# actionml/universal-recommender

Measured on AMD Instinct MI355X. Metric: cooccurrence pairs/sec (A'A+A'B) + LLR top-k items/sec, higher is better.
Workload: dtype int32 counts / f64 LLR; 1 GPU; config4: synthetic 10M users x 2M items, Zipf-1.0, 5 event types (purchase/view/add-to-cart/search/category-pref); generator=torch Philox on the GPU (universal_recommender_amd.synth.generate_device), maxEventsPerEventType=500, maxCorrelatorsPerEventType=50, seed=20260925, entry_point=urcco_context_build_device (C ABI, include/urcco.h), launch=one process per GPU, parallelism=items range-partitioned over 1 GPU(s), one HIP stream per event type

## Files before the change

universal-recommender_amd/csrc/cco_common.h:

```cpp
#pragma once
#include "cco_kernels.h"

namespace urcco {


constexpr int WAVE = 64;

__device__ __forceinline__ unsigned long long shfl_xor_u64(unsigned long long v, int m) {
  unsigned lo = (unsigned)v, hi = (unsigned)(v >> 32);
  lo = __shfl_xor(lo, m);
  hi = __shfl_xor(hi, m);
  return ((unsigned long long)hi << 32) | lo;
}
__device__ __forceinline__ long long shfl_i64(long long v, int src) {
  unsigned lo = (unsigned)v, hi = (unsigned)((unsigned long long)v >> 32);
  lo = __shfl(lo, src);
  hi = __shfl(hi, src);
  return (long long)(((unsigned long long)hi << 32) | lo);
}
__device__ __forceinline__ long long shfl_up_i64(long long v, unsigned d) {
  unsigned lo = (unsigned)v, hi = (unsigned)((unsigned long long)v >> 32);
  lo = __shfl_up(lo, d);
  hi = __shfl_up(hi, d);
  return (long long)(((unsigned long long)hi << 32) | lo);
}

__device__ __forceinline__ int64_t upper_bound_i64(const int64_t* __restrict__ rp, int64_t lo, int64_t hi, int64_t e) {
  while (lo < hi) {
    const int64_t mid = lo + ((hi - lo) >> 1);
    if (rp[mid] > e) hi = mid; else lo = mid + 1;
  }
  return lo;
}

constexpr int SCAN_THREADS = 256;
constexpr int SCAN_ITEMS = SCAN_TILE / SCAN_THREADS;

struct LoadI32 {
  const int32_t* p;
  __device__ __forceinline__ long long operator()(int64_t i) const { return p[i]; }
  __device__ __forceinline__ void load8(int64_t i, long long* x) const {
    if ((reinterpret_cast<uintptr_t>(p) & 15) == 0) {
      const int4 a = *reinterpret_cast<const int4*>(p + i), b = *reinterpret_cast<const int4*>(p + i + 4);
      x[0] = a.x; x[1] = a.y; x[2] = a.z; x[3] = a.w; x[4] = b.x; x[5] = b.y; x[6] = b.z; x[7] = b.w;
    } else {
#pragma unroll
      for (int q = 0; q < 8; ++q) x[q] = p[i + q];
    }
  }
};
struct LoadI64 {
  const int64_t* p;
  __device__ __forceinline__ long long operator()(int64_t i) const { return p[i]; }
  __device__ __forceinline__ void load8(int64_t i, long long* x) const {
    if ((reinterpret_cast<uintptr_t>(p) & 15) == 0) {
#pragma unroll
      for (int q = 0; q < 4; ++q) {
        const int4 a = *reinterpret_cast<const int4*>(p + i + 2 * q);
        x[2 * q] = (long long)(((unsigned long long)(unsigned)a.y << 32) | (unsigned)a.x);
        x[2 * q + 1] = (long long)(((unsigned long long)(unsigned)a.w << 32) | (unsigned)a.z);
      }
    } else {
#pragma unroll
      for (int q = 0; q < 8; ++q) x[q] = p[i + q];
    }
  }
};
template <int NT = SCAN_THREADS>
__device__ __forceinline__ long long block_exclusive_scan(long long v, long long* s_wave , long long* total) {
  const int lane = threadIdx.x & (WAVE - 1), wave = threadIdx.x / WAVE;
  long long inc = v;
#pragma unroll
  for (int d = 1; d < WAVE; d <<= 1) {
    const long long o = shfl_up_i64(inc, d);
    if (lane >= d) inc += o;
  }
  if (lane == WAVE - 1) s_wave[wave] = inc;
// ... 203 lines not shown
```

universal-recommender_amd/csrc/cco_expand.hip:

```cpp
#include "cco_kernels.h"

#include <atomic>
#include <cstdio>
#include <cstdlib>

#include "cco_common.h"
#include "cco_device.h"


namespace urcco {

__global__ __launch_bounds__(256) void item_entropy_kernel(const int32_t* __restrict__ counts, int32_t n, long long n_users,
                                                           double* __restrict__ ent, double* __restrict__ xlx_n) {
  const int64_t i = (int64_t)blockIdx.x * 256 + threadIdx.x;
  if (i < n) {
    const long long c = counts[i];
    ent[i] = entropy2(c, n_users - c);
  }
  if (i == 0 && xlx_n) *xlx_n = x_log_x(n_users);
}

hipError_t launch_item_entropy(hipStream_t st, const int32_t* counts, int32_t n, long long n_users, double* ent, double* xlx_n) {
  const int blocks = n > 0 ? (n + 255) / 256 : 1;
  hipLaunchKernelGGL(item_entropy_kernel, dim3(blocks), dim3(256), 0, st, counts, n, n_users, ent, xlx_n);
// ... 58 lines not shown
    const unsigned d0 = two ? (unsigned)cnt[z.x] : 0u, d1 = two ? (unsigned)cnt[z.y] : 0u, d2 = two ? (unsigned)cnt[z.z] : 0u, d3 = two ? (unsigned)cnt[z.w] : 0u;
    n_bad += (c0 >= limit) + (c1 >= limit) + (c2 >= limit) + (c3 >= limit) + (d0 >= limit) + (d1 >= limit) + (d2 >= limit) + (d3 >= limit);
    int4 y;
    y.x = (int)((unsigned)x.x | (c0 << shift)); y.y = (int)((unsigned)x.y | (c1 << shift));
    y.z = (int)((unsigned)x.z | (c2 << shift)); y.w = (int)((unsigned)x.w | (c3 << shift));
    nt_store4(out + 4 * v, y);
    if (two) {
      y.x = (int)((unsigned)z.x | (d0 << shift)); y.y = (int)((unsigned)z.y | (d1 << shift));
      y.z = (int)((unsigned)z.z | (d2 << shift)); y.w = (int)((unsigned)z.w | (d3 << shift));
      nt_store4(out + 4 * (v + stride), y);
    }
  }
  for (int64_t e = (nvec << 2) + (int64_t)blockIdx.x * 256 + threadIdx.x; e < nnz; e += stride) {
    const unsigned j = (unsigned)ci[e], c = (unsigned)cnt[j];
    n_bad += c >= limit;
    out[e] = (int)(j | (c << shift));
  }
  if (n_bad) atomicAdd(bad, n_bad);
}
hipError_t launch_pack_counts(hipStream_t st, int n_cu, const int32_t* col_idx, const int64_t* nnz_dev, int64_t nnz_bound, const unsigned short* counts16,
                              const int32_t* bad16, int32_t count_bits, int32_t* out, int32_t* bad) {
  hipError_t e = hipMemsetAsync(bad, 0, sizeof(int32_t), st);
  if (e != hipSuccess || nnz_bound <= 0) return e;
  const int shift = 32 - count_bits;
  int64_t blocks = (nnz_bound / 4 + 255) / 256;
  const int64_t cap = (int64_t)n_cu * 16;
  if (blocks > cap) blocks = cap;
  if (blocks < 1) blocks = 1;
  const int vec_ok = ((reinterpret_cast<uintptr_t>(col_idx) | reinterpret_cast<uintptr_t>(out)) & 15) == 0;
  hipLaunchKernelGGL(pack_counts_kernel, dim3((unsigned)blocks), dim3(256), 0, st, col_idx, nnz_dev, nnz_bound, counts16, bad16, shift, out, bad, vec_ok);
  return hipGetLastError();
}

__global__ __launch_bounds__(256) void xlx_table_kernel(double* __restrict__ tab) {
  const int x = blockIdx.x * 256 + threadIdx.x;
  if (x < XLX_TABLE) tab[x] = x_log_x((long long)x);
}
hipError_t launch_xlx_table(hipStream_t st, double* tab) {
  hipLaunchKernelGGL(xlx_table_kernel, dim3(XLX_TABLE / 256), dim3(256), 0, st, tab);
  return hipGetLastError();
}
__global__ __launch_bounds__(256) void xlx_hi_table_kernel(double* __restrict__ tab, const double* __restrict__ xlx_tab, long long n_users) {
  const int d = blockIdx.x * 256 + threadIdx.x;
  if (d >= XLX_TABLE) return;
  tab[d] = n_users - d >= 0 ? x_log_x(n_users - (long long)d) : 0.0;
  const double hi = n_users - d >= 0 ? x_log_x(n_users - (long long)d) : 0.0;
  tab[XLX_TABLE + d] = d <= n_users ? (x_log_x(n_users) - x_log_x_tab((long long)d, xlx_tab)) - hi : 0.0;
}
hipError_t launch_xlx_hi_table(hipStream_t st, double* tab, const double* xlx_tab, long long n_users) {
  hipLaunchKernelGGL(xlx_hi_table_kernel, dim3(XLX_TABLE / 256), dim3(256), 0, st, tab, xlx_tab, n_users);
  return hipGetLastError();
}

__global__ __launch_bounds__(SCAN_THREADS) void expand_downsweep_kernel(const int32_t* __restrict__ plen, int64_t n, const int64_t* __restrict__ tile_sums,
                                                                        int64_t n_tiles, int64_t* __restrict__ out, const int64_t* __restrict__ n_live,
                                                                        const int32_t* __restrict__ form, const unsigned* __restrict__ pstart32,
                                                                        int64_t* __restrict__ pstart64) {
  __shared__ long long s_wave[SCAN_THREADS / WAVE];
  if ((int64_t)blockIdx.x * SCAN_TILE > *n_live) return;
  const int f = *form;
  const LoadI32 ld{plen};
  const int64_t first = (int64_t)blockIdx.x * SCAN_TILE + (int64_t)threadIdx.x * SCAN_ITEMS;
  static_assert(SCAN_ITEMS == 8, "load8");
  long long x[SCAN_ITEMS];
  long long v = 0;
  const bool interior = first + SCAN_ITEMS <= n;
  if (interior) {
    ld.load8(first, x);
  } else {
#pragma unroll
    for (int q = 0; q < SCAN_ITEMS; ++q) x[q] = first + q < n ? ld(first + q) : 0;
  }
#pragma unroll
  for (int q = 0; q < SCAN_ITEMS; ++q) v += x[q];
  long long tot;
  long long run = block_exclusive_scan(v, s_wave, &tot) + tile_sums[blockIdx.x];
  if (f == 0) {
    unsigned* out32 = reinterpret_cast<unsigned*>(out);
    unsigned r = (unsigned)run;
    if (interior && (reinterpret_cast<uintptr_t>(out) & 15) == 0) {
      unsigned e[SCAN_ITEMS];
#pragma unroll
      for (int q = 0; q < SCAN_ITEMS; ++q) {
        e[q] = r;
        r += (unsigned)x[q];
      }
      *reinterpret_cast<uint4*>(out32 + first) = make_uint4(e[0], e[1], e[2], e[3]);
      *reinterpret_cast<uint4*>(out32 + first + 4) = make_uint4(e[4], e[5], e[6], e[7]);
    } else {
#pragma unroll
      for (int q = 0; q < SCAN_ITEMS; ++q) {
        if (first + q < n) out32[first + q] = r;
        r += (unsigned)x[q];
      }
    }
    if (blockIdx.x == 0 && threadIdx.x == 0) out32[n] = (unsigned)tile_sums[n_tiles];
    return;
  }
  if (interior && (reinterpret_cast<uintptr_t>(out) & 15) == 0) {
#pragma unroll
    for (int q = 0; q < SCAN_ITEMS; q += 2) {
      const long long e0 = run, e1 = run + x[q];
      run = e1 + x[q + 1];
      int4 w;
      w.x = (int)(unsigned)e0; w.y = (int)(unsigned)((unsigned long long)e0 >> 32);
      w.z = (int)(unsigned)e1; w.w = (int)(unsigned)((unsigned long long)e1 >> 32);
      *reinterpret_cast<int4*>(out + first + q) = w;
    }
  } else {
#pragma unroll
    for (int q = 0; q < SCAN_ITEMS; ++q) {
      const int64_t i = first + q;
      if (i < n) out[i] = run;
      run += x[q];
    }
  }
  if (!(f & FORM_PS64) && pstart32 && pstart64) {
#pragma unroll
    for (int q = 0; q < SCAN_ITEMS; ++q)
      if (first + q < n) pstart64[first + q] = (int64_t)pstart32[first + q];
  }
  if (blockIdx.x == 0 && threadIdx.x == 0) out[n] = tile_sums[n_tiles];
}
static hipError_t expand_scan(hipStream_t st, const int32_t* plen, int64_t cap, int64_t* wp, int64_t* tile_sums, const int64_t* n_live, bool tile_sums_ready,
                              const unsigned* pstart32, int64_t* pstart64, ExpandForm form) {
  const int64_t n_tiles = cap > 0 ? (cap + SCAN_TILE - 1) / SCAN_TILE : 1;
  if (!tile_sums_ready || cap <= 0)
    hipLaunchKernelGGL((scan_reduce_kernel<LoadI32>), dim3((unsigned)n_tiles), dim3(SCAN_THREADS), 0, st, LoadI32{plen}, cap, tile_sums, n_live);
  hipLaunchKernelGGL(scan_tiles_kernel, dim3(1), dim3(ST_THREADS), 0, st, tile_sums, n_tiles, n_live, form);
  hipLaunchKernelGGL(expand_downsweep_kernel, dim3((unsigned)n_tiles), dim3(SCAN_THREADS), 0, st, plen, cap, (const int64_t*)tile_sums, n_tiles, wp, n_live,
                     (const int32_t*)form.word, pstart32, pstart64);
  return hipGetLastError();
}

__global__ __launch_bounds__(256) void narrow_row_ptr_kernel(const int64_t* __restrict__ rp, int64_t n, unsigned* __restrict__ out) {
  for (int64_t i = (int64_t)blockIdx.x * 256 + threadIdx.x; i < n; i += (int64_t)gridDim.x * 256) out[i] = (unsigned)rp[i];
}

__global__ __launch_bounds__(256) void expand_prepare_kernel(const int64_t* __restrict__ a_cp, int32_t n_items_a, const int32_t* __restrict__ a_ri,
                                                             const int64_t* __restrict__ b_rp, const unsigned* __restrict__ b_rp32, int64_t n_rows_b,
                                                             int64_t cap, unsigned* __restrict__ pstart32, int64_t* __restrict__ pstart64,
                                                             int32_t* __restrict__ plen, int32_t* __restrict__ form) {
  const int64_t nnz = a_cp[n_items_a];
  int64_t lim = (nnz / SCAN_TILE + 1) * SCAN_TILE;
  if (lim > cap) lim = cap;
  const bool narrow = b_rp32 != nullptr && b_rp[n_rows_b] < ((int64_t)1 << 32);
  if (!narrow && pstart64 && blockIdx.x == 0 && threadIdx.x == 0) *form = FORM_PS64;
  const int64_t stride = (int64_t)gridDim.x * 256;
  for (int64_t p0 = (int64_t)blockIdx.x * 256 + threadIdx.x; p0 < lim; p0 += stride * 4) {
    int u[4];
#pragma unroll
    for (int q = 0; q < 4; ++q) {
      const int64_t p = p0 + q * stride;
      u[q] = p < nnz ? a_ri[p] : -1;
    }
    int64_t s[4], e[4];
    if (narrow) {
#pragma unroll
      for (int q = 0; q < 4; ++q) {
        s[q] = u[q] >= 0 ? (int64_t)b_rp32[u[q]] : 0;
        e[q] = u[q] >= 0 ? (int64_t)b_rp32[u[q] + 1] : 0;
      }
    } else {
#pragma unroll
      for (int q = 0; q < 4; ++q) {
        s[q] = u[q] >= 0 ? b_rp[u[q]] : 0;
        e[q] = u[q] >= 0 ? b_rp[u[q] + 1] : 0;
      }
    }
#pragma unroll
    for (int q = 0; q < 4; ++q) {
      const int64_t p = p0 + q * stride;
      if (p < lim) {
        if (narrow) {
          if (pstart32) pstart32[p] = (unsigned)s[q];
        } else if (pstart64) {
          pstart64[p] = s[q];
        }
        plen[p] = (int32_t)(e[q] - s[q]);
      }
    }
  }
}

hipError_t launch_expand_prepare(hipStream_t st, int n_cu, const int64_t* a_col_ptr, int32_t n_items_a, const int32_t* a_row_idx,
                                 const int64_t* b_row_ptr, unsigned* b_rp32_scratch, int64_t n_rows_b, int64_t cap, unsigned* pstart32, int64_t* pstart64,
                                 int32_t* plen, int64_t* wp, int64_t* tile_sums, ExpandForm form) {
  hipError_t e = hipMemsetAsync(form.word, 0, sizeof(int32_t), st);
  if (e != hipSuccess) return e;
  if (cap > 0) {
    if (b_rp32_scratch) {
      int64_t nb = (n_rows_b + 1 + 255) / 256;
      if (nb > (int64_t)n_cu * 8) nb = (int64_t)n_cu * 8;
      hipLaunchKernelGGL(narrow_row_ptr_kernel, dim3((unsigned)nb), dim3(256), 0, st, b_row_ptr, n_rows_b + 1, b_rp32_scratch);
    }
    int64_t blocks = (cap + 1023) / 1024;
    const int64_t lim = (int64_t)n_cu * 16;
    if (blocks > lim) blocks = lim;
    hipLaunchKernelGGL(expand_prepare_kernel, dim3((unsigned)blocks), dim3(256), 0, st, a_col_ptr, n_items_a, a_row_idx, b_row_ptr,
                       (const unsigned*)b_rp32_scratch, n_rows_b, cap, pstart32, pstart64, plen, form.word);
  }
  return expand_scan(st, plen, cap, wp, tile_sums, a_col_ptr + n_items_a, false, pstart32, pstart64, form);
}

struct __attribute__((packed, aligned(4))) Words4 { unsigned a, b, c, d; };
struct __attribute__((packed, aligned(4))) Words2 { unsigned a, b; };
struct ExpandMultiArgs {
  const int64_t* b_rp[EXPAND_MULTI_MAX];
  unsigned* pstart[EXPAND_MULTI_MAX];
  int32_t* plen[EXPAND_MULTI_MAX];
  int64_t* tsum[EXPAND_MULTI_MAX];
  int n;
};
__global__ __launch_bounds__(256) void expand_pack_kernel(ExpandMultiArgs a, int64_t n_rows_b, unsigned* __restrict__ T) {
  for (int64_t u = (int64_t)blockIdx.x * 256 + threadIdx.x; u <= n_rows_b; u += (int64_t)gridDim.x * 256)
    for (int d = 0; d < a.n; ++d) T[u * a.n + d] = (unsigned)a.b_rp[d][u];
}
template <int N>
__global__ __launch_bounds__(256) void expand_prepare_multi_kernel(const int64_t* __restrict__ a_cp, int32_t n_items_a, const int32_t* __restrict__ a_ri,
                                                                   const unsigned* __restrict__ T, int64_t cap, ExpandMultiArgs a) {
  __shared__ long long s_part[256 / WAVE][N];
  const int64_t nnz = a_cp[n_items_a];
  int64_t lim = (nnz / SCAN_TILE + 1) * SCAN_TILE;
  if (lim > cap) lim = cap;
  const int64_t n_tiles = (lim + SCAN_TILE - 1) / SCAN_TILE;
  for (int64_t tile = blockIdx.x; tile < n_tiles; tile += gridDim.x) {
    const int64_t base = tile * SCAN_TILE;
    long long sum[N];
#pragma unroll
    for (int d = 0; d < N; ++d) sum[d] = 0;
    for (int r = 0; r < SCAN_ITEMS; r += 2) {
      int u[2];
      unsigned v[2][2 * N];
#pragma unroll
      for (int q = 0; q < 2; ++q) {
        const int64_t p = base + (int64_t)(r + q) * 256 + threadIdx.x;
        u[q] = p < nnz ? a_ri[p] : -1;
      }
#pragma unroll
      for (int q = 0; q < 2; ++q) {
        if (u[q] >= 0) {
          const unsigned* t = T + (int64_t)u[q] * N;
          if (N == 4) {
            const uint4 x = *reinterpret_cast<const uint4*>(t), y = *reinterpret_cast<const uint4*>(t + 4);
            v[q][0] = x.x; v[q][1] = x.y; v[q][2] = x.z; v[q][3] = x.w;
            v[q][4 % (2 * N)] = y.x; v[q][5 % (2 * N)] = y.y; v[q][6 % (2 * N)] = y.z; v[q][7 % (2 * N)] = y.w;
          } else {
            constexpr int W = 2 * N;
#pragma unroll
            for (int d = 0; d + 4 <= W; d += 4) {
              const Words4 x = *reinterpret_cast<const Words4*>(t + d);
              v[q][d] = x.a; v[q][(d + 1) % W] = x.b; v[q][(d + 2) % W] = x.c; v[q][(d + 3) % W] = x.d;
            }
            if (W % 4 >= 2) {
              const Words2 x = *reinterpret_cast<const Words2*>(t + (W / 4) * 4);
              v[q][(W / 4) * 4 % W] = x.a; v[q][((W / 4) * 4 + 1) % W] = x.b;
            }
            if (W % 2 == 1) v[q][W - 1] = t[W - 1];
          }
        } else {
#pragma unroll
          for (int d = 0; d < 2 * N; ++d) v[q][d] = 0u;
        }
      }
#pragma unroll
      for (int q = 0; q < 2; ++q) {
        const int64_t p = base + (int64_t)(r + q) * 256 + threadIdx.x;
        if (p < lim) {
#pragma unroll
          for (int d = 0; d < N; ++d) {
            const int32_t len = (int32_t)(v[q][N + d] - v[q][d]);
            a.pstart[d][p] = v[q][d];
            a.plen[d][p] = len;
            sum[d] += (long long)len;
          }
        }
      }
    }
#pragma unroll
    for (int d = 0; d < N; ++d) {
      unsigned long long x = (unsigned long long)sum[d];
#pragma unroll
      for (int m = 1; m < WAVE; m <<= 1) x += shfl_xor_u64(x, m);
      if ((threadIdx.x & (WAVE - 1)) == 0) s_part[threadIdx.x / WAVE][d] = (long long)x;
    }
    __syncthreads();
    if (threadIdx.x < N && a.tsum[threadIdx.x]) {
      long long tot = 0;
#pragma unroll
      for (int w = 0; w < 256 / WAVE; ++w) tot += s_part[w][threadIdx.x];
      a.tsum[threadIdx.x][tile] = tot;
    }
    __syncthreads();
  }
}
hipError_t launch_expand_prepare_multi(hipStream_t st, int n_cu, const int64_t* a_col_ptr, int32_t n_items_a, const int32_t* a_row_idx, int n,
                                       const int64_t* const* b_row_ptr, int64_t n_rows_b, int64_t cap, unsigned* const* pstart, int32_t* const* plen, void* T,
                                       int64_t* const* tsum) {
  if (n < 1 || n > EXPAND_MULTI_MAX) return hipErrorInvalidValue;
  if (cap <= 0) return hipSuccess;
  ExpandMultiArgs a;
  a.n = n;
  for (int d = 0; d < EXPAND_MULTI_MAX; ++d) {
    a.b_rp[d] = d < n ? b_row_ptr[d] : nullptr;
    a.pstart[d] = d < n ? pstart[d] : nullptr;
    a.plen[d] = d < n ? plen[d] : nullptr;
    a.tsum[d] = (d < n && tsum) ? tsum[d] : nullptr;
  }
  int64_t nb = (n_rows_b + 255) / 256;
  if (nb > (int64_t)n_cu * 8) nb = (int64_t)n_cu * 8;
  if (nb < 1) nb = 1;
  hipLaunchKernelGGL(expand_pack_kernel, dim3((unsigned)nb), dim3(256), 0, st, a, n_rows_b, static_cast<unsigned*>(T));
  int64_t blocks = (cap + SCAN_TILE - 1) / SCAN_TILE;
  const int64_t lim = (int64_t)n_cu * 16;
  if (blocks > lim) blocks = lim;
  const unsigned* Tc = static_cast<const unsigned*>(T);
  switch (n) {
    case 1: hipLaunchKernelGGL(expand_prepare_multi_kernel<1>, dim3((unsigned)blocks), dim3(256), 0, st, a_col_ptr, n_items_a, a_row_idx, Tc, cap, a); break;
    case 2: hipLaunchKernelGGL(expand_prepare_multi_kernel<2>, dim3((unsigned)blocks), dim3(256), 0, st, a_col_ptr, n_items_a, a_row_idx, Tc, cap, a); break;
    case 3: hipLaunchKernelGGL(expand_prepare_multi_kernel<3>, dim3((unsigned)blocks), dim3(256), 0, st, a_col_ptr, n_items_a, a_row_idx, Tc, cap, a); break;
    case 4: hipLaunchKernelGGL(expand_prepare_multi_kernel<4>, dim3((unsigned)blocks), dim3(256), 0, st, a_col_ptr, n_items_a, a_row_idx, Tc, cap, a); break;
    case 5: hipLaunchKernelGGL(expand_prepare_multi_kernel<5>, dim3((unsigned)blocks), dim3(256), 0, st, a_col_ptr, n_items_a, a_row_idx, Tc, cap, a); break;
    case 6: hipLaunchKernelGGL(expand_prepare_multi_kernel<6>, dim3((unsigned)blocks), dim3(256), 0, st, a_col_ptr, n_items_a, a_row_idx, Tc, cap, a); break;
    case 7: hipLaunchKernelGGL(expand_prepare_multi_kernel<7>, dim3((unsigned)blocks), dim3(256), 0, st, a_col_ptr, n_items_a, a_row_idx, Tc, cap, a); break;
    default: hipLaunchKernelGGL(expand_prepare_multi_kernel<8>, dim3((unsigned)blocks), dim3(256), 0, st, a_col_ptr, n_items_a, a_row_idx, Tc, cap, a); break;
  }
  return hipGetLastError();
}
hipError_t launch_expand_scan(hipStream_t st, const int64_t* a_col_ptr, int32_t n_items_a, const int32_t* plen, int64_t cap, int64_t* wp, int64_t* tile_sums,
                              bool tile_sums_ready, const unsigned* pstart32, int64_t* pstart64, ExpandForm form) {
  hipError_t e = hipMemsetAsync(form.word, 0, sizeof(int32_t), st);
  if (e != hipSuccess) return e;
  return expand_scan(st, plen, cap, wp, tile_sums, a_col_ptr + n_items_a, tile_sums_ready, pstart32, pstart64, form);
}

__device__ __forceinline__ int64_t work_prefix_at(const int64_t* __restrict__ wp, const int64_t* __restrict__ tile_sums, bool narrow, int64_t p) {
  if (!narrow) return wp[p];
  const int64_t base = tile_sums[p / SCAN_TILE];
  return base + (int64_t)(unsigned)(reinterpret_cast<const unsigned*>(wp)[p] - (unsigned)base);
}
__global__ __launch_bounds__(256) void row_work_kernel(int32_t item_lo, int32_t item_hi, const int64_t* __restrict__ a_cp,
                                                       const int64_t* __restrict__ wp, const int64_t* __restrict__ tile_sums, const int32_t* __restrict__ form,
                                                       int64_t* __restrict__ work) {
  const int64_t n = (int64_t)item_hi - item_lo;
  const bool narrow = *form == 0;
  for (int64_t t = (int64_t)blockIdx.x * 256 + threadIdx.x; t < n; t += (int64_t)gridDim.x * 256) {
    const int64_t i = item_lo + t;
    work[t] = work_prefix_at(wp, tile_sums, narrow, a_cp[i + 1]) - work_prefix_at(wp, tile_sums, narrow, a_cp[i]);
  }
}

hipError_t launch_row_work(hipStream_t st, int n_cu, int32_t item_lo, int32_t item_hi, const int64_t* a_col_ptr, const int64_t* wp, const int64_t* tile_sums,
                           const int32_t* form, int64_t* work) {
  const int64_t n = (int64_t)item_hi - item_lo;
  if (n <= 0) return hipSuccess;
  int64_t blocks = (n + 255) / 256;
  const int64_t cap = (int64_t)n_cu * 8;
  if (blocks > cap) blocks = cap;
  hipLaunchKernelGGL(row_work_kernel, dim3((unsigned)blocks), dim3(256), 0, st, item_lo, item_hi, a_col_ptr, wp, tile_sums, form, work);
  return hipGetLastError();
}


}
```

universal-recommender_amd/csrc/cco_kernels.h:

```cpp
#pragma once
#include <hip/hip_runtime.h>
#include <stdint.h>

namespace urcco {

constexpr int NBINS = 7;
constexpr int MP_KMAX_HOST = 256;

constexpr int SCAN_TILE = 2048;
constexpr int DS_TILE = 4096;
constexpr int GLOBAL_BIN_BLOCKS = 128;
constexpr int BIN_TILE = 1024;
constexpr int XLX_TABLE_HOST = 4096;
constexpr int BIN_COLS_HOST = 3 * NBINS + 3;
constexpr int BIN_OFF_LEN = NBINS + 3;
constexpr int CAND_SLOTS = 64;
constexpr int STATS_LEN = 32;

constexpr int32_t DBG_GATHER_ONLY = 1;
constexpr int32_t DBG_NO_LLR = 2;
constexpr int32_t DBG_NO_TOPK = 4;
constexpr int32_t DBG_NO_SELECT = 8;
constexpr int32_t DBG_NO_RANK = 16;
constexpr int32_t DBG_NO_COUNT_GATHER = 512;
constexpr int32_t DBG_UNFUSED_EXPAND = 4096;
constexpr int32_t DBG_GATHERED_PRIMARY = 8192;
constexpr int32_t DBG_UNFILTERED_EXCHANGE = 16384;
constexpr int32_t DBG_SELECT_DELAY = 131072;
constexpr int32_t DBG_UNPACKED_COUNTS = 1048576;
constexpr int32_t DBG_ROW_KERNELS = DBG_GATHER_ONLY | DBG_NO_LLR | DBG_NO_TOPK | DBG_NO_SELECT | DBG_NO_RANK | DBG_NO_COUNT_GATHER | DBG_SELECT_DELAY;

constexpr int32_t FORM_WIDE = 1;
constexpr int32_t FORM_PS64 = 2;
constexpr int32_t FORM_TILE = 4;
constexpr int32_t FORM_PACK = 8;
constexpr int32_t FORM_HOST = 16;
constexpr unsigned long long NARROW_LIMIT = 1ull << 32;
struct ExpandForm {
  int32_t* word;
  const int32_t* pack_bad;
  int32_t host_wide;
  int32_t host_narrow;
  unsigned long long limit;
  long long seed;
};

struct CcoArgs {
  const int32_t* bin_rows;
  const int32_t* bin_off;
  const int64_t* a_col_ptr;
  const unsigned* pstart32;
  const int64_t* wp;
  const int32_t* b_col_idx;
  const int32_t* b_packed;
  const int32_t* form;
  int32_t pk_known;
  uint32_t b_col_mask;
  const int32_t* cnt_a;
  const int32_t* cnt_b;
  const double* ent_a;
  const unsigned short* cnt_b16;
  const int32_t* cnt16_bad;
  const double* xlx_n;
  const double* xlx_tab;
  const double* xlx_hi;
  const double* col_ent;
  int32_t debug;
  long long n_users;
  int32_t n_cols_b;
  int32_t item_lo;
  int32_t exclude_self;
  int32_t k;
  int32_t has_min_llr;
  double min_llr;
  int32_t count_bits;
  int32_t col_bytes;
  int32_t g_log2;
  int32_t unordered;
  int32_t* out_count;
  int32_t* out_idx;
  double* out_llr;
  unsigned long long* err;
  unsigned long long* cand;
  int32_t* g_counts;
  unsigned long long* g_cand_key;
  int32_t* g_cand_col;
  int32_t g_blocks;
  const int64_t* pstart64;
  const int64_t* work;
};

hipError_t launch_column_counts(hipStream_t st, int n_cu, const int32_t* col_idx, int64_t nnz, int32_t n_cols, int32_t* counts);
constexpr int64_t PH_MIN_NNZ = 1 << 20;
int64_t column_counts_scratch_bytes(int64_t nnz, int32_t n_cols);
hipError_t launch_column_counts_partitioned(hipStream_t st, const int32_t* col_idx, int64_t nnz, const int64_t* nnz_dev, int32_t n_cols,
                                            int32_t* counts, char* scratch);

hipError_t launch_scan_i32(hipStream_t st, const int32_t* in, int64_t n, int64_t* out, int64_t* tile_sums);
hipError_t launch_slice_weights(hipStream_t st, const unsigned short* loc_t, int n_buckets, int64_t n_parts, long long* weight);

hipError_t launch_downsample_flags(hipStream_t st, int n_cu, int64_t n_rows, const int64_t* row_ptr, const int32_t* col_idx, int64_t nnz,
                                   int32_t n_cols, const int32_t* raw_counts, unsigned long long* thresholds, uint32_t seed, int32_t max_n,
                                   int row_rate_mode, int64_t row_base, int64_t* tile_rows, unsigned long long* flags, int64_t* tile_count,
                                   int32_t* post_counts);
hipError_t launch_downsample_scan(hipStream_t st, int64_t nnz, int64_t* tile_count);
hipError_t launch_downsample_compact(hipStream_t st, int64_t n_rows, const int64_t* row_ptr, const int32_t* col_idx, int64_t nnz,
                                     const int64_t* tile_rows, const unsigned long long* flags, const int64_t* tile_off, int64_t* out_row_ptr,
                                     int32_t* out_col_idx);

hipError_t launch_scan_i32_range(hipStream_t st, const int32_t* in, int64_t n, int32_t lo, int32_t hi, int64_t* out, int64_t* tile_sums);
hipError_t launch_transpose(hipStream_t st, int n_cu, int64_t n_rows, const int64_t* row_ptr, const int32_t* col_idx, int g_log2,
                            const int64_t* col_ptr, int32_t* cursor, int32_t* out_row_idx, int32_t col_lo, int32_t col_hi);
int64_t transpose_scratch_bytes(int64_t n_rows, int64_t nnz, int32_t n_cols);
hipError_t launch_transpose_partitioned(hipStream_t st, int64_t n_rows, const int64_t* row_ptr, const int32_t* col_idx, int64_t nnz, int32_t n_cols,
                                        const int64_t* col_ptr, int32_t* cursor , int32_t* out_row_idx, int32_t col_lo, int32_t col_hi, char* scratch);
hipError_t launch_row_work_csr(hipStream_t st, int n_cu, int64_t n_rows, const int64_t* a_row_ptr, const int32_t* a_col_idx,
                               const int64_t* b_row_ptr, int g_log2, int32_t n_items_a, int64_t* work);

struct KeyTable {
  unsigned long long* keys;
  unsigned* minpos;
  unsigned* count;
  int32_t* id;
  unsigned long long mask;
};
hipError_t launch_dictionary_build(hipStream_t st, int n_cu, KeyTable t, int64_t n, const unsigned long long* keys, const int32_t* select,
                                   int32_t min_count, int32_t* flag, int64_t* prefix, int64_t* tile_sums, int64_t* first_pos);
hipError_t launch_dictionary_lookup(hipStream_t st, int n_cu, KeyTable t, int64_t n, const unsigned long long* keys, const int32_t* select,
                                    int32_t* ids);
hipError_t launch_dictionary_verify(hipStream_t st, int n_cu, KeyTable t, int64_t n, const unsigned long long* keys, const int32_t* select,
                                    const unsigned long long* check, const unsigned long long* ref_check, const int64_t* first_pos, unsigned long long* err);
hipError_t launch_csr_from_pairs(hipStream_t st, int n_cu, int64_t n, const int32_t* rows, const int32_t* cols, int64_t n_rows, int32_t* cnt,
                                 int64_t* raw_ptr, int32_t* tmp, int64_t* tile_sums, int64_t* out_row_ptr, int32_t* out_col_idx);

constexpr int EXCH_SIZES = 4;
hipError_t launch_row_lengths(hipStream_t st, int n_cu, int64_t n_rows, const int64_t* row_ptr, int32_t* len, unsigned short* len16, int64_t* sizes);
hipError_t launch_counts_over_limit(hipStream_t st, int n_cu, const int32_t* counts, int64_t n, int32_t count_bits, int64_t* out);
hipError_t launch_need_mask(hipStream_t st, int n_cu, int64_t n_rows, const int64_t* a_row_ptr, const int32_t* a_col_idx, const int32_t* bounds, int world,
                            unsigned long long* mask);
hipError_t launch_masked_lengths(hipStream_t st, int n_cu, int64_t n_rows, const int64_t* row_ptr, const unsigned long long* mask, int world, int32_t* mlen, int64_t* off,
                                 int64_t* tile_sums, int64_t* to_nnz);
hipError_t launch_pack_rows(hipStream_t st, int n_cu, int64_t n_rows, const int64_t* row_ptr, const int32_t* col_idx, const unsigned long long* mask, int world,
                            const int64_t* off, int32_t* pack);
hipError_t launch_scan_u16(hipStream_t st, const unsigned short* in, int64_t n, int64_t* out, int64_t* tile_sums);
hipError_t launch_frag_record(hipStream_t st, int32_t world, const int32_t* bounds, const int64_t* l_cp, const int32_t* bad, int64_t* rec);
hipError_t launch_frag_place(hipStream_t st, int n_cu, int32_t world, int32_t lo, int32_t n_range, const void* lens, int wire16, const int64_t* src_off,
                             const int32_t* ents, const int64_t* a_cp, const int64_t* sizes, int32_t* a_ri);

hipError_t launch_validate_csr(hipStream_t st, int n_cu, int64_t n_rows, const int64_t* row_ptr, const int32_t* col_idx, int64_t nnz, int32_t n_cols,
                               int g_log2, int64_t rp0, unsigned long long* err);
hipError_t launch_rebase_i64(hipStream_t st, int n_cu, int64_t* p, int64_t n, int64_t delta);
hipError_t launch_publish_word(hipStream_t st, const unsigned long long* src, unsigned long long* dst_mapped);

hipError_t launch_pop_counts(hipStream_t st, int n_cu, int64_t n, const int32_t* item, const int64_t* t_ms, int32_t n_items, int n_buckets,
                             const int64_t* bounds, int32_t* counts);

hipError_t launch_pack_counts(hipStream_t st, int n_cu, const int32_t* col_idx, const int64_t* nnz_dev, int64_t nnz_bound, const unsigned short* counts16,
                              const int32_t* bad16, int32_t count_bits, int32_t* out, int32_t* bad);
hipError_t launch_xlx_table(hipStream_t st, double* tab);
hipError_t launch_xlx_hi_table(hipStream_t st, double* tab , const double* xlx_tab, long long n_users);
hipError_t launch_item_entropy(hipStream_t st, const int32_t* counts, int32_t n, long long n_users, double* ent, double* xlx_n);
hipError_t launch_narrow_counts(hipStream_t st, int n_cu, const int32_t* counts, int64_t n, unsigned short* out16, int32_t* bad);

hipError_t launch_expand_prepare(hipStream_t st, int n_cu, const int64_t* a_col_ptr, int32_t n_items_a, const int32_t* a_row_idx,
                                 const int64_t* b_row_ptr, unsigned* b_rp32_scratch , int64_t n_rows_b, int64_t cap,
                                 unsigned* pstart32, int64_t* pstart64, int32_t* plen, int64_t* wp, int64_t* tile_sums, ExpandForm form);
constexpr int EXPAND_MULTI_MAX = 8;
hipError_t launch_expand_prepare_multi(hipStream_t st, int n_cu, const int64_t* a_col_ptr, int32_t n_items_a, const int32_t* a_row_idx, int n,
                                       const int64_t* const* b_row_ptr, int64_t n_rows_b, int64_t cap, unsigned* const* pstart, int32_t* const* plen, void* T,
                                       int64_t* const* tsum );
hipError_t launch_expand_scan(hipStream_t st, const int64_t* a_col_ptr, int32_t n_items_a, const int32_t* plen, int64_t cap, int64_t* wp, int64_t* tile_sums,
                              bool tile_sums_ready, const unsigned* pstart32, int64_t* pstart64, ExpandForm form);
hipError_t launch_row_work(hipStream_t st, int n_cu, int32_t item_lo, int32_t item_hi, const int64_t* a_col_ptr, const int64_t* wp, const int64_t* tile_sums,
                           const int32_t* form, int64_t* work);

hipError_t launch_binning(hipStream_t st, int32_t item_lo, int32_t n, const int64_t* work, const int32_t* cnt_a, int32_t n_cols_b,
                          int32_t count_bits, int32_t k, int64_t* tile_counts, int32_t* bin_off, int32_t* bin_rows, int64_t* stats);

hipError_t launch_cco_rows_bin(hipStream_t st, int n_cu, const CcoArgs& args, int bin, int32_t n_rows );
hipError_t launch_bin_out_stats(hipStream_t st, const int32_t* bin_rows, const int32_t* bin_off, int32_t item_lo, const int32_t* out_count,
                                const unsigned long long* cand, int64_t* stats);

hipError_t launch_compact_indicators(hipStream_t st, int32_t n_rows, int32_t k, const int32_t* count, const int32_t* idx,
                                     const double* llr, const int64_t* row_ptr, int32_t* out_idx, double* out_llr);

hipError_t launch_partition(hipStream_t st, int32_t n_items, const int64_t* work_prefix, int32_t n_parts, int32_t* bounds);
hipError_t launch_scan_i64(hipStream_t st, const int64_t* in, int64_t n, int64_t* out, int64_t* tile_sums);

constexpr int REC_MAX_CLAUSES = 16;
constexpr int REC_MAX_NUM = 256;
constexpr int REC_NO_BACKFILL = 1;
constexpr int REC_STATS_LEN = 8;
constexpr int REC_LDS_LIMIT = 3072;
struct RecClause {
  const int64_t* ind_col_ptr;
  const int32_t* ind_row_idx;
  const int64_t* q_row_ptr;
  const int32_t* q_col_idx;
  double boost;
  int32_t n_cols;
  int32_t reserved;
};
constexpr int REC_MAX_RULES = 16;
constexpr int REC_RULE_ANY = 0;
constexpr int REC_RULE_NONE = 1;
constexpr int REC_RULE_RANGE = 2;
struct RecRule {
  const int64_t* m_row_ptr;
  const int32_t* m_col_idx;
  const int64_t* q_row_ptr;
  const int32_t* q_col_idx;
  const int64_t* item_value;
  const int64_t* q_lo;
  const int64_t* q_hi;
  int32_t kind, n_cols;
};
struct RecArgs;
int32_t recommend_global_blocks(int64_t n_queries, int32_t n_items, int n_cu);
hipError_t launch_recommend(hipStream_t st, int n_cu, int64_t n_queries, int32_t n_items, const RecClause* clauses, int32_t n_clauses, const int64_t* excl_row_ptr,
                            const int32_t* excl_col_idx, const uint8_t* item_mask, const int32_t* fill_order, int32_t num, int32_t flags, int32_t* out_count,
                            int32_t* out_idx, double* out_score, int64_t* stats_dev, unsigned long long* ctr, int32_t* list, int32_t* pos, int32_t g_blocks,
                            unsigned* g_state, unsigned* g_m, int32_t* g_list, double* g_score, int32_t lds_limit = REC_LDS_LIMIT, const RecRule* rules = nullptr,
                            int32_t n_rules = 0);

hipError_t launch_llr_test(hipStream_t st, int64_t n, const int64_t* a, const int64_t* b, const int64_t* ab, const int64_t* nu, double* out);
hipError_t launch_u01_test(hipStream_t st, int64_t n, uint32_t seed, const int32_t* row, const int32_t* col, double* out, int rng32 = 0);

// ... 2 lines not shown
```

universal-recommender_amd/csrc/cco_rows.hip:

```cpp
#include "cco_kernels.h"

#include <atomic>
#include <cstdlib>

#include "cco_common.h"
#include "cco_device.h"


namespace urcco {

constexpr int E0 = 1024, E1S = 4096, E1 = 8192, E2S = 16384, E2 = 32768;
constexpr int MP_KMAX = 256;

__host__ __device__ constexpr int table_slots(int E, int T) { return (2 * E / 3) / (2 * T) * (2 * T); }
constexpr int URCCO_WB1 = 512;
constexpr int URCCO_WB2 = 8192;
__device__ __forceinline__ int choose_bin(long long w, long long ca, int32_t n_cols_b, int32_t count_bits, int32_t k) {
  if (ca <= 0 || w <= 0) return -1;
  if (count_bits < 31 && ca > ((1ll << count_bits) - 1)) return NBINS - 1;
  if (w <= 64 && ca <= 64) return 0;
  int cap_bin = NBINS - 1;
  const long long dmax = (w < (long long)n_cols_b ? w : (long long)n_cols_b) * 3 + (long long)k * 3 + 2;
  if (dmax <= E0) cap_bin = 1;
  else if (dmax <= E1S) cap_bin = 2;
// ... 390 lines not shown

template <int T>
__device__ __forceinline__ unsigned claim_positions(bool want, unsigned* counter, unsigned& wave_count) {
  const unsigned long long m = __ballot(want);
  const unsigned c = (unsigned)__popcll(m);
  unsigned base;
  if (T == WAVE) {
    base = wave_count;
    wave_count += c;
  } else {
    unsigned b = 0u;
    if ((threadIdx.x & (WAVE - 1)) == 0 && c != 0u) b = atomicAdd(counter, c);
    base = wave_read_lane(b, 0);
  }
  return base + lanes_below(m);
}
template <int T>
__device__ __forceinline__ unsigned team_exclusive_scan(unsigned v, unsigned* s_wsum , unsigned* total) {
  const int lane = threadIdx.x & (WAVE - 1);
  const unsigned inc = wave_inclusive_sum(v);
  if (T == WAVE) {
    *total = wave_read_lane(inc, WAVE - 1);
    return inc - v;
  }
  const int wave = (threadIdx.x % T) / WAVE;
  if (lane == WAVE - 1) s_wsum[wave] = inc;
  __syncthreads();
  unsigned base = 0, tot = 0;
#pragma unroll
  for (int w = 0; w < T / WAVE; ++w) {
    const unsigned sw = s_wsum[w];
    if (w < wave) base += sw;
    tot += sw;
  }
  __syncthreads();
  *total = tot;
  return base + inc - v;
}

constexpr int URCCO_U_WAVE = 2;
constexpr int URCCO_U_BS = 2;
constexpr int URCCO_U_B = 2;
constexpr int URCCO_U_H = 1;
constexpr int URCCO_U_C = 1;
constexpr int URCCO_OCC_WAVE = 8;
constexpr int URCCO_OCC_BS = 7;
constexpr int URCCO_G_WAVE = 2;
constexpr int URCCO_SEL_AMB_WAVE = 64;
constexpr int URCCO_SEL_AMB_BLOCK = 128;
constexpr int URCCO_G_BLOCK = 2;
constexpr int URCCO_SEL_M_BLOCK = 128;
constexpr int URCCO_G_CU = 2;
template <bool NARROW> struct PStart { typedef int64_t type; };
template <> struct PStart<true> { typedef unsigned type; };
template <int T, int E, int U, bool MP = false, bool DBG = false, bool PK = false>
__global__ __launch_bounds__((T < 256 ? 256 : T), (T == 64 ? URCCO_OCC_WAVE : (T == 256 && E == 4096 ? URCCO_OCC_BS : (T == 512 ? 4 : 1)))) void cco_rows_kernel(CcoArgs a, int bin) {
  if ((a.b_packed != nullptr && (a.pk_known != 0 || *a.form == 0)) != PK) return;
  using PS = typename PStart<PK>::type;
  constexpr int WS = PK ? 1 : 2;
  const int dbg = DBG ? a.debug : 0;
  constexpr bool packed = PK;
  URCCO_OWN_GLOBAL_PTR(const int32_t, b_col_idx, PK ? a.b_packed : a.b_col_idx);
  const int cshift = 32 - a.count_bits;
  const unsigned colmask = PK ? (1u << cshift) - 1u : a.b_col_mask;
  URCCO_OWN_GLOBAL_PTR(const unsigned short, cnt_b16, a.cnt_b16);
  URCCO_OWN_GLOBAL_PTR(const int32_t, cnt_b, a.cnt_b);
  URCCO_OWN_GLOBAL_PTR(const double, xlx_tab, a.xlx_tab);
  URCCO_OWN_GLOBAL_PTR(const double, xlx_hi, a.xlx_hi);
  URCCO_OWN_GLOBAL_PTR(const double, col_ent, a.col_ent);
  URCCO_OWN_GLOBAL_PTR(int32_t, out_idx, a.out_idx);
  URCCO_OWN_GLOBAL_PTR(double, out_llr, a.out_llr);
  long long n_users = a.n_users;
  URCCO_OWN_SGPRS(n_users);
  constexpr int BLOCK = T < 256 ? 256 : T;
  constexpr int TEAMS = BLOCK / T;
  constexpr int SH = table_slots(E, T);
  constexpr int SPT = SH / T;
  static_assert(SH % (2 * T) == 0 && SH + SH / 2 <= E && SH <= 65536, "slots and the candidate list share the table; a slot index takes 16 bits of a list word");
  constexpr unsigned CAND_CAP = (unsigned)(E - SH);
  constexpr int CPT = ((E - 5) / 3 + T - 1) / T;
  constexpr int NW = T / WAVE;
  constexpr int G = T == WAVE ? URCCO_G_WAVE : (T == 256 ? URCCO_G_BLOCK : URCCO_G_CU);
  constexpr int LOG2E = E == 1024 ? 10 : (E == 4096 ? 12 : (E == 8192 ? 13 : (E == 16384 ? 14 : 15)));
  static_assert((1 << LOG2E) == E, "table size");
  constexpr int LOG2T = T == 64 ? 6 : (T == 256 ? 8 : (T == 512 ? 9 : 10));
  static_assert((1 << LOG2T) == T, "team size");
  __shared__ __attribute__((aligned(16))) unsigned s_tab[TEAMS * E];
  constexpr int NH = T == WAVE ? 1 : 3;
  constexpr int SEL_CAP = T == WAVE ? 0 : (T == 256 ? 512 : 2048);
  constexpr int SEL_M = T == WAVE ? 64 : URCCO_SEL_M_BLOCK;
  constexpr int SEL_AMB = T == WAVE ? URCCO_SEL_AMB_WAVE : URCCO_SEL_AMB_BLOCK;
  static_assert(SEL_AMB <= SEL_M, "ambiguous set capacity");
  constexpr bool SHARE = T == WAVE || (T == 256 && E == 4096);
  constexpr int SH_INS = T * 8 + (T + 1) * 4;
  constexpr int SH_LST = ((NH * 128 * 4 > SEL_M * 12 ? NH * 128 * 4 : SEL_M * 12) + 7) / 8 * 8;
  constexpr int SH_SEL = SH_LST + SEL_CAP * 2;
  constexpr int SHARE_WORDS = ((SH_INS > SH_SEL ? SH_INS : SH_SEL) + 7) / 8;
  __shared__ unsigned long long s_share[SHARE ? TEAMS * SHARE_WORDS : 1];
  __shared__ long long s_ustart[SHARE ? 1 : TEAMS * T];
  __shared__ unsigned s_uoff[SHARE ? 1 : TEAMS * (T + 1)];
  __shared__ unsigned s_wsum[NW];
  __shared__ unsigned s_hist[SHARE ? 1 : TEAMS * NH * 128];
  __shared__ unsigned s_selres[TEAMS * 4];
  __shared__ unsigned short s_lst[SHARE ? 1 : TEAMS * (SEL_CAP > 0 ? SEL_CAP : 1)];
  __shared__ unsigned long long s_ambkey[SHARE ? 1 : TEAMS * SEL_M];
  __shared__ unsigned s_ambcol[SHARE ? 1 : TEAMS * SEL_M];
  __shared__ unsigned long long s_selthr[TEAMS * 2];
  constexpr bool SKIP_SHARED = T >= 256;
  __shared__ unsigned long long s_kbits[2 * NW];
  __shared__ unsigned s_mpflag;
  __shared__ unsigned s_ncand;
  __shared__ unsigned long long s_runk[MP ? 2 * MP_KMAX : 1];
  __shared__ unsigned s_runc[MP ? 2 * MP_KMAX : 1];

  const int team = TEAMS == 1 ? 0 : uni((int)threadIdx.x / T);
  const int tl = threadIdx.x % T;
  const int lane = threadIdx.x & (WAVE - 1);
  unsigned* tab = s_tab + team * E;
  unsigned* cand = tab + SH;
  unsigned long long* share = s_share + (SHARE ? team * SHARE_WORDS : 0);
  PS* ustart = reinterpret_cast<PS*>(SHARE ? reinterpret_cast<long long*>(share) : s_ustart + team * T);
  unsigned* uoff = SHARE ? reinterpret_cast<unsigned*>(share + T) : s_uoff + team * (T + 1);
  unsigned* hist = SHARE ? reinterpret_cast<unsigned*>(share) : s_hist + team * NH * 128;
  unsigned* sel_res = s_selres + team * 4;
  unsigned* nsel = sel_res + 3;
  unsigned short* lst = SHARE ? reinterpret_cast<unsigned short*>(share) + SH_LST / 2 : s_lst + team * (SEL_CAP > 0 ? SEL_CAP : 1);
  unsigned long long* amb_key = SHARE ? share : s_ambkey + team * SEL_M;
  unsigned* amb_col = SHARE ? reinterpret_cast<unsigned*>(share + SEL_M) : s_ambcol + team * SEL_M;
  unsigned long long* sel_thr = s_selthr + team * 2;
  const int list_start = a.bin_off[bin];
  const int list_n = a.bin_off[bin + 1] - list_start;
  const int total_teams = gridDim.x * TEAMS;
  bool ident = (long long)a.n_cols_b * 3 + (long long)a.k * 3 + 2 <= E && a.n_cols_b <= SH;
  int cb = a.count_bits;
  unsigned cmask = (1u << cb) - 1u;
  unsigned long long cand_acc = 0ull;
  const double xlx_n = *a.xlx_n;
  const bool use16 = *a.cnt16_bad == 0;

  int li = blockIdx.x * TEAMS + team;
  if (li >= list_n) return;
  const int S = total_teams;
  auto pos_of = [&](int l) { return list_start + (l < list_n ? l : list_n - 1); };
  const unsigned* wp32 = reinterpret_cast<const unsigned*>(a.wp);
  const PS* pstart;
  if constexpr (PK) pstart = a.pstart32;
  else pstart = a.pstart64;
  const int lane3 = lane < 3 ? lane : 2;
  int idv = a.bin_rows[pos_of(li + lane3 * S)];
  int64_t cs_c, ce_c;
  int64_t bnd_b;
  {
    const int id0 = (int)wave_read_lane((unsigned)idv, 0);
    const int id1 = (int)wave_read_lane((unsigned)idv, 1);
    cs_c = uni(a.a_col_ptr[id0]);
    ce_c = uni(a.a_col_ptr[id0 + 1]);
    bnd_b = a.a_col_ptr[id1 + (lane & 1)];
  }
  unsigned pf_w0, pf_w1, pf_wp;
  PS pf_start;
  {
    const int64_t c1 = cs_c + T < ce_c ? cs_c + T : ce_c;
    const int64_t pl = cs_c + tl < c1 ? cs_c + tl : c1 - 1;
    pf_w0 = wp32[WS * cs_c];
    pf_w1 = wp32[WS * c1];
    pf_wp = wp32[WS * pl];
    pf_start = pstart[pl];
  }
  URCCO_SETTLE(idv); URCCO_SETTLE(bnd_b); URCCO_SETTLE(pf_w0); URCCO_SETTLE(pf_w1); URCCO_SETTLE(pf_wp); URCCO_SETTLE(pf_start);
  int64_t cs_n = 0, ce_n = 0, bnd_c = 0;
  for (; li < list_n; li += S, cs_c = cs_n, ce_c = ce_n, bnd_b = bnd_c) {
    const int i = (int)wave_read_lane((unsigned)idv, 0);
    const int id2 = (int)wave_read_lane((unsigned)idv, 2);
    const int64_t cs = cs_c, ce = ce_c;
    cs_n = wave_read_lane64(bnd_b, 0);
    ce_n = wave_read_lane64(bnd_b, 1);
    const unsigned row_w0 = uni(pf_w0), row_w1 = uni(pf_w1);
    const unsigned my_wp = pf_wp;
    const PS my_start = pf_start;
    int lz = lane;
    URCCO_OPAQUE(lz);
    idv = a.bin_rows[pos_of(li + (1 + (lz < 3 ? lz : 2)) * S)];
    bnd_c = a.a_col_ptr[id2 + (lz & 1)];
    if (!MP) {
      const int64_t c1 = cs_n + T < ce_n ? cs_n + T : ce_n;
      const int64_t pl = cs_n + tl < c1 ? cs_n + tl : c1 - 1;
      pf_w0 = wp32[WS * cs_n];
      pf_w1 = wp32[WS * c1];
      pf_wp = wp32[WS * pl];
      pf_start = pstart[pl];
    }
    int mp_s = 0;
    unsigned mp_q = 0u, n_run = 0u, run_cur = 0u;
    if (MP) {
      const long long w_row = (long long)uni(a.work[i - a.item_lo]);
      const long long ca_row = a.cnt_a[i];
      const long long dd = w_row < (long long)a.n_cols_b ? w_row : (long long)a.n_cols_b;
      const long long cap = ((long long)E - 3ll * a.k - 2ll) / 3ll;
      for (;; ++mp_s) {
        const long long cols_pp = ((long long)a.n_cols_b + (1ll << mp_s) - 1) >> mp_s;
        int kb = 1;
        while ((1ll << kb) <= cols_pp) ++kb;
        const bool count_ok = kb <= 1 || ca_row <= (1ll << (32 - kb)) - 1;
        const long long exp_d = ((dd >> mp_s) + (dd >> (mp_s + 2)) + 1) < cols_pp ? ((dd >> mp_s) + (dd >> (mp_s + 2)) + 1) : cols_pp;
        if (count_ok && exp_d <= cap) break;
      }
    }
  mp_again:
    if (MP) {
      const long long cols_pp = ((long long)a.n_cols_b + (1ll << mp_s) - 1) >> mp_s;
      int kb = 1;
      while ((1ll << kb) <= cols_pp) ++kb;
      cb = 32 - kb;
      cmask = cb >= 32 ? 0xffffffffu : (1u << cb) - 1u;
      ident = cols_pp * 3 + 3ll * a.k + 2ll <= (long long)E && cols_pp <= (long long)SH;
      if (tl == 0) s_mpflag = 0u;
    }
    const unsigned mp_mask = MP ? (1u << mp_s) - 1u : 0u;
#pragma unroll
    for (int q = 0; q < SPT / 2; ++q) *reinterpret_cast<uint2*>(&tab[2 * (tl + q * T)]) = make_uint2(0u, 0u);
    unsigned n_cand = 0u;
    if (T != WAVE && tl == 0) s_ncand = 0u;
    team_sync<T>();
    for (int64_t c0 = cs; c0 < ce; c0 += T) {
      const int64_t c1 = c0 + T < ce ? c0 + T : ce;
      const bool pre = !MP && c0 == cs;
      const unsigned w0 = pre ? row_w0 : uni(wp32[WS * c0]);
      const unsigned total = (pre ? row_w1 : uni(wp32[WS * c1])) - w0;
      const int64_t p = c0 + tl;
      if (p < c1) {
        ustart[tl] = pre ? my_start : pstart[p];
        uoff[tl] = (pre ? my_wp : wp32[WS * p]) - w0;
      } else {
        uoff[tl] = total;
      }
      if (tl == 0) uoff[T] = total;
      team_sync<T>();
      if (total > 0u) {
        const unsigned per = (total + T - 1) / T;
        const unsigned first = (unsigned)tl * per;
        const bool act = first < total;
        const unsigned last = act ? (first + per < total ? first + per : total) : first;
        int o = 0;
        int64_t pos = 0;
        unsigned uend = 0u;
        if (act) {
          int lo = 1, hi = T;
#pragma unroll
          for (int step = 0; step < LOG2T; ++step) {
            const int mid = (lo + hi) >> 1;
            const bool gt = uoff[mid] > first;
            hi = gt ? mid : hi;
            lo = gt ? lo : mid + 1;
          }
          o = lo - 1;
          pos = (int64_t)ustart[o] + (first - uoff[o]);
          uend = uoff[o + 1];
        }
        for (unsigned x = 0; x < per; x += G) {
          unsigned jj[G];
          bool on[G];
#pragma unroll
          for (int q = 0; q < G; ++q) {
            const unsigned t = first + x + (unsigned)q;
            on[q] = t < last;
            jj[q] = 0u;
            if (on[q]) {
              if (t >= uend) {
                do { ++o; } while (uoff[o + 1] <= t);
                pos = (int64_t)ustart[o];
                uend = uoff[o + 1];
              }
              jj[q] = (unsigned)b_col_idx[pos++];
            }
          }
          unsigned at[G];
#pragma unroll
          for (int q = 0; q < G; ++q) {
            at[q] = ~0u;
            if (on[q]) {
              const unsigned col = jj[q] & colmask;
              if (dbg & DBG_GATHER_ONLY) {
                if (jj[q] == 0xffffffffu) tab[0] = 1u;
              } else if (MP) {
                if ((col & mp_mask) == mp_q && !tab_insert<SH>(tab, (col >> mp_s) + 1u, cb, ident, at[q])) s_mpflag = 1u;
// ... 72 lines not shown
    }
    cand_acc += D;
    unsigned long long* kk = reinterpret_cast<unsigned long long*>(tab + ((D + 1u) & ~1u));
    unsigned n_valid = 0;
    unsigned long long kand = ~0ull, kor = 0ull;
    {
      const long long ca = a.cnt_a[i];
      const double row_entropy = a.ent_a[i];
      for (unsigned base = 0; base < D; base += U * T) {
        const unsigned t0 = base + (unsigned)tl;
        unsigned vv[U];
        int cbj[U];
#pragma unroll
        for (int x = 0; x < U; ++x) {
          const unsigned t = t0 + (unsigned)x * T;
          vv[x] = t < D ? tab[t] : 0u;
          cbj[x] = 0;
          if (vv[x] != 0u) {
            const int j = MP ? (int)((((vv[x] >> cb) - 1u) << mp_s) | mp_q) : (int)(vv[x] >> cb) - 1;
            cbj[x] = packed ? (int)(unsigned)kk[t] : ((dbg & DBG_NO_COUNT_GATHER) ? (int)(vv[x] & cmask) + 100 : (use16 ? (int)cnt_b16[j] : cnt_b[j]));
          }
        }
        bool in_tables = true;
#pragma unroll
        for (int x = 0; x < U; ++x)
          if (vv[x] != 0u) in_tables = in_tables && llr_operands_in_tables(vv[x] & cmask, ca, (unsigned)cbj[x], n_users, col_ent);
        const bool all_in_tables = !(dbg & DBG_NO_LLR) && __ballot(!in_tables) == 0ull;
#pragma unroll
        for (int x = 0; x < U; ++x) {
          const unsigned t = t0 + (unsigned)x * T;
          if (t < D) {
            const int j = MP ? (int)((((vv[x] >> cb) - 1u) << mp_s) | mp_q) : (int)(vv[x] >> cb) - 1;
            const long long k11 = (long long)(vv[x] & cmask);
            unsigned long long key = 0ull;
            if (!(a.exclude_self && j == i)) {
              const double llr = all_in_tables ? llr_from_tables(row_entropy, xlx_n, (unsigned)k11, (unsigned)ca, (unsigned)cbj[x], xlx_tab, xlx_hi, col_ent)
                                               : ((dbg & DBG_NO_LLR) ? (double)k11
                                                            : llr_of(row_entropy, xlx_n, k11, ca, (long long)cbj[x], n_users, xlx_tab, xlx_hi, col_ent));
              if (llr > 0.0 && (!a.has_min_llr || llr >= a.min_llr)) key = (unsigned long long)__double_as_longlong(llr);
            }
            kk[t] = key;
            if (key != 0ull) {
              ++n_valid;
              if (SKIP_SHARED) {
                kand &= key;
                kor |= key;
              }
            }
          }
        }
      }
    }
    URCCO_SETTLE(idv); URCCO_SETTLE(bnd_c);
    if (!MP) { URCCO_SETTLE(pf_w0); URCCO_SETTLE(pf_w1); URCCO_SETTLE(pf_wp); URCCO_SETTLE(pf_start); }
    if (SKIP_SHARED) {
      wave_and_or_u64(kand, kor);
      if (lane == 0) {
        s_kbits[2 * (tl / WAVE)] = kand;
        s_kbits[2 * (tl / WAVE) + 1] = kor;
      }
    }
    unsigned C;
    team_exclusive_scan<T>(n_valid, s_wsum, &C);
    C = uni(C);
    team_sync<T>();
    const int64_t obase = ((int64_t)(i - a.item_lo)) * a.k;
    unsigned long long thr_key = 0ull;
    unsigned thr_ncol = 0u;
    bool row_done = false;
    if (!(dbg & DBG_NO_TOPK)) {
      if (dbg & DBG_NO_SELECT) {
        if (C > (unsigned)a.k) thr_key = ~0ull;
      } else if (C > (unsigned)a.k) {
        unsigned need = (unsigned)a.k;
        if (a.col_bytes < 4) thr_ncol = 0xffffffffu << (8 * a.col_bytes);
        int p0 = 0;
        if (!SKIP_SHARED) {
          kand = ~0ull;
          kor = 0ull;
          for (unsigned base = 0; base < D; base += T) {
            const unsigned t = base + (unsigned)tl;
            const unsigned long long key = t < D ? kk[t] : 0ull;
            if (key != 0ull) {
              kand &= key;
              kor |= key;
            }
          }
          wave_and_or_u64(kand, kor);
          if (T != WAVE) {
            if (lane == 0) {
              s_kbits[2 * (tl / WAVE)] = kand;
              s_kbits[2 * (tl / WAVE) + 1] = kor;
            }
            team_sync<T>();
          }
        }
        {
          if (T != WAVE) {
#pragma unroll
            for (int w = 0; w < NW; ++w) {
              kand &= s_kbits[2 * w];
              kor |= s_kbits[2 * w + 1];
            }
          }
          const unsigned long long kdiff = kand ^ kor;
          p0 = kdiff == 0ull ? 8 : (__clzll((long long)kdiff) >> 3);
          thr_key = p0 == 0 ? 0ull : (kor & ~(p0 >= 8 ? 0ull : (~0ull >> (8 * p0))));
// ... 267 lines not shown
    }
    team_sync<T>();
  }
  if (a.cand && tl == 0 && cand_acc != 0ull) atomicAdd(&a.cand[(blockIdx.x * TEAMS + team) & (CAND_SLOTS - 1)], cand_acc);
}

constexpr int URCCO_OCC_MICRO = 8;
template <int L> struct MicroGeom {
  static constexpr int S = WAVE / L;
  static constexpr int TW = 256 / S;
  static constexpr int LOG2TW = S == 1 ? 8 : (S == 2 ? 7 : 6);
  static constexpr int LIST = L + 4;
  static constexpr int MARKS = L + 2;
  static constexpr int ROW_WORDS = LIST + 2 * LIST + MARKS;
  static constexpr int WORDS = (256 + S * ROW_WORDS + 3) / 4 * 4;
};
template <int L>
__device__ __forceinline__ unsigned seg_inclusive_max(unsigned v) {
  if (L == WAVE) return wave_inclusive_max(v);
  int x = (int)v;
  int y;
  y = __builtin_amdgcn_update_dpp(0, x, 0x111, 0xf, 0xf, true);
  x = (unsigned)y > (unsigned)x ? y : x;
  y = __builtin_amdgcn_update_dpp(0, x, 0x112, 0xf, 0xf, true);
  x = (unsigned)y > (unsigned)x ? y : x;
  y = __builtin_amdgcn_update_dpp(0, x, 0x114, 0xf, 0xf, true);
  x = (unsigned)y > (unsigned)x ? y : x;
  y = __builtin_amdgcn_update_dpp(0, x, 0x118, 0xf, 0xf, true);
  x = (unsigned)y > (unsigned)x ? y : x;
  if (L == 32) {
    y = __builtin_amdgcn_update_dpp(0, x, 0x142, 0xa, 0xf, false);
    x = (unsigned)y > (unsigned)x ? y : x;
  }
  return (unsigned)x;
}
template <int L>
__device__ __forceinline__ unsigned seg_max_popc(unsigned long long m) {
  if (L == WAVE) return (unsigned)__popcll(m);
  unsigned best = 0;
#pragma unroll
  for (int q = 0; q < WAVE / L; ++q) {
    const unsigned c = (unsigned)__popcll((m >> (q * L)) & ((1ull << L) - 1ull));
    best = c > best ? c : best;
  }
  return best;
}

__device__ __forceinline__ unsigned gather_start(unsigned v, unsigned src) { return wave_gather(v, src); }
__device__ __forceinline__ int64_t gather_start(int64_t v, unsigned src) { return wave_gather64(v, src); }
template <int L, bool DBG, bool PK = false>
__global__ __launch_bounds__(256, (L == WAVE ? URCCO_OCC_MICRO : URCCO_OCC_MICRO - 2)) void cco_rows_micro_kernel(CcoArgs a) {
  if ((a.b_packed != nullptr && (a.pk_known != 0 || *a.form == 0)) != PK) return;
  using PS = typename PStart<PK>::type;
  constexpr int WS = PK ? 1 : 2;
  using G = MicroGeom<L>;
  constexpr int S = G::S;
  const int dbg = DBG ? a.debug : 0;
  const int32_t* bin_rows = a.bin_rows;
  const int64_t* a_col_ptr = a.a_col_ptr;
  const PS* pstart;
  if constexpr (PK) pstart = a.pstart32;
  else pstart = a.pstart64;
  constexpr bool packed = PK;
  const int32_t* b_col_idx = PK ? a.b_packed : a.b_col_idx;
  const int cshift = 32 - a.count_bits;
  const unsigned colmask = PK ? (1u << cshift) - 1u : a.b_col_mask;
  const int32_t* cnt_a = a.cnt_a;
  const double* ent_a = a.ent_a;
  const double* xlx_tab = a.xlx_tab;
  const double* xlx_hi = a.xlx_hi;
  const double* col_ent = a.col_ent;
  int32_t* out_idx = a.out_idx;
  double* out_llr = a.out_llr;
  int32_t* out_count = a.out_count;
  long long n_users = a.n_users;
  constexpr int TEAMS = 256 / WAVE;
  __shared__ __attribute__((aligned(16))) unsigned s_tab[TEAMS * G::WORDS];
  const int team = threadIdx.x / WAVE;
  const int lane = threadIdx.x & (WAVE - 1);
  const int seg = lane / L, sl = lane % L;
  const unsigned long long seg_mask = L == WAVE ? ~0ull : (((1ull << (L % WAVE)) - 1ull) << (seg * L));
  unsigned* tab_w = s_tab + team * G::WORDS;
  unsigned* tab = tab_w + seg * G::TW;
  unsigned* cand = tab_w + 256 + seg * G::ROW_WORDS;
  unsigned long long* kkm = reinterpret_cast<unsigned long long*>(cand + G::LIST);
  unsigned* marks = cand + 3 * G::LIST;
  const int list_start = L == 16 ? a.bin_off[0] : a.bin_off[NBINS + (L == 32 ? 1 : 2)];
  const int list_n = (L == 16 ? a.bin_off[NBINS + 1] : (L == 32 ? a.bin_off[NBINS + 2] : a.bin_off[1])) - list_start;
  const int n_groups = (list_n + S - 1) / S;
  const int total_teams = gridDim.x * TEAMS;
  const bool ident = a.n_cols_b <= G::TW;
  const int cb = a.count_bits;
  const unsigned cmask = (1u << cb) - 1u;
  const double xlx_n = *a.xlx_n;
  const bool use16 = *a.cnt16_bad == 0;
  unsigned long long cand_acc = 0ull;

  int li = blockIdx.x * TEAMS + team;
  if (li >= n_groups) return;
  const int stride = total_teams;
  auto row_at = [&](int g) { const int l = g * S + seg; return bin_rows[list_start + (l < list_n ? l : list_n - 1)]; };
  const unsigned* wp32 = reinterpret_cast<const unsigned*>(a.wp);
  const unsigned* cnt_words = use16 ? reinterpret_cast<const unsigned*>(a.cnt_b16) : reinterpret_cast<const unsigned*>(a.cnt_b);
  int i_cur = row_at(li);
  int i_n1 = row_at(li + stride);
  int i_n2 = row_at(li + 2 * stride);
  int64_t cs1 = a_col_ptr[i_n1], ce1 = a_col_ptr[i_n1 + 1];
  unsigned pf_w1, pf_wp;
  PS pf_start;
  int pf_ca;
  double pf_ent;
  int n_cur;
  {
    const int64_t cs0 = a_col_ptr[i_cur], ce0 = a_col_ptr[i_cur + 1];
    n_cur = (int)(ce0 - cs0);
    const int64_t pl = sl < n_cur ? cs0 + sl : ce0 - 1;
    pf_w1 = wp32[WS * ce0];
    pf_wp = wp32[WS * pl];
    pf_start = pstart[pl];
    pf_ca = cnt_a[i_cur];
    pf_ent = ent_a[i_cur];
  }
  URCCO_SETTLE(pf_w1); URCCO_SETTLE(pf_wp); URCCO_SETTLE(pf_start); URCCO_SETTLE(pf_ca); URCCO_SETTLE(pf_ent);
  URCCO_SETTLE(cs1); URCCO_SETTLE(ce1); URCCO_SETTLE(i_n2);
#pragma unroll
  for (int q = 0; q < 4; ++q) tab_w[lane + q * WAVE] = 0u;
  for (; li < n_groups; li += stride) {
    const int i = i_cur;
    const bool live = S == 1 || li * S + seg < list_n;
    const unsigned w0 = S == 1 ? wave_read_lane(pf_wp, 0) : wave_gather(pf_wp, (unsigned)(lane & ~(L - 1)));
    const unsigned total = live ? pf_w1 - w0 : 0u;
    const bool owns_user = live && sl < n_cur;
    const long long ca = (long long)pf_ca;
    const double row_entropy = pf_ent;
    const PS my_start = owns_user ? pf_start : (PS)0;
    const unsigned my_off = owns_user ? pf_wp - w0 : total;
    int i_n3 = row_at(li + 3 * stride);
    int64_t cs2 = a_col_ptr[i_n2], ce2 = a_col_ptr[i_n2 + 1];
    n_cur = (int)(ce1 - cs1);
    {
      const int64_t pl = sl < n_cur ? cs1 + sl : ce1 - 1;
      pf_w1 = wp32[WS * ce1];
      pf_wp = wp32[WS * pl];
      pf_start = pstart[pl];
      pf_ca = cnt_a[i_n1];
      pf_ent = ent_a[i_n1];
    }
    marks[sl] = 0u;
    wave_sync();
    if (owns_user) atomicMax(&marks[my_off], (unsigned)sl);
    wave_sync();
    const unsigned o = seg_inclusive_max<L>(marks[sl]);
    const PS base_o = gather_start(my_start - (PS)my_off, (unsigned)(seg * L) + o);
    unsigned slot = 0xffffffffu;
    unsigned jj = 0u;
    if ((unsigned)sl < total) {
      jj = (unsigned)b_col_idx[base_o + (PS)sl];
      if (!(dbg & DBG_GATHER_ONLY)) {
        bool ok;
        slot = tab_insert_claim(tab, (jj & colmask) + 1u, cb, (unsigned)(G::TW - 1), 32 - G::LOG2TW, ident, &ok);
        if (!ok) atomicAdd(a.err, 1ull);
      }
    }
    wave_sync();
    const bool is_cand = slot != 0xffffffffu;
    const unsigned long long cand_mask = __ballot(is_cand);
    const unsigned D = (unsigned)__popcll(cand_mask & seg_mask);
    const unsigned D_max = seg_max_popc<L>(cand_mask);
    cand_acc += (unsigned)__popcll(cand_mask);
    unsigned long long mk = 0ull;
    unsigned vv = 0u, cb_raw = 0u;
    if (is_cand) {
      vv = tab[slot];
      tab[slot] = 0u;
      const int j = (int)(vv >> cb) - 1;
      if (!packed) cb_raw = cnt_words[use16 ? j >> 1 : j];
    }
    if (D + (unsigned)sl < (unsigned)G::LIST) {
      kkm[D + (unsigned)sl] = 0ull;
      cand[D + (unsigned)sl] = 0xffffffffu;
    }
    bool in_tables = true;
    if (is_cand) {
      const int j = (int)(vv >> cb) - 1;
      const long long k11 = (long long)(vv & cmask);
      const unsigned cbj = packed ? jj >> cshift : ((dbg & DBG_NO_COUNT_GATHER) ? (unsigned)k11 + 100u : (use16 ? ((j & 1) ? cb_raw >> 16 : cb_raw & 0xffffu) : cb_raw));
      in_tables = llr_operands_in_tables((unsigned)k11, ca, cbj, n_users, col_ent);
    }
    const bool all_in_tables = !(dbg & DBG_NO_LLR) && __ballot(is_cand && !in_tables) == 0ull;
    if (is_cand) {
      const int j = (int)(vv >> cb) - 1;
      const long long k11 = (long long)(vv & cmask);
      if (!(a.exclude_self && j == i)) {
        const unsigned cbj = packed ? jj >> cshift : ((dbg & DBG_NO_COUNT_GATHER) ? (unsigned)k11 + 100u : (use16 ? ((j & 1) ? cb_raw >> 16 : cb_raw & 0xffffu) : cb_raw));
        const double llr = all_in_tables ? llr_from_tables(row_entropy, xlx_n, (unsigned)k11, (unsigned)ca, cbj, xlx_tab, xlx_hi, col_ent)
                                         : ((dbg & DBG_NO_LLR) ? (double)k11
                                                      : llr_of(row_entropy, xlx_n, k11, ca, (long long)cbj, n_users, xlx_tab, xlx_hi, col_ent));
        if (llr > 0.0 && (!a.has_min_llr || llr >= a.min_llr)) mk = (unsigned long long)__double_as_longlong(llr);
      }
      const unsigned pos = lanes_below(cand_mask & seg_mask);
      kkm[pos] = mk;
      cand[pos] = (unsigned)j;
    }
    wave_sync();
    const unsigned long long valid_mask = __ballot(mk != 0ull);
    const int n_valid = __popcll(valid_mask & seg_mask);
    const bool all_fit_k = (int)seg_max_popc<L>(valid_mask) <= a.k;
    auto settle_prefetch = [&]() {
      URCCO_SETTLE(pf_w1); URCCO_SETTLE(pf_wp); URCCO_SETTLE(pf_start); URCCO_SETTLE(pf_ca); URCCO_SETTLE(pf_ent);
      URCCO_SETTLE(cs2); URCCO_SETTLE(ce2); URCCO_SETTLE(i_n3);
    };
    if (a.unordered && all_fit_k && !(dbg & DBG_NO_TOPK)) {
      const int64_t obase = ((int64_t)(i - a.item_lo)) * a.k;
      settle_prefetch();
      if (mk != 0ull) {
        const unsigned opos = lanes_below(valid_mask & seg_mask);
        out_idx[obase + opos] = (int)(vv >> cb) - 1;
        out_llr[obase + opos] = __longlong_as_double((long long)mk);
      }
      if (sl == 0 && live) out_count[i - a.item_lo] = n_valid;
    } else if (!(dbg & DBG_NO_TOPK)) {
      const int64_t obase = ((int64_t)(i - a.item_lo)) * a.k;
      unsigned rank;
      unsigned long long rk;
      unsigned rc;
      unsigned ln = (unsigned)sl;
      URCCO_OPAQUE(ln);
      if (D_max <= (unsigned)(L / 4)) {
        const unsigned c = ln & (unsigned)(L / 4 - 1);
        rk = kkm[c];
        rc = cand[c];
        rank = rank_by_counting_strided<4>(kkm, cand, ln / (unsigned)(L / 4), (D_max + 3u) & ~3u, rk, rc);
        rank += (unsigned)__shfl_xor((int)rank, L / 4);
        rank += (unsigned)__shfl_xor((int)rank, L / 2);
      } else if (D_max <= (unsigned)(L / 2)) {
        const unsigned c = ln & (unsigned)(L / 2 - 1);
        rk = kkm[c];
        rc = cand[c];
        rank = rank_by_counting_strided<2>(kkm, cand, ln / (unsigned)(L / 2), (D_max + 1u) & ~1u, rk, rc);
        rank += (unsigned)__shfl_xor((int)rank, L / 2);
      } else {
        rk = kkm[ln];
        rc = cand[ln];
        rank = rank_by_counting_strided<1>(kkm, cand, 0u, D_max, rk, rc);
      }
      wave_sync();
      const unsigned n_out = (unsigned)(n_valid < a.k ? n_valid : a.k);
      if ((unsigned)sl < D && rk != 0ull && rank < n_out) {
        cand[rank] = rc;
        kkm[rank] = rk;
      }
      wave_sync();
      settle_prefetch();
      if ((unsigned)sl < n_out) {
        out_idx[obase + sl] = (int)cand[sl];
        out_llr[obase + sl] = __longlong_as_double((long long)kkm[sl]);
      }
      if (sl == 0 && live) out_count[i - a.item_lo] = (int)n_out;
    } else {
      settle_prefetch();
    }
    i_cur = i_n1;
    i_n1 = i_n2;
    i_n2 = i_n3;
    cs1 = cs2;
    ce1 = ce2;
    wave_sync();
  }
  if (a.cand && lane == 0 && cand_acc != 0ull) atomicAdd(&a.cand[(blockIdx.x * TEAMS + team) & (CAND_SLOTS - 1)], cand_acc);
}

constexpr int GB_THREADS = 1024;
constexpr int GSEL_K = 1024;

__device__ __forceinline__ int64_t g_start(const unsigned* ps32, const int64_t* ps64, bool nar, int64_t p) { return nar ? (int64_t)ps32[p] : ps64[p]; }
__device__ __forceinline__ int64_t g_len(const int64_t* wp, bool nar, int64_t p) {
  const unsigned* w = reinterpret_cast<const unsigned*>(wp);
  return nar ? (int64_t)(unsigned)(w[p + 1] - w[p]) : wp[p + 1] - wp[p];
}
__global__ __launch_bounds__(GB_THREADS) void cco_rows_global_kernel(CcoArgs a) {
  constexpr int NW = GB_THREADS / WAVE;
  __shared__ unsigned long long s_pkey[2][NW];
  __shared__ int s_pcol[2][NW];
  __shared__ int s_ncand;
  __shared__ unsigned s_hist[256];
  __shared__ unsigned s_sel[4];
  __shared__ int s_nsel;
  __shared__ unsigned long long s_selk[GSEL_K];
  __shared__ unsigned s_selc[GSEL_K];
  const int bin = NBINS - 1;
  const int list_start = a.bin_off[bin];
  const int list_n = a.bin_off[bin + 1] - list_start;
  int32_t* cnt = a.g_counts + (int64_t)blockIdx.x * a.n_cols_b;
  unsigned long long* ckey = a.g_cand_key + (int64_t)blockIdx.x * a.n_cols_b;
  int32_t* ccol = a.g_cand_col + (int64_t)blockIdx.x * a.n_cols_b;
  const int lane = threadIdx.x & (WAVE - 1), wv = threadIdx.x / WAVE;
  const int G = 1 << a.g_log2;
  const int grp = threadIdx.x >> a.g_log2, gl = threadIdx.x & (G - 1), ngrp = GB_THREADS >> a.g_log2;
  const double xlx_n = *a.xlx_n;
  const bool nar = *a.form == 0;
  for (int li = blockIdx.x; li < list_n; li += gridDim.x) {
    const int i = a.bin_rows[list_start + li];
    const int64_t cs = a.a_col_ptr[i], ce = a.a_col_ptr[i + 1];
    if (threadIdx.x == 0) s_ncand = 0;
    for (int64_t p = cs + grp; p < ce; p += ngrp) {
      const int64_t s = g_start(a.pstart32, a.pstart64, nar, p), e = s + g_len(a.wp, nar, p);
      for (int64_t q = s + gl; q < e; q += G) atomicAdd(&cnt[(unsigned)a.b_col_idx[q] & a.b_col_mask], 1);
    }
    __syncthreads();
    const long long ca = a.cnt_a[i];
    const double row_entropy = a.ent_a[i];
    for (int64_t p = cs + grp; p < ce; p += ngrp) {
      const int64_t s = g_start(a.pstart32, a.pstart64, nar, p), e = s + g_len(a.wp, nar, p);
      for (int64_t q = s + gl; q < e; q += G) {
        const int j = (int)((unsigned)a.b_col_idx[q] & a.b_col_mask);
        const long long k11 = atomicExch(&cnt[j], 0);
        if (k11 > 0 && !(a.exclude_self && j == i)) {
          const long long cbj = a.cnt_b[j];
          const double llr = llr_from_entropies_tab(row_entropy, column_entropy_of(cbj, xlx_n, a.n_users, a.xlx_tab, a.xlx_hi, a.col_ent), xlx_n, k11, ca - k11, cbj - k11,
                                                    a.n_users - ca - cbj + k11, a.xlx_tab, a.n_users, a.xlx_hi);
          if (llr > 0.0 && (!a.has_min_llr || llr >= a.min_llr)) {
            const int pos = atomicAdd(&s_ncand, 1);
            ckey[pos] = (unsigned long long)__double_as_longlong(llr);
            ccol[pos] = j;
          }
        }
      }
    }
    __syncthreads();
    const int ncand = s_ncand;
    const int64_t obase = ((int64_t)(i - a.item_lo)) * a.k;
    if (a.k <= GSEL_K) {
      unsigned long long thr_key = 0ull;
      unsigned thr_ncol = 0u;
      if (ncand > a.k) {
        unsigned need = (unsigned)a.k;
        if (a.col_bytes < 4) thr_ncol = 0xffffffffu << (8 * a.col_bytes);
        const int first_col_pass = 8 + (3 - (a.col_bytes - 1));
        for (int p = 0; p < 12; ++p) {
          if (p >= 8 && p < first_col_pass) continue;
          if (threadIdx.x < 256) s_hist[threadIdx.x] = 0u;
          __syncthreads();
          const int shk = p < 8 ? 56 - 8 * p : 0, shc = p < 8 ? 0 : 24 - 8 * (p - 8);
          for (int t = threadIdx.x; t < ncand; t += GB_THREADS) {
            const unsigned long long key = ckey[t];
            bool match;
            unsigned dig;
            if (p < 8) {
              match = p == 0 || (key >> (shk + 8)) == (thr_key >> (shk + 8));
              dig = (unsigned)(key >> shk) & 255u;
            } else {
              const unsigned ncol = ~(unsigned)ccol[t];
              match = key == thr_key && (p == first_col_pass || (ncol >> (shc + 8)) == (thr_ncol >> (shc + 8)));
              dig = (ncol >> shc) & 255u;
            }
            if (match) atomicAdd(&s_hist[dig], 1u);
          }
          __syncthreads();
          if (threadIdx.x == 0) {
            unsigned above = 0u, d = 255u;
            for (;; --d) {
              if (above + s_hist[d] >= need || d == 0u) break;
              above += s_hist[d];
            }
            s_sel[0] = d;
            s_sel[1] = s_hist[d];
// ... 188 lines not shown
```

universal-recommender_amd/csrc/urcco_api.hip:

```cpp
#include <memory>

#include "urcco_internal.h"

using namespace urcco_detail;

#include <signal.h>
#include <unistd.h>

#include <mutex>

namespace urcco_detail {
char* err_buf() {
  static thread_local char buf[512] = "";
  return buf;
}

const DebugCfg& debug_cfg() {
  static const DebugCfg cfg = [] {
    DebugCfg c;
    const char* m = getenv("URCCO_DEBUG_MARKS");
    const char* p = getenv("URCCO_DEBUG_POISON");
    c.marks = m && *m && *m != '0';
    c.poison = p && *p && *p != '0';
    return c;
// ... 258 lines not shown
    HIPC(urcco::launch_column_counts_partitioned(s->stream, out_col_idx, nnz, out_row_ptr + n_rows, n_cols, post_counts, s->take<char>((size_t)ph_bytes)));
    s->end();
  }
  return URCCO_OK;
}

int urcco_dev_transpose(urcco_session* s, int64_t n_rows, const int64_t* row_ptr, const int32_t* col_idx, int64_t nnz, int32_t n_cols,
                        const int32_t* counts, int32_t col_lo, int32_t col_hi, int64_t* out_col_ptr, int32_t* out_row_idx) {
  if (!s || n_rows < 0 || nnz < 0 || n_cols < 0 || !row_ptr || !out_col_ptr || (n_cols > 0 && !counts) || (nnz > 0 && (!col_idx || !out_row_idx)) ||
      col_lo < 0 || col_hi < col_lo || col_hi > n_cols)
    return fail(URCCO_BAD_ARG, "urcco_dev_transpose: bad argument");
  const int64_t n_tiles = ((int64_t)n_cols + urcco::SCAN_TILE - 1) / urcco::SCAN_TILE;
  const int64_t tr_bytes = urcco::transpose_scratch_bytes(n_rows, nnz, n_cols);
  URC(s->reserve(urcco_session::need((size_t)n_cols, 4) + urcco_session::need((size_t)n_tiles + 2, 8) + (size_t)tr_bytes + 256));
  int32_t* cursor = s->take<int32_t>((size_t)n_cols);
  int64_t* tile_sums = s->take<int64_t>((size_t)n_tiles + 2);
  s->begin(URCCO_STAGE_TRANSPOSE);
  HIPC(urcco::launch_scan_i32_range(s->stream, counts, n_cols, col_lo, col_hi, out_col_ptr, tile_sums));
  if (nnz > 0 && n_rows > 0) {
    int g = ceil_log2_i64((nnz + n_rows - 1) / n_rows);
    if (g < 1) g = 1;
    if (g > 6) g = 6;
    HIPC(hipMemsetAsync(cursor, 0, sizeof(int32_t) * (size_t)n_cols, s->stream));
    if (tr_bytes > 0) {
      HIPC(urcco::launch_transpose_partitioned(s->stream, n_rows, row_ptr, col_idx, nnz, n_cols, out_col_ptr, cursor, out_row_idx, col_lo, col_hi,
                                               s->take<char>((size_t)tr_bytes)));
    } else {
      HIPC(urcco::launch_transpose(s->stream, s->n_cu, n_rows, row_ptr, col_idx, g, out_col_ptr, cursor, out_row_idx, col_lo, col_hi));
    }
  }
  s->end();
  return URCCO_OK;
}

int urcco_dev_row_work_csr(urcco_session* s, int64_t n_rows, const int64_t* a_row_ptr, const int32_t* a_col_idx, int64_t nnz_a, const int64_t* b_row_ptr,
                           int32_t n_items_a, int64_t* work) {
  if (!s || n_rows < 0 || nnz_a < 0 || n_items_a < 0 || !a_row_ptr || !b_row_ptr || (nnz_a > 0 && !a_col_idx) || (n_items_a > 0 && !work))
    return fail(URCCO_BAD_ARG, "urcco_dev_row_work_csr: bad argument");
  int g = n_rows > 0 ? ceil_log2_i64((nnz_a + n_rows - 1) / n_rows) : 1;
  if (g < 1) g = 1;
  if (g > 6) g = 6;
  s->begin(URCCO_STAGE_ROW_WORK);
  HIPC(urcco::launch_row_work_csr(s->stream, s->n_cu, n_rows, a_row_ptr, a_col_idx, b_row_ptr, g, n_items_a, work));
  s->end();
  return URCCO_OK;
}

int urcco_dev_row_work(urcco_session* s, int32_t item_lo, int32_t item_hi, int32_t n_items_a, const int64_t* a_col_ptr, const int32_t* a_row_idx,
                       int64_t nnz_a_bound, const int64_t* b_row_ptr, int64_t* work) {
  if (!s || item_lo < 0 || item_hi < item_lo || item_hi > n_items_a || nnz_a_bound < 0 || !a_col_ptr || !b_row_ptr || (item_hi > item_lo && !work))
    return fail(URCCO_BAD_ARG, "urcco_dev_row_work: bad argument");
  const int64_t cap = nnz_a_bound;
  const int64_t n_tiles = (cap + urcco::SCAN_TILE - 1) / urcco::SCAN_TILE;
  URC(s->reserve(urcco_session::need((size_t)cap, 4) + urcco_session::need((size_t)cap + 1, 8) + urcco_session::need((size_t)n_tiles + 2, 8)));
  if (!s->form_word) HIPC(hipMalloc((void**)&s->form_word, sizeof(int32_t)));
  s->form_valid = false;
  int32_t* plen = s->take<int32_t>((size_t)cap);
  int64_t* wp = s->take<int64_t>((size_t)cap + 1);
  int64_t* tile_sums = s->take<int64_t>((size_t)n_tiles + 2);
  int32_t* form = s->form_word;
  s->begin(URCCO_STAGE_ROW_WORK);
  HIPC(urcco::launch_expand_prepare(s->stream, s->n_cu, a_col_ptr, n_items_a, a_row_idx, b_row_ptr, nullptr, 0, cap, nullptr, nullptr, plen, wp, tile_sums,
                                    urcco::ExpandForm{form, nullptr, 0, 0, s->narrow_limit, s->prefix_seed}));
  HIPC(urcco::launch_row_work(s->stream, s->n_cu, item_lo, item_hi, a_col_ptr, wp, tile_sums, form, work));
  s->form_valid = true;
  s->end();
  return URCCO_OK;
}

int urcco_dev_partition(urcco_session* s, int32_t n_items, const int64_t* work, int32_t n_parts, int32_t* bounds_host) {
  if (!s || n_items < 0 || n_parts <= 0 || n_parts > 4096 || !bounds_host || (n_items > 0 && !work)) return fail(URCCO_BAD_ARG, "urcco_dev_partition: bad argument");
  int32_t* bounds = nullptr;
  URC(urcco_detail::partition_dev(s, n_items, work, n_parts, nullptr, &bounds));
  HIPC(hipMemcpyAsync(bounds_host, bounds, sizeof(int32_t) * (size_t)(n_parts + 1), hipMemcpyDeviceToHost, s->stream));
  HIPC(hipStreamSynchronize(s->stream));
  return URCCO_OK;
}

int urcco_dev_merge_fragments(urcco_session* s, int32_t world, int32_t item_lo, int32_t item_hi, int32_t n_items, const void* lens, int32_t wire16,
                              const int32_t* entries, int64_t n_entries, const int64_t* sizes, const int32_t* counts, int64_t* out_col_ptr,
                              int32_t* out_row_idx) {
  if (!s || world <= 0 || item_lo < 0 || item_hi < item_lo || item_hi > n_items || n_entries < 0 || !sizes || !out_col_ptr || (n_items > 0 && !counts) ||
      (item_hi > item_lo && !lens) || (n_entries > 0 && (!entries || !out_row_idx)))
    return fail(URCCO_BAD_ARG, "urcco_dev_merge_fragments: bad argument");
  const int32_t n_range = item_hi - item_lo;
  const int64_t n_runs = (int64_t)world * n_range;
  const int64_t t_items = ((int64_t)n_items + urcco::SCAN_TILE - 1) / urcco::SCAN_TILE, t_runs = (n_runs + urcco::SCAN_TILE - 1) / urcco::SCAN_TILE;
  URC(s->reserve(urcco_session::need((size_t)n_runs + 1, 8) + urcco_session::need((size_t)(t_items > t_runs ? t_items : t_runs) + 2, 8)));
  int64_t* src_off = s->take<int64_t>((size_t)n_runs + 1);
  int64_t* tile_sums = s->take<int64_t>((size_t)(t_items > t_runs ? t_items : t_runs) + 2);
  s->begin(URCCO_STAGE_TRANSPOSE);
  HIPC(urcco::launch_scan_i32_range(s->stream, counts, n_items, item_lo, item_hi, out_col_ptr, tile_sums));
  if (wire16) {
    HIPC(urcco::launch_scan_u16(s->stream, static_cast<const unsigned short*>(lens), n_runs, src_off, tile_sums));
  } else {
    HIPC(urcco::launch_scan_i32(s->stream, static_cast<const int32_t*>(lens), n_runs, src_off, tile_sums));
  }
  HIPC(urcco::launch_frag_place(s->stream, s->n_cu, world, item_lo, n_range, lens, wire16, src_off, entries, out_col_ptr, sizes, out_row_idx));
  s->end();
  return URCCO_OK;
}

int urcco_dev_cco_rows(urcco_session* s, int32_t item_lo, int32_t item_hi, int32_t n_items_a, const int64_t* a_col_ptr,
                       const int32_t* a_row_idx, int64_t nnz_a_bound, const int64_t* b_row_ptr, const int32_t* b_col_idx, int32_t n_cols_b,
                       const int32_t* counts_a, const int32_t* counts_b, int64_t n_users, int32_t exclude_self, int32_t k,
                       int32_t has_min_llr, double min_llr, int32_t* out_count, int32_t* out_idx, double* out_llr, int64_t* stats_dev) {
  return urcco_detail::cco_rows_impl(s, item_lo, item_hi, n_items_a, a_col_ptr, a_row_idx, nnz_a_bound, b_row_ptr, b_col_idx, n_cols_b, counts_a, counts_b, n_users,
                                     exclude_self, k, has_min_llr, min_llr, out_count, out_idx, out_llr, stats_dev, nullptr, nullptr);
}

int urcco_dev_pack_counts(urcco_session* s, int64_t n_rows_b, const int64_t* b_row_ptr, const int32_t* b_col_idx, int64_t nnz_b_bound, const int32_t* counts_b,
                          int32_t n_cols_b, int32_t* out_packed, int32_t* out_bad) {
  return urcco_detail::pack_counts(s, b_row_ptr, n_rows_b, b_col_idx, nnz_b_bound, counts_b, n_cols_b, out_packed, out_bad);
}

int urcco_dev_cco_rows_packed(urcco_session* s, int32_t item_lo, int32_t item_hi, int32_t n_items_a, const int64_t* a_col_ptr,
                              const int32_t* a_row_idx, int64_t nnz_a_bound, const int64_t* b_row_ptr, const int32_t* b_col_idx, int32_t n_cols_b,
                              const int32_t* counts_a, const int32_t* counts_b, int64_t n_users, int32_t exclude_self, int32_t k,
                              int32_t has_min_llr, double min_llr, int32_t* out_count, int32_t* out_idx, double* out_llr, int64_t* stats_dev,
                              const int32_t* b_packed, const int32_t* pack_bad) {
  if ((b_packed == nullptr) != (pack_bad == nullptr)) return fail(URCCO_BAD_ARG, "urcco_dev_cco_rows_packed: b_packed and pack_bad come together");
  return urcco_detail::cco_rows_impl(s, item_lo, item_hi, n_items_a, a_col_ptr, a_row_idx, nnz_a_bound, b_row_ptr, b_col_idx, n_cols_b, counts_a, counts_b, n_users,
                                     exclude_self, k, has_min_llr, min_llr, out_count, out_idx, out_llr, stats_dev, nullptr, nullptr, nullptr, b_packed, pack_bad);
}

}

namespace urcco_detail {

int partition_dev(urcco_session* s, int32_t n_items, const int64_t* work, int32_t n_parts, int32_t* bounds_dev, int32_t** bounds_out) {
  const int64_t n_tiles = ((int64_t)n_items + urcco::SCAN_TILE - 1) / urcco::SCAN_TILE;
  URC(s->reserve(urcco_session::need((size_t)n_items + 1, 8) + urcco_session::need((size_t)n_tiles + 2, 8) + urcco_session::need((size_t)n_parts + 1, 4)));
  int64_t* prefix = s->take<int64_t>((size_t)n_items + 1);
  int64_t* tile_sums = s->take<int64_t>((size_t)n_tiles + 2);
  int32_t* bounds = bounds_dev ? bounds_dev : s->take<int32_t>((size_t)n_parts + 1);
  HIPC(urcco::launch_scan_i64(s->stream, work, n_items, prefix, tile_sums));
  HIPC(urcco::launch_partition(s->stream, n_items, prefix, n_parts, bounds));
  if (bounds_out) *bounds_out = bounds;
  return URCCO_OK;
}

int cco_rows_impl(urcco_session* s, int32_t item_lo, int32_t item_hi, int32_t n_items_a, const int64_t* a_col_ptr, const int32_t* a_row_idx, int64_t nnz_a_bound,
                  const int64_t* b_row_ptr, const int32_t* b_col_idx, int32_t n_cols_b, const int32_t* counts_a, const int32_t* counts_b, int64_t n_users,
                  int32_t exclude_self, int32_t k, int32_t has_min_llr, double min_llr, int32_t* out_count, int32_t* out_idx, double* out_llr, int64_t* stats_dev,
                  const unsigned* pre_pstart, const int32_t* pre_plen, int64_t* pre_tile_sums, const int32_t* b_packed, const int32_t* pack_bad, bool pk_known, int64_t b_nnz_bound) {
  if (!s || item_lo < 0 || item_hi < item_lo || item_hi > n_items_a || n_cols_b < 0 || n_users < 0 || nnz_a_bound < 0 || !a_col_ptr || !b_row_ptr)
    return fail(URCCO_BAD_ARG, "urcco_dev_cco_rows: bad argument");
  if (k <= 0) return fail(URCCO_BAD_ARG, "maxInterestingElements must be positive, got %d", k);
  const int32_t n = item_hi - item_lo;
  if (n == 0) {
    if (stats_dev) HIPC(hipMemsetAsync(stats_dev, 0, sizeof(int64_t) * URCCO_STATS_LEN, s->stream));
    return URCCO_OK;
  }
  if (!out_count || !out_idx || !out_llr || !counts_a || (n_cols_b > 0 && !counts_b)) return fail(URCCO_BAD_ARG, "urcco_dev_cco_rows: NULL buffer");
  HIPC(hipMemsetAsync(out_count, 0, sizeof(int32_t) * (size_t)n, s->stream));
  if (n_cols_b == 0 || n_users == 0) {
    if (stats_dev) HIPC(hipMemsetAsync(stats_dev, 0, sizeof(int64_t) * URCCO_STATS_LEN, s->stream));
    return URCCO_OK;
  }
  int key_bits = 1;
  while (((int64_t)1 << key_bits) <= (int64_t)n_cols_b) ++key_bits;
  const int count_bits = 32 - key_bits;
  if (count_bits < 1) return fail(URCCO_BAD_ARG, "n_cols_b %d too large for the packed accumulator", n_cols_b);
  const bool dense_bin6 = k > urcco::MP_KMAX_HOST || 3ll * k + 5 > 32768ll;
  if (dense_bin6) URC(s->ensure_global_bin(n_cols_b));
  if (!s->xlx_tab) {
    HIPC(hipMalloc((void**)&s->xlx_tab, sizeof(double) * urcco::XLX_TABLE_HOST));
    HIPC(urcco::launch_xlx_table(s->stream, s->xlx_tab));
  }
  if (!s->xlx_hi) HIPC(hipMalloc((void**)&s->xlx_hi, sizeof(double) * 2 * urcco::XLX_TABLE_HOST));
  if (s->xlx_hi_n != n_users) {
    HIPC(urcco::launch_xlx_hi_table(s->stream, s->xlx_hi, s->xlx_tab, n_users));
    s->xlx_hi_n = n_users;
  }
  const int64_t n_tiles = ((int64_t)n + urcco::BIN_TILE - 1) / urcco::BIN_TILE;
  const int64_t cap = nnz_a_bound;
  const int64_t p_tiles = (cap + urcco::SCAN_TILE - 1) / urcco::SCAN_TILE;
  if (!s->form_word) HIPC(hipMalloc((void**)&s->form_word, sizeof(int32_t)));
  s->form_valid = false;
  URC(s->reserve(urcco_session::need((size_t)cap, 8) + urcco_session::need((size_t)cap, 4) + (pre_pstart ? 0 : urcco_session::need((size_t)cap, 4)) + urcco_session::need((size_t)cap + 1, 8) +
                 urcco_session::need((size_t)p_tiles + 2, 8) +
                 urcco_session::need((size_t)n, 8) + urcco_session::need((size_t)(n_tiles + 1) * urcco::BIN_COLS_HOST, 8) +
                 urcco_session::need(urcco::BIN_OFF_LEN, 4) + urcco_session::need((size_t)n, 4) + urcco_session::need((size_t)n_items_a, 8) +
                 urcco_session::need((size_t)n_cols_b, 2) + urcco_session::need(1, 4) + urcco_session::need(urcco::CAND_SLOTS, 8) + urcco_session::need(1, 8) + urcco_session::need(URCCO_STATS_LEN, 8) +
                 urcco_session::need((size_t)n_users + 1, 4)));
  int64_t* pstart64 = s->take<int64_t>((size_t)cap);
  unsigned* own_pstart = pre_pstart ? nullptr : s->take<unsigned>((size_t)cap);
  int32_t* own_plen = s->take<int32_t>((size_t)cap);
  const unsigned* pstart32 = pre_pstart ? pre_pstart : own_pstart;
  int64_t* wp = s->take<int64_t>((size_t)cap + 1);
  int32_t* form = s->form_word;
  int64_t* p_tile_sums = s->take<int64_t>((size_t)p_tiles + 2);
  int64_t* work = s->take<int64_t>((size_t)n);
  int64_t* tile_counts = s->take<int64_t>((size_t)(n_tiles + 1) * urcco::BIN_COLS_HOST);
  int32_t* bin_off = s->take<int32_t>(urcco::BIN_OFF_LEN);
  int32_t* bin_rows = s->take<int32_t>((size_t)n);
  double* ent_a = s->take<double>((size_t)n_items_a);
  unsigned short* cnt_b16 = s->take<unsigned short>((size_t)n_cols_b);
  int32_t* cnt16_bad = s->take<int32_t>(1);
  unsigned long long* cand = s->take<unsigned long long>(urcco::CAND_SLOTS);
  double* xlx_n = s->take<double>(1);
  int64_t* stats = stats_dev ? stats_dev : s->take<int64_t>(URCCO_STATS_LEN);
  unsigned* b_rp32 = s->take<unsigned>((size_t)n_users + 1);

  const int32_t* packed = pk_known ? b_col_idx : ((b_packed && pack_bad && !(s->debug & urcco::DBG_UNPACKED_COUNTS)) ? b_packed : nullptr);
  const bool host_wide = packed == nullptr || (s->debug & urcco::DBG_ROW_KERNELS) != 0;
  const bool narrow_known = pk_known && !host_wide && b_nnz_bound >= 0 && b_nnz_bound < ((int64_t)1 << 32) &&
                            (unsigned long long)n_cols_b * (unsigned long long)urcco::SCAN_TILE < s->narrow_limit;
  const urcco::ExpandForm ef{form, pk_known ? nullptr : pack_bad, host_wide ? 1 : 0, narrow_known ? 1 : 0, s->narrow_limit, s->prefix_seed};
  int64_t* tile_sums = (pre_pstart && pre_plen && pre_tile_sums) ? pre_tile_sums : p_tile_sums;
  s->begin(URCCO_STAGE_ROW_WORK);
  if (pre_pstart && pre_plen)
    HIPC(urcco::launch_expand_scan(s->stream, a_col_ptr, n_items_a, pre_plen, cap, wp, tile_sums, pre_tile_sums != nullptr, pre_pstart, pstart64, ef));
  else
    HIPC(urcco::launch_expand_prepare(s->stream, s->n_cu, a_col_ptr, n_items_a, a_row_idx, b_row_ptr, b_rp32, n_users, cap, own_pstart, pstart64, own_plen, wp, tile_sums, ef));
  HIPC(urcco::launch_row_work(s->stream, s->n_cu, item_lo, item_hi, a_col_ptr, wp, tile_sums, form, work));
  s->form_valid = true;
  s->end();
  s->begin(URCCO_STAGE_BINNING);
  HIPC(hipMemsetAsync(stats, 0, sizeof(int64_t) * URCCO_STATS_LEN, s->stream));
  HIPC(urcco::launch_binning(s->stream, item_lo, n, work, counts_a, n_cols_b, count_bits, k, tile_counts, bin_off, bin_rows, stats));
  s->end();
  s->begin(URCCO_STAGE_ENTROPY);
  HIPC(urcco::launch_item_entropy(s->stream, counts_a, n_items_a, n_users, ent_a, xlx_n));
  HIPC(urcco::launch_narrow_counts(s->stream, s->n_cu, counts_b, n_cols_b, cnt_b16, cnt16_bad));
  s->end();

  urcco::CcoArgs a;
  a.bin_rows = bin_rows; a.bin_off = bin_off;
  a.a_col_ptr = a_col_ptr; a.pstart32 = pstart32; a.pstart64 = pstart64; a.wp = wp; a.form = form; a.work = work; a.b_col_idx = b_col_idx;
  a.b_packed = packed; a.pk_known = narrow_known ? 1 : 0;
  a.b_col_mask = pk_known ? (key_bits >= 32 ? 0xffffffffu : (1u << key_bits) - 1u) : 0xffffffffu;
  a.cnt_a = counts_a; a.cnt_b = counts_b; a.ent_a = ent_a; a.cnt_b16 = cnt_b16; a.cnt16_bad = cnt16_bad; a.xlx_n = xlx_n; a.xlx_tab = s->xlx_tab; a.xlx_hi = s->xlx_hi; a.col_ent = s->xlx_hi + urcco::XLX_TABLE_HOST; a.debug = s->debug;
  a.n_users = n_users; a.n_cols_b = n_cols_b; a.item_lo = item_lo; a.exclude_self = exclude_self ? 1 : 0; a.k = k;
  a.has_min_llr = has_min_llr ? 1 : 0; a.min_llr = min_llr; a.count_bits = count_bits;
  a.col_bytes = n_cols_b <= (1 << 8) ? 1 : (n_cols_b <= (1 << 16) ? 2 : (n_cols_b <= (1 << 24) ? 3 : 4));
  a.unordered = s->unordered_rows ? 1 : 0;
  a.g_log2 = 4;
  a.out_count = out_count; a.out_idx = out_idx; a.out_llr = out_llr;
  a.err = reinterpret_cast<unsigned long long*>(stats + 1 + 4 * urcco::NBINS);
  a.cand = s->timing ? cand : nullptr;
  if (s->timing) HIPC(hipMemsetAsync(cand, 0, sizeof(unsigned long long) * urcco::CAND_SLOTS, s->stream));
  a.g_counts = s->g_counts; a.g_cand_key = s->g_cand_key; a.g_cand_col = s->g_cand_col; a.g_blocks = dense_bin6 ? s->g_blocks : 0;
  for (int step = 0; step < urcco::NBINS; ++step) {
    const int bin = urcco::NBINS - 1 - step;
    s->begin(URCCO_STAGE_CCO_BIN0 + bin);
    HIPC(urcco::launch_cco_rows_bin(s->stream, s->n_cu, a, bin, n));
    s->end();
  }
  if (s->timing) HIPC(urcco::launch_bin_out_stats(s->stream, bin_rows, bin_off, item_lo, out_count, cand, stats));
  return URCCO_OK;
}

int pack_counts(urcco_session* s, const int64_t* b_row_ptr, int64_t n_rows_b, const int32_t* b_col_idx, int64_t nnz_bound, const int32_t* counts_b, int32_t n_cols_b,
                int32_t* out, int32_t* bad) {
  if (!s || !b_row_ptr || n_rows_b < 0 || nnz_bound < 0 || !out || !bad || (nnz_bound > 0 && (!b_col_idx || !counts_b))) return fail(URCCO_BAD_ARG, "pack_counts: bad argument");
  int key_bits = 1;
  while (((int64_t)1 << key_bits) <= (int64_t)n_cols_b) ++key_bits;
  const int count_bits = 32 - key_bits;
  if (count_bits < 1) return fail(URCCO_BAD_ARG, "n_cols_b %d too large for the packed accumulator", n_cols_b);
  URC(s->reserve(urcco_session::need((size_t)n_cols_b + 8, 2) + urcco_session::need(1, 4) + 256));
  unsigned short* c16 = s->take<unsigned short>((size_t)n_cols_b + 8);
  int32_t* bad16 = s->take<int32_t>(1);
  s->begin(URCCO_STAGE_ENTROPY);
  HIPC(urcco::launch_narrow_counts(s->stream, s->n_cu, counts_b, n_cols_b, c16, bad16));
  HIPC(urcco::launch_pack_counts(s->stream, s->n_cu, b_col_idx, b_row_ptr + n_rows_b, nnz_bound, c16, bad16, count_bits, out, bad));
  s->end();
  return URCCO_OK;
}

int expand_multi(urcco_session* s, int n, const int64_t* a_col_ptr, int32_t n_items_a, const int32_t* a_row_idx, int64_t cap, const int64_t* const* b_row_ptr,
                 int64_t n_users, unsigned* const* pstart, int32_t* const* plen, int64_t* const* tile_sums) {
  if (!s || n < 1 || n > urcco::EXPAND_MULTI_MAX || !a_col_ptr || cap < 0) return fail(URCCO_BAD_ARG, "expand_multi: bad argument");
  URC(s->reserve(urcco_session::need(((size_t)n_users + 2) * (size_t)n, 4) + 256));
  void* T = s->take<unsigned>(((size_t)n_users + 2) * (size_t)n);
  s->begin(URCCO_STAGE_ROW_WORK);
  HIPC(urcco::launch_expand_prepare_multi(s->stream, s->n_cu, a_col_ptr, n_items_a, a_row_idx, n, b_row_ptr, n_users, cap, pstart, plen, T, tile_sums));
  s->end();
  return URCCO_OK;
}

}

extern "C" {

int urcco_dev_compact_indicators(urcco_session* s, int32_t n_rows, int32_t k, const int32_t* count, const int32_t* idx, const double* llr,
                                 int64_t* out_row_ptr, int32_t* out_col_idx, double* out_llr) {
  if (!s || n_rows < 0 || k <= 0 || !out_row_ptr || (n_rows > 0 && (!count || !idx || !llr || !out_col_idx || !out_llr)))
    return fail(URCCO_BAD_ARG, "urcco_dev_compact_indicators: bad argument");
  const int64_t n_tiles = ((int64_t)n_rows + urcco::SCAN_TILE - 1) / urcco::SCAN_TILE;
  URC(s->reserve(urcco_session::need((size_t)n_tiles + 2, 8)));
  int64_t* tile_sums = s->take<int64_t>((size_t)n_tiles + 2);
  s->begin(URCCO_STAGE_COMPACT_INDICATORS);
  HIPC(urcco::launch_scan_i32(s->stream, count, n_rows, out_row_ptr, tile_sums));
  HIPC(urcco::launch_compact_indicators(s->stream, n_rows, k, count, idx, llr, out_row_ptr, out_col_idx, out_llr));
  s->end();
  return URCCO_OK;
}

struct urcco_key_table {
  urcco::KeyTable t{};
  int64_t capacity = 0;
  int device = 0;
};

void urcco_key_table_destroy(urcco_key_table* table) {
  if (!table) return;
  (void)hipSetDevice(table->device);
  if (table->t.keys) (void)hipFree(table->t.keys);
  if (table->t.minpos) (void)hipFree(table->t.minpos);
  if (table->t.count) (void)hipFree(table->t.count);
  if (table->t.id) (void)hipFree(table->t.id);
  delete table;
}

int urcco_dev_dictionary_build(urcco_session* s, int64_t n, const uint64_t* keys, const int32_t* select, int32_t min_count,
                               int64_t* first_pos, urcco_key_table** table, int64_t* n_ids) {
  if (!s || n < 0 || (n > 0 && (!keys || !first_pos)) || !table || !n_ids) return fail(URCCO_BAD_ARG, "urcco_dev_dictionary_build: bad argument");
  if (n >= ((int64_t)1 << 32) - 1) return fail(URCCO_BAD_ARG, "urcco_dev_dictionary_build: at most 2^32 - 2 events per stream, got %lld", (long long)n);
  *table = nullptr;
  std::unique_ptr<urcco_key_table, void (*)(urcco_key_table*)> tab(new (std::nothrow) urcco_key_table(), urcco_key_table_destroy);
  if (!tab) return fail(URCCO_OOM_HOST, "key table alloc");
  tab->device = s->device;
  int64_t cap = 1024;
  while (cap < 2 * n) cap <<= 1;
  tab->capacity = cap;
  tab->t.mask = (unsigned long long)cap - 1ull;
  HIPC(hipMalloc((void**)&tab->t.keys, sizeof(unsigned long long) * (size_t)cap));
  HIPC(hipMalloc((void**)&tab->t.minpos, sizeof(unsigned) * (size_t)cap));
  HIPC(hipMalloc((void**)&tab->t.count, sizeof(unsigned) * (size_t)cap));
// ... 173 lines not shown
```

universal-recommender_amd/csrc/urcco_context.hip:

```cpp
#include <dlfcn.h>

#include <algorithm>
#include <atomic>
#include <chrono>
#include <condition_variable>
#include <functional>
#include <memory>
#include <future>
#include <mutex>
#include <string>
#include <thread>
#include <unordered_map>

#include "urcco_internal.h"

using namespace urcco_detail;

namespace {

struct Rccl {
  typedef struct { char internal[URCCO_UNIQUE_ID_BYTES]; } UniqueId;
  typedef void* Comm;
  void* handle = nullptr;
  int (*GetUniqueId)(UniqueId*) = nullptr;
// ... 99 lines not shown
    return false;
  }
  void trim() {
    std::lock_guard<std::mutex> g(mu);
    std::vector<Block> keep;
    for (Block& b : blocks) {
      if (b.used) keep.push_back(b);
      else (void)hipHostFree(b.p);
    }
    blocks.swap(keep);
  }
};
PinnedPool& pinned_pool() {
  static PinnedPool* pool = new PinnedPool();
  return *pool;
}

constexpr int A_SETS = 2;

struct EvState {
  urcco_session* s = nullptr;
  DBuf<int64_t> in_rp;
  DBuf<int32_t> in_ci;
  DBuf<int32_t> raw, post;
  DBuf<int64_t> s_rp;
  DBuf<int32_t> s_ci;
  DBuf<int32_t> deg, f_deg;
  DBuf<unsigned short> deg16, f_deg16;
  DBuf<int64_t> f_rp;
  DBuf<int32_t> f_ci;
  DBuf<int64_t> sizes;
  DBuf<int64_t> scan_tmp;
  DBuf<int32_t> o_count, o_idx;
  DBuf<double> o_llr;
  DBuf<int64_t> c_rp;
  DBuf<int32_t> c_idx;
  DBuf<double> c_llr;
  DBuf<int64_t> stats;
  DBuf<unsigned long long> verr;
  DBuf<int32_t> b_pk;
  DBuf<int32_t> pk_bad;
  DBuf<int32_t> s_pk;
  bool b_pk_known = false;
  uint32_t b_col_mask = 0xffffffffu;
  unsigned long long* h_verr = nullptr;
  unsigned long long* h_verr_dev = nullptr;
  int ensure_h_verr() {
    if (h_verr) return URCCO_OK;
    HIPC(hipHostMalloc((void**)&h_verr, sizeof(unsigned long long), hipHostMallocMapped | hipHostMallocCoherent));
    HIPC(hipHostGetDevicePointer((void**)&h_verr_dev, h_verr, 0));
    return URCCO_OK;
  }
  DBuf<unsigned> pre_pstart;
  DBuf<int32_t> pre_plen;
  DBuf<int64_t> pre_tsum;
  DBuf<int32_t> mlen, pack;
  DBuf<unsigned short> mlen16;
  DBuf<int32_t> mlen_bad;
  DBuf<int64_t> moff, mtmp, to_nnz;
  hipEvent_t ev_sampled = nullptr, ev_done = nullptr, ev_rp = nullptr;
  hipEvent_t ev_cons[A_SETS] = {};
  bool cons_valid[A_SETS] = {};
  const int64_t* b_rp = nullptr;
  const int32_t* b_ci = nullptr;
  int64_t b_rows = 0, b_nnz_bound = 0;
  void release() {
    in_rp.release(); in_ci.release(); raw.release(); post.release(); s_rp.release(); s_ci.release(); deg.release(); f_deg.release();
    deg16.release(); f_deg16.release();
    f_rp.release(); f_ci.release(); sizes.release(); scan_tmp.release(); o_count.release(); o_idx.release(); o_llr.release(); c_rp.release();
    c_idx.release(); c_llr.release(); stats.release(); verr.release(); b_pk.release(); pk_bad.release(); s_pk.release(); pre_pstart.release(); pre_plen.release(); pre_tsum.release();
    mlen.release(); pack.release(); mlen16.release(); mlen_bad.release(); moff.release(); mtmp.release(); to_nnz.release();
    if (h_verr) (void)hipHostFree(h_verr);
    h_verr = nullptr;
    h_verr_dev = nullptr;
    if (ev_sampled) (void)hipEventDestroy(ev_sampled);
    if (ev_done) (void)hipEventDestroy(ev_done);
    if (ev_rp) (void)hipEventDestroy(ev_rp);
    for (int q = 0; q < A_SETS; ++q) {
      if (ev_cons[q]) (void)hipEventDestroy(ev_cons[q]);
      ev_cons[q] = nullptr;
      cons_valid[q] = false;
    }
    ev_sampled = ev_done = ev_rp = nullptr;
  }
};

struct DevState {
  int device = 0;
  int rank = 0;
  int n_cu = 256;
  std::vector<urcco_session*> sessions;
  std::vector<EvState> ev;
  DBuf<int64_t> a_cp[A_SETS];
  DBuf<int32_t> a_ri[A_SETS];
  DBuf<int32_t> a_post[A_SETS];
  int par = 0;
  DBuf<int64_t> work;
  DBuf<int32_t> bounds;
  DBuf<int32_t> l_cnt, l_ri, len_bad, f_ent;
  DBuf<int64_t> l_cp, rec;
  DBuf<unsigned short> len16;
  DBuf<char> f_len;
  DBuf<unsigned long long> need;
  hipEvent_t need_ready = nullptr;
  hipEvent_t a_ready = nullptr, in_ready = nullptr, b_expanded = nullptr;
  Rccl::Comm comm = nullptr;
  int32_t item_lo = 0, item_hi = 0;
  int64_t a_ents = 0;
};

struct Shard {
  int64_t n_rows = 0, row_base = 0, nnz = 0;
  const int64_t* rp = nullptr;
  const int32_t* ci = nullptr;
};
struct DsParams {
  int64_t n_cols = 0;
  int32_t max_rows = 500, k = 50, has_min_llr = 0;
  double min_llr = 0.0;
};

struct DevWorkers {
  std::vector<std::thread> threads;
// ... 214 lines not shown
    s->unordered_rows = (c->flags & URCCO_FLAG_UNORDERED_ROWS) ? 1 : 0;
    D.sessions.push_back(s);
  }
  if ((int)D.ev.size() < n_ds) D.ev.resize((size_t)n_ds);
  for (int d = 0; d < n_ds; ++d) {
    EvState& E = D.ev[(size_t)d];
    E.s = sess_of(c, D, d);
    E.s->unordered_rows = (c->flags & URCCO_FLAG_UNORDERED_ROWS) ? 1 : 0;
    if (!E.ev_sampled) HIPC(hipEventCreateWithFlags(&E.ev_sampled, hipEventDisableTiming));
    if (!E.ev_done) HIPC(hipEventCreateWithFlags(&E.ev_done, hipEventDisableTiming));
    for (int q = 0; q < A_SETS; ++q)
      if (!E.ev_cons[q]) HIPC(hipEventCreateWithFlags(&E.ev_cons[q], hipEventDisableTiming));
    if (!E.ev_rp) HIPC(hipEventCreateWithFlags(&E.ev_rp, hipEventDisableTiming));
  }
  if (!D.a_ready) HIPC(hipEventCreateWithFlags(&D.a_ready, hipEventDisableTiming));
  if (!D.in_ready) HIPC(hipEventCreateWithFlags(&D.in_ready, hipEventDisableTiming));
  if (!D.b_expanded) HIPC(hipEventCreateWithFlags(&D.b_expanded, hipEventDisableTiming));
  if (!D.need_ready) HIPC(hipEventCreateWithFlags(&D.need_ready, hipEventDisableTiming));
  return URCCO_OK;
}

int stage_raw_counts(DevState& D, EvState& E, const Shard& sh, const DsParams& p) {
  URC(E.raw.ensure((size_t)p.n_cols + 1));
  return urcco_dev_column_counts(E.s, sh.nnz, sh.ci, (int32_t)p.n_cols, E.raw.p);
}
DBuf<int32_t>& post_of(DevState& D, int d) { return d == 0 ? D.a_post[D.par] : D.ev[(size_t)d].post; }

int stage_downsample(urcco_context* c, DevState& D, int d, const Shard& sh, const DsParams& p, int32_t seed) {
  EvState& E = D.ev[(size_t)d];
  URC(E.s_rp.ensure((size_t)sh.n_rows + 1));
  URC(E.s_ci.ensure((size_t)sh.nnz + 4));
  URC(post_of(D, d).ensure((size_t)p.n_cols + 1));
  return urcco_dev_downsample(E.s, sh.n_rows, sh.rp, sh.ci, sh.nnz, (int32_t)p.n_cols, E.raw.p, seed, p.max_rows, c->row_rate_mode, sh.row_base, E.s_rp.p,
                              E.s_ci.p, post_of(D, d).p);
}

int stage_rows(DevState& D, EvState& E, EvState& A, int d, const DsParams& pa, const DsParams& p, int64_t n_users, int64_t a_nnz_bound, bool pre_expanded = false) {
  const int32_t n = D.item_hi - D.item_lo;
  const size_t strided = (size_t)(n > 0 ? n : 1) * (size_t)p.k;
  URC(E.o_count.ensure((size_t)n + 1));
  URC(E.o_idx.ensure(strided));
  URC(E.o_llr.ensure(strided));
  URC(E.c_rp.ensure((size_t)n + 2));
  URC(E.c_idx.ensure(strided));
  URC(E.c_llr.ensure(strided));
  URC(E.stats.ensure(URCCO_STATS_LEN));
  if (!E.b_pk_known) {
    URC(E.b_pk.ensure((size_t)E.b_nnz_bound + 4));
    URC(E.pk_bad.ensure(1));
    URC(pack_counts(E.s, E.b_rp, E.b_rows, E.b_ci, E.b_nnz_bound, post_of(D, d).p, (int32_t)p.n_cols, E.b_pk.p, E.pk_bad.p));
  }
  URC(cco_rows_impl(E.s, D.item_lo, D.item_hi, (int32_t)pa.n_cols, D.a_cp[D.par].p, D.a_ri[D.par].p, a_nnz_bound, E.b_rp, E.b_ci, (int32_t)p.n_cols,
                    post_of(D, 0).p, post_of(D, d).p, n_users, d == 0 ? 1 : 0, p.k, p.has_min_llr, p.min_llr, E.o_count.p, E.o_idx.p, E.o_llr.p, E.stats.p,
                    pre_expanded ? E.pre_pstart.p : nullptr, pre_expanded ? E.pre_plen.p : nullptr, pre_expanded ? E.pre_tsum.p : nullptr,
                    E.b_pk_known ? nullptr : E.b_pk.p, E.b_pk_known ? nullptr : E.pk_bad.p, E.b_pk_known, E.b_nnz_bound));
  URC(urcco_dev_compact_indicators(E.s, n, p.k, E.o_count.p, E.o_idx.p, E.o_llr.p, E.c_rp.p, E.c_idx.p, E.c_llr.p));
  HIPC(hipEventRecord(E.ev_done, E.s->stream));
  HIPC(hipEventRecord(E.ev_cons[D.par], E.s->stream));
  E.cons_valid[D.par] = true;
  return URCCO_OK;
}

struct InputGate {
  const HostTrace* trace = nullptr;
  std::function<int(int)> after_chain;
  std::vector<int> order;
  std::vector<std::promise<int>> staged;
  std::vector<std::shared_future<int>> fut;
  std::vector<char> released;
  explicit InputGate(int n) : staged((size_t)n), fut((size_t)n), released((size_t)n, 0) {
    for (int d = 0; d < n; ++d) fut[(size_t)d] = staged[(size_t)d].get_future().share();
  }
  void release(int d, int status) {
    released[(size_t)d] = 1;
    staged[(size_t)d].set_value(status);
  }
  int wait(DevState& D, int d) {
    const int st = fut[(size_t)d].get();
    if (st != URCCO_OK) return fail(st, "dataset %d: staging failed", d);
    EvState& E = D.ev[(size_t)d];
    HIPC(hipStreamSynchronize(E.s->stream));
    const unsigned long long bad = E.h_verr ? *(volatile unsigned long long*)E.h_verr : 0ull;
    if (bad)
      return fail(URCCO_BAD_ARG, "dataset %d: %llu invalid entries (row_ptr not monotone, or col_idx out of [0, n_cols) / not strictly increasing inside a row)", d, bad);
    if (trace) trace->mark("matrices landed and checked", d);
    return URCCO_OK;
  }
};

int build_single(urcco_context* c, DevState& D, const std::vector<Shard>& sh, const std::vector<DsParams>& ps_, int64_t n_users, int32_t seed,
                 InputGate* gate) {
  const int n_ds = (int)sh.size();
  URC(set_dev(D));
  EvState& A = D.ev[0];
  D.item_lo = 0;
  D.item_hi = (int32_t)ps_[0].n_cols;
  URC(D.a_cp[D.par].ensure((size_t)ps_[0].n_cols + 2));
  URC(D.a_ri[D.par].ensure((size_t)sh[0].nnz + 4));
  std::atomic<bool> a_ok{false};
  const bool threaded = n_ds > 1 && !c->single_stream();
  std::promise<void> a_recorded;
  std::shared_future<void> a_recorded_f = a_recorded.get_future().share();
  bool fuse = n_ds >= 3 && n_ds - 1 <= urcco::EXPAND_MULTI_MAX && !(c->debug & urcco::DBG_UNFUSED_EXPAND) && gate == nullptr;
  for (int d = 1; d < n_ds; ++d) fuse = fuse && sh[(size_t)d].nnz < ((int64_t)1 << 32);
  const bool fold = fuse && n_ds <= urcco::EXPAND_MULTI_MAX && sh[0].nnz < ((int64_t)1 << 32);
  const int f0 = fold ? 0 : 1;
  std::vector<std::promise<int>> sampled((size_t)n_ds);
  std::vector<std::shared_future<int>> sampled_f((size_t)n_ds);
  for (int d = 0; d < n_ds; ++d) sampled_f[(size_t)d] = sampled[(size_t)d].get_future().share();
  std::promise<int> expanded;
  std::shared_future<int> expanded_f = expanded.get_future().share();
  const int64_t a_cap = sh[0].nnz;
  auto fused_expand = [&]() -> int {
    EvState& L = D.ev[1];
    if (L.s != A.s) HIPC(hipStreamWaitEvent(L.s->stream, D.a_ready, 0));
    std::vector<const int64_t*> rp((size_t)(n_ds - f0));
    std::vector<unsigned*> ps((size_t)(n_ds - f0));
    std::vector<int32_t*> pl((size_t)(n_ds - f0));
    std::vector<int64_t*> ts((size_t)(n_ds - f0));
    for (int d = f0; d < n_ds; ++d) {
      EvState& E = D.ev[(size_t)d];
      if (d > 0 && E.s != L.s) HIPC(hipStreamWaitEvent(L.s->stream, E.ev_sampled, 0));
      URC(E.pre_pstart.ensure((size_t)a_cap + 1));
      URC(E.pre_plen.ensure((size_t)a_cap + 1));
      URC(E.pre_tsum.ensure(expand_tile_words(a_cap)));
      ts[(size_t)(d - f0)] = E.pre_tsum.p;
      rp[(size_t)(d - f0)] = E.s_rp.p;
      ps[(size_t)(d - f0)] = E.pre_pstart.p;
      pl[(size_t)(d - f0)] = E.pre_plen.p;
    }
    URC(expand_multi(L.s, n_ds - f0, D.a_cp[D.par].p, (int32_t)ps_[0].n_cols, D.a_ri[D.par].p, a_cap, rp.data(), n_users, ps.data(), pl.data(), ts.data()));
    HIPC(hipEventRecord(D.b_expanded, L.s->stream));
    return URCCO_OK;
  };
  auto sample_secondary = [&](int d) -> int {
    URC(set_dev(D));
    EvState& E = D.ev[(size_t)d];
    if (gate) URC(gate->wait(D, d));
    URC(stage_raw_counts(D, E, sh[(size_t)d], ps_[(size_t)d]));
    URC(stage_downsample(c, D, d, sh[(size_t)d], ps_[(size_t)d], seed));
    HIPC(hipEventRecord(E.ev_sampled, E.s->stream));
    return URCCO_OK;
  };
  auto rows_secondary = [&](int d) -> int {
    EvState& E = D.ev[(size_t)d];
    if (E.s != A.s) HIPC(hipStreamWaitEvent(E.s->stream, D.a_ready, 0));
    if (fuse && E.s != D.ev[1].s) HIPC(hipStreamWaitEvent(E.s->stream, D.b_expanded, 0));
    E.b_rp = E.s_rp.p;
    E.b_ci = E.s_ci.p;
    E.b_pk_known = false;
    E.b_col_mask = 0xffffffffu;
    E.b_rows = sh[(size_t)d].n_rows;
    E.b_nnz_bound = sh[(size_t)d].nnz;
    URC(stage_rows(D, E, A, d, ps_[0], ps_[(size_t)d], n_users, sh[0].nnz, fuse));
    if (gate && gate->trace) gate->trace->mark("chain enqueued", d);
    if (threaded && gate && gate->after_chain) URC(gate->after_chain(d));
    return URCCO_OK;
  };
  struct Fulfil {
    std::promise<int>* p;
    bool done = false;
    void set(int v) { if (p && !done) { done = true; p->set_value(v); } }
    ~Fulfil() { set(URCCO_INTERNAL); }
  };
  auto secondary_thread = [&](int d) -> int {
    Fulfil my_sample{fuse ? &sampled[(size_t)d] : nullptr};
    Fulfil my_expand{fuse && d == 1 ? &expanded : nullptr};
    int st = sample_secondary(d);
    my_sample.set(st);
    if (st == URCCO_OK) a_recorded_f.wait();
    if (fuse && d == 1) {
      for (int d2 = 2; d2 < n_ds && st == URCCO_OK; ++d2) st = sampled_f[(size_t)d2].get();
      if (st == URCCO_OK) st = a_ok ? fused_expand() : URCCO_INTERNAL;
      my_expand.set(st);
    } else if (fuse && st == URCCO_OK) {
      st = expanded_f.get();
    }
    if (st != URCCO_OK) return st;
    if (!a_ok) return URCCO_INTERNAL;
    return rows_secondary(d);
  };
  std::vector<std::thread> workers;
// ... 428 lines not shown
  } else {
    c->h_bounds.assign((size_t)W + 1, 0);
    for (DevState& D : c->devs) {
      URC(set_dev(D));
      std::vector<int32_t> b((size_t)W + 1);
      URC(urcco_dev_partition(D.ev[0].s, n_items_a, D.work.p, W, b.data()));
      c->h_bounds = b;
      D.item_lo = b[(size_t)D.rank];
      D.item_hi = b[(size_t)D.rank + 1];
    }
    URC(exchange_phase(c, 0, sh, ps, n_users, sizes));
  }
  c->h_sizes.assign((size_t)n_ds, 0);
  int64_t a_nnz = 0;
  for (int r = 0; r < W; ++r) a_nnz += sizes[(size_t)XS * r + 1];
  c->h_sizes[0] = a_nnz;
  URC(c->workers->run([&](size_t g) -> int {
    DevState& D = c->devs[g];
    URC(set_dev(D));
    EvState& A = D.ev[0];
    URC(D.a_cp[D.par].ensure((size_t)n_items_a + 2));
    if (fp.on) {
      int64_t ents = 0;
      for (int p = 0; p < W; ++p) ents += fp.cpb[(size_t)p * (size_t)(W + 1) + (size_t)D.rank + 1] - fp.cpb[(size_t)p * (size_t)(W + 1) + (size_t)D.rank];
      D.a_ents = ents;
      URC(D.a_ri[D.par].ensure((size_t)ents + 4));
      URC(urcco_dev_merge_fragments(A.s, W, D.item_lo, D.item_hi, n_items_a, D.f_len.p, fp.wire16 ? 1 : 0, D.f_ent.p, ents, A.sizes.p, post_of(D, 0).p,
                                    D.a_cp[D.par].p, D.a_ri[D.par].p));
    } else {
      D.a_ents = a_nnz;
      URC(D.a_ri[D.par].ensure((size_t)a_nnz + 4));
      URC(urcco_dev_transpose(A.s, n_users, A.f_rp.p, A.f_ci.p, a_nnz, n_items_a, post_of(D, 0).p, D.item_lo, D.item_hi, D.a_cp[D.par].p, D.a_ri[D.par].p));
    }
    HIPC(hipEventRecord(D.a_ready, A.s->stream));
    return stage_rows(D, A, A, 0, ps[0], ps[0], n_users, D.a_ents);
  }));
  for (int d = 1; d < n_ds; ++d) URC(input_phase(c, d, sh, ps, seed));
  std::vector<int64_t> b_nnz((size_t)n_ds, 0);
  for (int d = 1; d < n_ds; ++d) {
    URC(exchange_phase(c, d, sh, ps, n_users, sizes));
    for (int r = 0; r < W; ++r) b_nnz[(size_t)d] += sizes[(size_t)XS * r + 1];
    c->h_sizes[(size_t)d] = b_nnz[(size_t)d];
  }
  bool fuse = n_ds >= 3 && n_ds - 1 <= urcco::EXPAND_MULTI_MAX && !(c->debug & urcco::DBG_UNFUSED_EXPAND);
  for (int d = 1; d < n_ds; ++d) fuse = fuse && b_nnz[(size_t)d] < ((int64_t)1 << 32);
  URC(c->workers->run([&](size_t g) -> int {
    DevState& D = c->devs[g];
    URC(set_dev(D));
    if (fuse && D.a_ents > 0) {
      EvState& L = D.ev[1];
      if (L.s != D.ev[0].s) HIPC(hipStreamWaitEvent(L.s->stream, D.a_ready, 0));
      std::vector<const int64_t*> rp((size_t)n_ds - 1);
      std::vector<unsigned*> pst((size_t)n_ds - 1);
      std::vector<int32_t*> pl((size_t)n_ds - 1);
      std::vector<int64_t*> ts((size_t)n_ds - 1);
      for (int d = 1; d < n_ds; ++d) {
        EvState& E = D.ev[(size_t)d];
        HIPC(hipEventRecord(E.ev_sampled, E.s->stream));
        if (E.s != L.s) HIPC(hipStreamWaitEvent(L.s->stream, E.ev_sampled, 0));
        URC(E.pre_pstart.ensure((size_t)D.a_ents + 1));
        URC(E.pre_plen.ensure((size_t)D.a_ents + 1));
        URC(E.pre_tsum.ensure(expand_tile_words(D.a_ents)));
        ts[(size_t)d - 1] = E.pre_tsum.p;
        rp[(size_t)d - 1] = E.b_rp;
        pst[(size_t)d - 1] = E.pre_pstart.p;
        pl[(size_t)d - 1] = E.pre_plen.p;
      }
      URC(expand_multi(L.s, n_ds - 1, D.a_cp[D.par].p, n_items_a, D.a_ri[D.par].p, D.a_ents, rp.data(), n_users, pst.data(), pl.data(), ts.data()));
      HIPC(hipEventRecord(D.b_expanded, L.s->stream));
    }
    for (int d = 1; d < n_ds; ++d) {
      EvState& E = D.ev[(size_t)d];
      if (E.s != D.ev[0].s) HIPC(hipStreamWaitEvent(E.s->stream, D.a_ready, 0));
      if (fuse && D.a_ents > 0 && E.s != D.ev[1].s) HIPC(hipStreamWaitEvent(E.s->stream, D.b_expanded, 0));
      URC(stage_rows(D, E, D.ev[0], d, ps[0], ps[(size_t)d], n_users, D.a_ents, fuse && D.a_ents > 0));
    }
    return URCCO_OK;
  }));
  return URCCO_OK;
}

int check_params(const DsParams& p, int d) {
  if (p.n_cols < 0 || p.n_cols > 0x7ffffff0ll) return fail(URCCO_BAD_ARG, "dataset %d: bad column count", d);
  if (p.max_rows <= 0 || p.k <= 0) return fail(URCCO_BAD_ARG, "dataset %d: maxElementsPerRow / maxInterestingElements must be positive", d);
  return URCCO_OK;
}

int run_build(urcco_context* c, const std::vector<std::vector<Shard>>& sh, const std::vector<DsParams>& ps, int64_t n_users, int32_t seed,
              hipStream_t input_stream, InputGate* gate = nullptr) {
  const int n_ds = (int)ps.size();
  for (DevState& D : c->devs) {
    if (!gate) URC(ensure_events(c, D, n_ds));
    D.par = (D.par + 1) % A_SETS;
    for (size_t d = 1; d < D.ev.size(); ++d)
      if (D.ev[d].cons_valid[D.par] && D.ev[d].s != D.ev[0].s) HIPC(hipStreamWaitEvent(D.ev[0].s->stream, D.ev[d].ev_cons[D.par], 0));
    if (input_stream && c->devs.size() == 1) {
      HIPC(hipEventRecord(D.in_ready, input_stream));
      for (int d = 0; d < n_ds; ++d) HIPC(hipStreamWaitEvent(D.ev[(size_t)d].s->stream, D.in_ready, 0));
    }
  }
  if (!c->exchange()) return build_single(c, c->devs[0], [&] {
    std::vector<Shard> one((size_t)n_ds);
    for (int d = 0; d < n_ds; ++d) one[(size_t)d] = sh[(size_t)d][0];
    return one;
  }(), ps, n_users, seed, gate);
  return build_sharded(c, sh, ps, n_users, seed);
}

PendingBuild::~PendingBuild() {
  if (gate)
    for (size_t d = 0; d < gate->staged.size(); ++d)
      if (!gate->released[d]) gate->release((int)d, URCCO_INTERNAL);
  if (builder.joinable()) builder.join();
  for (urcco_indicators& o : res)
    for (void* p : {(void*)o.row_ptr, (void*)o.col_idx, (void*)o.llr})
      if (p) (void)pinned_pool().put(p);
  if (stats_block) (void)pinned_pool().put(stats_block);
}

// ... 735 lines not shown
```

universal-recommender_amd/csrc/urcco_internal.h:

```cpp
#pragma once
#include <hip/hip_runtime.h>

#include <cstdarg>
#include <cstdio>
#include <cstdlib>
#include <cstring>
#include <new>
#include <vector>

#include "../../include/urcco.h"
#include "cco_kernels.h"
static_assert(urcco::EXCH_SIZES == URCCO_EXCH_SIZES && urcco::STATS_LEN == URCCO_STATS_LEN, "include/urcco.h and cco_kernels.h agree");
static_assert(urcco::REC_MAX_CLAUSES == URCCO_REC_MAX_CLAUSES && urcco::REC_MAX_NUM == URCCO_REC_MAX_NUM && urcco::REC_NO_BACKFILL == URCCO_REC_NO_BACKFILL &&
                  urcco::REC_STATS_LEN == URCCO_REC_STATS_LEN && urcco::REC_MAX_RULES == URCCO_REC_MAX_RULES && urcco::REC_RULE_ANY == URCCO_RULE_ANY &&
                  urcco::REC_RULE_NONE == URCCO_RULE_NONE && urcco::REC_RULE_RANGE == URCCO_RULE_RANGE,
              "include/urcco.h and cco_kernels.h agree on the recommendation call");

struct urcco_session;
namespace urcco_detail {

char* err_buf();

inline int fail(int status, const char* fmt, ...) {
  va_list ap;
// ... 3 lines not shown
  return status;
}

inline int hip_fail(hipError_t e, const char* what) {
  return fail(e == hipErrorOutOfMemory ? URCCO_OOM_DEVICE : URCCO_HIP_ERROR, "%s: %s", what, hipGetErrorString(e));
}

#define HIPC(expr)                                                  \
  do {                                                              \
    hipError_t _e = (expr);                                         \
    if (_e != hipSuccess) return urcco_detail::hip_fail(_e, #expr); \
  } while (0)

#define URC(expr)                  \
  do {                             \
    int _s = (expr);               \
    if (_s != URCCO_OK) return _s; \
  } while (0)

template <typename F>
inline int guarded(F&& body) {
  try {
    return body();
  } catch (const std::bad_alloc&) {
    return fail(URCCO_OOM_HOST, "out of host memory");
  } catch (const std::exception& e) {
    return fail(URCCO_INTERNAL, "unexpected exception: %s", e.what());
  } catch (...) {
    return fail(URCCO_INTERNAL, "unexpected exception");
  }
}

inline size_t align_up(size_t v, size_t a) { return (v + a - 1) / a * a; }

struct DebugCfg { bool marks = false, poison = false; };
const DebugCfg& debug_cfg();
void debug_mark(urcco_session* s, int which , int stage);
void debug_register(urcco_session* s);
void debug_unregister(urcco_session* s);
void debug_poison(void* p, size_t bytes, hipStream_t st, bool async);

inline int ceil_log2_i64(int64_t v) {
  int l = 0;
  while (((int64_t)1 << l) < v) ++l;
  return l;
}

}

namespace urcco_detail {
int cco_rows_impl(urcco_session* s, int32_t item_lo, int32_t item_hi, int32_t n_items_a, const int64_t* a_col_ptr, const int32_t* a_row_idx, int64_t nnz_a_bound,
                  const int64_t* b_row_ptr, const int32_t* b_col_idx, int32_t n_cols_b, const int32_t* counts_a, const int32_t* counts_b, int64_t n_users,
                  int32_t exclude_self, int32_t k, int32_t has_min_llr, double min_llr, int32_t* out_count, int32_t* out_idx, double* out_llr, int64_t* stats_dev,
                  const unsigned* pre_pstart, const int32_t* pre_plen, int64_t* pre_tile_sums = nullptr ,
                  const int32_t* b_packed = nullptr , const int32_t* pack_bad = nullptr ,
                  bool pk_known = false ,
                  int64_t b_nnz_bound = -1 );
int pack_counts(urcco_session* s, const int64_t* b_row_ptr, int64_t n_rows_b, const int32_t* b_col_idx, int64_t nnz_bound, const int32_t* counts_b, int32_t n_cols_b,
                int32_t* out, int32_t* bad);
int partition_dev(urcco_session* s, int32_t n_items, const int64_t* work, int32_t n_parts, int32_t* bounds_dev, int32_t** bounds_out);
int expand_multi(urcco_session* s, int n, const int64_t* a_col_ptr, int32_t n_items_a, const int32_t* a_row_idx, int64_t cap, const int64_t* const* b_row_ptr,
                 int64_t n_users, unsigned* const* pstart, int32_t* const* plen, int64_t* const* tile_sums = nullptr );
inline size_t expand_tile_words(int64_t cap) { return (size_t)((cap + urcco::SCAN_TILE - 1) / urcco::SCAN_TILE + 2); }
}

using namespace urcco_detail;

struct urcco_session {
  int device = 0;
  hipStream_t stream = nullptr;
  bool own_stream = false;
  int n_cu = 256;
  char* arena = nullptr;
  size_t arena_cap = 0;
  size_t arena_off = 0;
  int32_t* g_counts = nullptr;
  unsigned long long* g_cand_key = nullptr;
  int32_t* g_cand_col = nullptr;
  int64_t g_cols = 0;
  double* xlx_tab = nullptr;
  double* xlx_hi = nullptr;
  long long xlx_hi_n = -1;
  int debug = 0;
  unsigned long long narrow_limit = urcco::NARROW_LIMIT;
  long long prefix_seed = 0;
  int32_t* form_word = nullptr;
  bool form_valid = false;
  unsigned* marks = nullptr;
  unsigned mark_seq = 0;
  int unordered_rows = 0;
  bool timing = false;
  struct Rec { int stage; hipEvent_t e0, e1; };
  std::vector<Rec> recs;
  std::vector<hipEvent_t> free_events;
  double acc_ms[URCCO_N_STAGES] = {0};
  int64_t acc_n[URCCO_N_STAGES] = {0};

  hipEvent_t get_event() noexcept {
    if (!free_events.empty()) { hipEvent_t e = free_events.back(); free_events.pop_back(); return e; }
    hipEvent_t e = nullptr;
    (void)hipEventCreate(&e);
    return e;
  }
  void begin(int stage) noexcept {
    cur_stage = stage;
    if (marks) debug_mark(this, 0, stage);
    if (!timing) return;
    try {
      recs.reserve(recs.size() + 1);
      free_events.reserve(free_events.size() + 2 * (recs.size() + 1));
    } catch (...) {
      open_rec = false;
      return;
    }
    Rec r{stage, get_event(), get_event()};
// ... 98 lines not shown
```

Before: 35.08 billion pairs/s.

## Fuse intra-tile work scan into multi-expand prepare and store tile-relative offsets

The multi-dataset expand prepare kernel now computes a per-tile exclusive scan of the pair lengths, using DPP wave scans and a shared-memory carry, and writes tile-relative 32-bit offsets in place of raw lengths. This removes the separate reduce pass and most of the downsweep for pre-expanded datasets. The finish kernel recovers lengths from neighbouring offsets and only writes the 64-bit prefix when the form needs it, using a grid-stride launch capped at 8 blocks per CU. Consumers read the work prefix as the tile base plus the offset. The trade-off is extra block-level synchronisation in the prepare kernel, architecture-specific DPP code, and an interface change rippling through several call sites.

```diff
diff --git a/universal-recommender_amd/csrc/cco_common.h b/universal-recommender_amd/csrc/cco_common.h
--- a/universal-recommender_amd/csrc/cco_common.h
+++ b/universal-recommender_amd/csrc/cco_common.h
@@ -23,6 +23,25 @@
   lo = __shfl_up(lo, d);
   hi = __shfl_up(hi, d);
   return (long long)(((unsigned long long)hi << 32) | lo);
+}
+
+__device__ __forceinline__ unsigned wave_inclusive_scan_u32(unsigned v) {
+#ifdef HIPSIM_HOST_BUILD
+  const int lane = threadIdx.x & (WAVE - 1);
+  for (int d = 1; d < WAVE; d <<= 1) {
+    const unsigned o = __shfl_up(v, d);
+    if (lane >= d) v += o;
+  }
+  return v;
+#else
+  v += (unsigned)__builtin_amdgcn_update_dpp(0, (int)v, 0x111, 0xf, 0xf, true);
+  v += (unsigned)__builtin_amdgcn_update_dpp(0, (int)v, 0x112, 0xf, 0xf, true);
+  v += (unsigned)__builtin_amdgcn_update_dpp(0, (int)v, 0x114, 0xf, 0xf, true);
+  v += (unsigned)__builtin_amdgcn_update_dpp(0, (int)v, 0x118, 0xf, 0xf, true);
+  v += (unsigned)__builtin_amdgcn_update_dpp(0, (int)v, 0x142, 0xa, 0xf, false);
+  v += (unsigned)__builtin_amdgcn_update_dpp(0, (int)v, 0x143, 0xc, 0xf, false);
+  return v;
+#endif
 }
 
 __device__ __forceinline__ int64_t upper_bound_i64(const int64_t* __restrict__ rp, int64_t lo, int64_t hi, int64_t e) {
diff --git a/universal-recommender_amd/csrc/cco_expand.hip b/universal-recommender_amd/csrc/cco_expand.hip
--- a/universal-recommender_amd/csrc/cco_expand.hip
+++ b/universal-recommender_amd/csrc/cco_expand.hip
@@ -134,84 +134,114 @@
   return hipGetLastError();
 }
 
-__global__ __launch_bounds__(SCAN_THREADS) void expand_downsweep_kernel(const int32_t* __restrict__ plen, int64_t n, const int64_t* __restrict__ tile_sums,
-                                                                        int64_t n_tiles, int64_t* __restrict__ out, const int64_t* __restrict__ n_live,
-                                                                        const int32_t* __restrict__ form, const unsigned* __restrict__ pstart32,
-                                                                        int64_t* __restrict__ pstart64) {
+template <bool LENS>
+__global__ __launch_bounds__(SCAN_THREADS) void expand_finish_kernel(unsigned* __restrict__ wl, int64_t n, const int64_t* __restrict__ tile_sums, int64_t n_tiles,
+                                                                     int64_t* __restrict__ out, const int64_t* __restrict__ n_live,
+                                                                     const int32_t* __restrict__ form, const unsigned* __restrict__ pstart32,
+                                                                     int64_t* __restrict__ pstart64) {
   __shared__ long long s_wave[SCAN_THREADS / WAVE];
-  if ((int64_t)blockIdx.x * SCAN_TILE > *n_live) return;
   const int f = *form;
-  const LoadI32 ld{plen};
-  const int64_t first = (int64_t)blockIdx.x * SCAN_TILE + (int64_t)threadIdx.x * SCAN_ITEMS;
-  static_assert(SCAN_ITEMS == 8, "load8");
-  long long x[SCAN_ITEMS];
-  long long v = 0;
-  const bool interior = first + SCAN_ITEMS <= n;
-  if (interior) {
-    ld.load8(first, x);
-  } else {
-#pragma unroll
-    for (int q = 0; q < SCAN_ITEMS; ++q) x[q] = first + q < n ? ld(first + q) : 0;
-  }
-#pragma unroll
-  for (int q = 0; q < SCAN_ITEMS; ++q) v += x[q];
-  long long tot;
-  long long run = block_exclusive_scan(v, s_wave, &tot) + tile_sums[blockIdx.x];
-  if (f == 0) {
-    unsigned* out32 = reinterpret_cast<unsigned*>(out);
-    unsigned r = (unsigned)run;
+  if (!LENS && f == 0) return;
+  static_assert(SCAN_ITEMS == 8, "eight consecutive entries per thread");
+  const int64_t live = *n_live;
+  for (int64_t tile = blockIdx.x; tile < n_tiles; tile += gridDim.x) {
+    if (tile * SCAN_TILE > live) break;
+    const int64_t first = tile * SCAN_TILE + (int64_t)threadIdx.x * SCAN_ITEMS;
+    const long long tile_base = tile_sums[tile];
+    long long x[SCAN_ITEMS];
+    const bool interior = first + SCAN_ITEMS <= n;
+    if (LENS) {
+      const LoadI32 ld{reinterpret_cast<const int32_t*>(wl)};
+      if (interior) {
+        ld.load8(first, x);
+      } else {
+#pragma unroll
+        for (int q = 0; q < SCAN_ITEMS; ++q) x[q] = first + q < n ? ld(first + q) : 0;
+      }
+    } else {
+      const unsigned closing = (unsigned)(tile_sums[tile + 1] - tile_base);
+      unsigned e[SCAN_ITEMS + 1];
+#pragma unroll
+      for (int q = 0; q < SCAN_ITEMS; ++q) e[q] = first + q < n ? wl[first + q] : 0u;
+      e[SCAN_ITEMS] = (threadIdx.x + 1 < SCAN_THREADS && first + SCAN_ITEMS < n) ? wl[first + SCAN_ITEMS] : closing;
+#pragma unroll
+      for (int q = 0; q < SCAN_ITEMS; ++q) {
+        const int64_t i = first + q;
+        x[q] = i < n ? (long long)(unsigned)((i + 1 < n ? e[q + 1] : closing) - e[q]) : 0;
+      }
+    }
+    long long v = 0;
+#pragma unroll
+    for (int q = 0; q < SCAN_ITEMS; ++q) v += x[q];
+    long long tot;
+    long long run = block_exclusive_scan(v, s_wave, &tot);
+    if (LENS) {
+      unsigned r = (unsigned)run;
+      if (interior && (reinterpret_cast<uintptr_t>(wl) & 15) == 0) {
+        unsigned e[SCAN_ITEMS];
+#pragma unroll
+        for (int q = 0; q < SCAN_ITEMS; ++q) {
+          e[q] = r;
+          r += (unsigned)x[q];
+        }
+        *reinterpret_cast<uint4*>(wl + first) = make_uint4(e[0], e[1], e[2], e[3]);
+        *reinterpret_cast<uint4*>(wl + first + 4) = make_uint4(e[4], e[5], e[6], e[7]);
+      } else {
+#pragma unroll
+        for (int q = 0; q < SCAN_ITEMS; ++q) {
+          if (first + q < n) wl[first + q] = r;
+          r += (unsigned)x[q];
+        }
+      }
+    }
+    if (f == 0) continue;
+    run += tile_base;
     if (interior && (reinterpret_cast<uintptr_t>(out) & 15) == 0) {
-      unsigned e[SCAN_ITEMS];
+#pragma unroll
+      for (int q = 0; q < SCAN_ITEMS; q += 2) {
+        const long long e0 = run, e1 = run + x[q];
+        run = e1 + x[q + 1];
+        int4 w;
+        w.x = (int)(unsigned)e0; w.y = (int)(unsigned)((unsigned long long)e0 >> 32);
+        w.z = (int)(unsigned)e1; w.w = (int)(unsigned)((unsigned long long)e1 >> 32);
+        *reinterpret_cast<int4*>(out + first + q) = w;
+      }
+    } else {
 #pragma unroll
       for (int q = 0; q < SCAN_ITEMS; ++q) {
-        e[q] = r;
-        r += (unsigned)x[q];
-      }
-      *reinterpret_cast<uint4*>(out32 + first) = make_uint4(e[0], e[1], e[2], e[3]);
-      *reinterpret_cast<uint4*>(out32 + first + 4) = make_uint4(e[4], e[5], e[6], e[7]);
-    } else {
-#pragma unroll
-      for (int q = 0; q < SCAN_ITEMS; ++q) {
-        if (first + q < n) out32[first + q] = r;
-        r += (unsigned)x[q];
-      }
-    }
-    if (blockIdx.x == 0 && threadIdx.x == 0) out32[n] = (unsigned)tile_sums[n_tiles];
-    return;
-  }
-  if (interior && (reinterpret_cast<uintptr_t>(out) & 15) == 0) {
-#pragma unroll
-    for (int q = 0; q < SCAN_ITEMS; q += 2) {
-      const long long e0 = run, e1 = run + x[q];
-      run = e1 + x[q + 1];
-      int4 w;
-      w.x = (int)(unsigned)e0; w.y = (int)(unsigned)((unsigned long long)e0 >> 32);
-      w.z = (int)(unsigned)e1; w.w = (int)(unsigned)((unsigned long long)e1 >> 32);
-      *reinterpret_cast<int4*>(out + first + q) = w;
-    }
-  } else {
-#pragma unroll
-    for (int q = 0; q < SCAN_ITEMS; ++q) {
-      const int64_t i = first + q;
-      if (i < n) out[i] = run;
-      run += x[q];
-    }
-  }
-  if (!(f & FORM_PS64) && pstart32 && pstart64) {
-#pragma unroll
-    for (int q = 0; q < SCAN_ITEMS; ++q)
-      if (first + q < n) pstart64[first + q] = (int64_t)pstart32[first + q];
-  }
-  if (blockIdx.x == 0 && threadIdx.x == 0) out[n] = tile_sums[n_tiles];
-}
-static hipError_t expand_scan(hipStream_t st, const int32_t* plen, int64_t cap, int64_t* wp, int64_t* tile_sums, const int64_t* n_live, bool tile_sums_ready,
+        const int64_t i = first + q;
+        if (i < n) out[i] = run;
+        run += x[q];
+      }
+    }
+    if (!(f & FORM_PS64) && pstart32 && pstart64) {
+#pragma unroll
+      for (int q = 0; q < SCAN_ITEMS; ++q)
+        if (first + q < n) pstart64[first + q] = (int64_t)pstart32[first + q];
+    }
+  }
+  if (blockIdx.x == 0 && threadIdx.x == 0) {
+    if (LENS) wl[n] = (unsigned)(tile_sums[n_tiles] - tile_sums[n / SCAN_TILE]);
+    if (f != 0) out[n] = tile_sums[n_tiles];
+  }
+}
+static hipError_t expand_scan(hipStream_t st, int n_cu, unsigned* wl, bool lens, int64_t cap, int64_t* wp, int64_t* tile_sums, const int64_t* n_live,
                               const unsigned* pstart32, int64_t* pstart64, ExpandForm form) {
   const int64_t n_tiles = cap > 0 ? (cap + SCAN_TILE - 1) / SCAN_TILE : 1;
-  if (!tile_sums_ready || cap <= 0)
-    hipLaunchKernelGGL((scan_reduce_kernel<LoadI32>), dim3((unsigned)n_tiles), dim3(SCAN_THREADS), 0, st, LoadI32{plen}, cap, tile_sums, n_live);
+  if (cap <= 0) lens = true;
+  if (lens)
+    hipLaunchKernelGGL((scan_reduce_kernel<LoadI32>), dim3((unsigned)n_tiles), dim3(SCAN_THREADS), 0, st, LoadI32{reinterpret_cast<const int32_t*>(wl)}, cap,
+                       tile_sums, n_live);
   hipLaunchKernelGGL(scan_tiles_kernel, dim3(1), dim3(ST_THREADS), 0, st, tile_sums, n_tiles, n_live, form);
-  hipLaunchKernelGGL(expand_downsweep_kernel, dim3((unsigned)n_tiles), dim3(SCAN_THREADS), 0, st, plen, cap, (const int64_t*)tile_sums, n_tiles, wp, n_live,
-                     (const int32_t*)form.word, pstart32, pstart64);
+  if (lens) {
+    hipLaunchKernelGGL(expand_finish_kernel<true>, dim3((unsigned)n_tiles), dim3(SCAN_THREADS), 0, st, wl, cap, (const int64_t*)tile_sums, n_tiles, wp, n_live,
+                       (const int32_t*)form.word, pstart32, pstart64);
+  } else if (!form.host_narrow) {
+    int64_t blocks = n_tiles;
+    if (blocks > (int64_t)n_cu * 8) blocks = (int64_t)n_cu * 8;
+    hipLaunchKernelGGL(expand_finish_kernel<false>, dim3((unsigned)blocks), dim3(SCAN_THREADS), 0, st, wl, cap, (const int64_t*)tile_sums, n_tiles, wp, n_live,
+                       (const int32_t*)form.word, pstart32, pstart64);
+  }
   return hipGetLastError();
 }
 
@@ -282,7 +312,7 @@
     hipLaunchKernelGGL(expand_prepare_kernel, dim3((unsigned)blocks), dim3(256), 0, st, a_col_ptr, n_items_a, a_row_idx, b_row_ptr,
                        (const unsigned*)b_rp32_scratch, n_rows_b, cap, pstart32, pstart64, plen, form.word);
   }
-  return expand_scan(st, plen, cap, wp, tile_sums, a_col_ptr + n_items_a, false, pstart32, pstart64, form);
+  return expand_scan(st, n_cu, reinterpret_cast<unsigned*>(plen), true, cap, wp, tile_sums, a_col_ptr + n_items_a, pstart32, pstart64, form);
 }
 
 struct __attribute__((packed, aligned(4))) Words4 { unsigned a, b, c, d; };
@@ -290,7 +320,7 @@
 struct ExpandMultiArgs {
   const int64_t* b_rp[EXPAND_MULTI_MAX];
   unsigned* pstart[EXPAND_MULTI_MAX];
-  int32_t* plen[EXPAND_MULTI_MAX];
+  unsigned* wl[EXPAND_MULTI_MAX];
   int64_t* tsum[EXPAND_MULTI_MAX];
   int n;
 };
@@ -302,15 +332,25 @@
 __global__ __launch_bounds__(256) void expand_prepare_multi_kernel(const int64_t* __restrict__ a_cp, int32_t n_items_a, const int32_t* __restrict__ a_ri,
                                                                    const unsigned* __restrict__ T, int64_t cap, ExpandMultiArgs a) {
   __shared__ long long s_part[256 / WAVE][N];
+  __shared__ __attribute__((aligned(16))) unsigned s_scan[2][2][N][256 / WAVE];
+  static_assert(256 / WAVE == 4 && (SCAN_ITEMS / 2) % 2 == 0, "one 16-byte read per total; the buffers alternate consistently from tile to tile");
+  const int lane = threadIdx.x & (WAVE - 1), wave = threadIdx.x / WAVE;
   const int64_t nnz = a_cp[n_items_a];
   int64_t lim = (nnz / SCAN_TILE + 1) * SCAN_TILE;
   if (lim > cap) lim = cap;
   const int64_t n_tiles = (lim + SCAN_TILE - 1) / SCAN_TILE;
+  const int64_t wlim = lim + ((lim == cap && cap % SCAN_TILE != 0) ? 1 : 0);
+  if (blockIdx.x == 0 && threadIdx.x < N && cap % SCAN_TILE == 0) a.wl[threadIdx.x][cap] = 0u;
   for (int64_t tile = blockIdx.x; tile < n_tiles; tile += gridDim.x) {
     const int64_t base = tile * SCAN_TILE;
     long long sum[N];
-#pragma unroll
-    for (int d = 0; d < N; ++d) sum[d] = 0;
+    unsigned carry[N];
+#pragma unroll
+    for (int d = 0; d < N; ++d) {
+      sum[d] = 0;
+      carry[d] = 0u;
+    }
+#pragma unroll 1
     for (int r = 0; r < SCAN_ITEMS; r += 2) {
       int u[2];
       unsigned v[2][2 * N];
@@ -345,17 +385,31 @@
           for (int d = 0; d < 2 * N; ++d) v[q][d] = 0u;
         }
       }
+      unsigned exc[2][N];
+      const int buf = (r >> 1) & 1;
 #pragma unroll
       for (int q = 0; q < 2; ++q) {
         const int64_t p = base + (int64_t)(r + q) * 256 + threadIdx.x;
-        if (p < lim) {
-#pragma unroll
-          for (int d = 0; d < N; ++d) {
-            const int32_t len = (int32_t)(v[q][N + d] - v[q][d]);
-            a.pstart[d][p] = v[q][d];
-            a.plen[d][p] = len;
-            sum[d] += (long long)len;
-          }
+#pragma unroll
+        for (int d = 0; d < N; ++d) {
+          const unsigned len = v[q][N + d] - v[q][d];
+          if (p < lim) a.pstart[d][p] = v[q][d];
+          sum[d] += (long long)(int32_t)len;
+          const unsigned inc = wave_inclusive_scan_u32(len);
+          if (lane == WAVE - 1) s_scan[buf][q][d][wave] = inc;
+          exc[q][d] = inc - len;
+        }
+      }
+      __syncthreads();
+#pragma unroll
+      for (int q = 0; q < 2; ++q) {
+        const int64_t p = base + (int64_t)(r + q) * 256 + threadIdx.x;
+#pragma unroll
+        for (int d = 0; d < N; ++d) {
+          const uint4 t = *reinterpret_cast<const uint4*>(&s_scan[buf][q][d][0]);
+          const unsigned before = carry[d] + (wave > 0 ? t.x : 0u) + (wave > 1 ? t.y : 0u) + (wave > 2 ? t.z : 0u);
+          carry[d] += t.x + t.y + t.z + t.w;
+          if (p < wlim) a.wl[d][p] = before + exc[q][d];
         }
       }
     }
@@ -367,7 +421,7 @@
       if ((threadIdx.x & (WAVE - 1)) == 0) s_part[threadIdx.x / WAVE][d] = (long long)x;
     }
     __syncthreads();
-    if (threadIdx.x < N && a.tsum[threadIdx.x]) {
+    if (threadIdx.x < N) {
       long long tot = 0;
 #pragma unroll
       for (int w = 0; w < 256 / WAVE; ++w) tot += s_part[w][threadIdx.x];
@@ -377,17 +431,19 @@
   }
 }
 hipError_t launch_expand_prepare_multi(hipStream_t st, int n_cu, const int64_t* a_col_ptr, int32_t n_items_a, const int32_t* a_row_idx, int n,
-                                       const int64_t* const* b_row_ptr, int64_t n_rows_b, int64_t cap, unsigned* const* pstart, int32_t* const* plen, void* T,
+                                       const int64_t* const* b_row_ptr, int64_t n_rows_b, int64_t cap, unsigned* const* pstart, unsigned* const* wl, void* T,
                                        int64_t* const* tsum) {
-  if (n < 1 || n > EXPAND_MULTI_MAX) return hipErrorInvalidValue;
+  if (n < 1 || n > EXPAND_MULTI_MAX || !tsum || !wl) return hipErrorInvalidValue;
+  for (int d = 0; d < n; ++d)
+    if (!tsum[d] || !wl[d]) return hipErrorInvalidValue;
   if (cap <= 0) return hipSuccess;
   ExpandMultiArgs a;
   a.n = n;
   for (int d = 0; d < EXPAND_MULTI_MAX; ++d) {
     a.b_rp[d] = d < n ? b_row_ptr[d] : nullptr;
     a.pstart[d] = d < n ? pstart[d] : nullptr;
-    a.plen[d] = d < n ? plen[d] : nullptr;
-    a.tsum[d] = (d < n && tsum) ? tsum[d] : nullptr;
+    a.wl[d] = d < n ? wl[d] : nullptr;
+    a.tsum[d] = d < n ? tsum[d] : nullptr;
   }
   int64_t nb = (n_rows_b + 255) / 256;
   if (nb > (int64_t)n_cu * 8) nb = (int64_t)n_cu * 8;
@@ -409,39 +465,39 @@
   }
   return hipGetLastError();
 }
-hipError_t launch_expand_scan(hipStream_t st, const int64_t* a_col_ptr, int32_t n_items_a, const int32_t* plen, int64_t cap, int64_t* wp, int64_t* tile_sums,
-                              bool tile_sums_ready, const unsigned* pstart32, int64_t* pstart64, ExpandForm form) {
+hipError_t launch_expand_scan(hipStream_t st, int n_cu, const int64_t* a_col_ptr, int32_t n_items_a, unsigned* wl, int64_t cap, int64_t* wp, int64_t* tile_sums,
+                              const unsigned* pstart32, int64_t* pstart64, ExpandForm form) {
   hipError_t e = hipMemsetAsync(form.word, 0, sizeof(int32_t), st);
   if (e != hipSuccess) return e;
-  return expand_scan(st, plen, cap, wp, tile_sums, a_col_ptr + n_items_a, tile_sums_ready, pstart32, pstart64, form);
-}
-
-__device__ __forceinline__ int64_t work_prefix_at(const int64_t* __restrict__ wp, const int64_t* __restrict__ tile_sums, bool narrow, int64_t p) {
+  return expand_scan(st, n_cu, wl, false, cap, wp, tile_sums, a_col_ptr + n_items_a, pstart32, pstart64, form);
+}
+
+__device__ __forceinline__ int64_t work_prefix_at(const int64_t* __restrict__ wp, const unsigned* __restrict__ wl, const int64_t* __restrict__ tile_sums, bool narrow,
+                                                  int64_t p) {
   if (!narrow) return wp[p];
-  const int64_t base = tile_sums[p / SCAN_TILE];
-  return base + (int64_t)(unsigned)(reinterpret_cast<const unsigned*>(wp)[p] - (unsigned)base);
-}
-__global__ __launch_bounds__(256) void row_work_kernel(int32_t item_lo, int32_t item_hi, const int64_t* __restrict__ a_cp,
-                                                       const int64_t* __restrict__ wp, const int64_t* __restrict__ tile_sums, const int32_t* __restrict__ form,
+  return tile_sums[p / SCAN_TILE] + (int64_t)wl[p];
+}
+__global__ __launch_bounds__(256) void row_work_kernel(int32_t item_lo, int32_t item_hi, const int64_t* __restrict__ a_cp, const int64_t* __restrict__ wp,
+                                                       const unsigned* __restrict__ wl, const int64_t* __restrict__ tile_sums, const int32_t* __restrict__ form,
                                                        int64_t* __restrict__ work) {
   const int64_t n = (int64_t)item_hi - item_lo;
   const bool narrow = *form == 0;
   for (int64_t t = (int64_t)blockIdx.x * 256 + threadIdx.x; t < n; t += (int64_t)gridDim.x * 256) {
     const int64_t i = item_lo + t;
-    work[t] = work_prefix_at(wp, tile_sums, narrow, a_cp[i + 1]) - work_prefix_at(wp, tile_sums, narrow, a_cp[i]);
-  }
-}
-
-hipError_t launch_row_work(hipStream_t st, int n_cu, int32_t item_lo, int32_t item_hi, const int64_t* a_col_ptr, const int64_t* wp, const int64_t* tile_sums,
-                           const int32_t* form, int64_t* work) {
+    work[t] = work_prefix_at(wp, wl, tile_sums, narrow, a_cp[i + 1]) - work_prefix_at(wp, wl, tile_sums, narrow, a_cp[i]);
+  }
+}
+
+hipError_t launch_row_work(hipStream_t st, int n_cu, int32_t item_lo, int32_t item_hi, const int64_t* a_col_ptr, const int64_t* wp, const unsigned* wl,
+                           const int64_t* tile_sums, const int32_t* form, int64_t* work) {
   const int64_t n = (int64_t)item_hi - item_lo;
   if (n <= 0) return hipSuccess;
   int64_t blocks = (n + 255) / 256;
   const int64_t cap = (int64_t)n_cu * 8;
   if (blocks > cap) blocks = cap;
-  hipLaunchKernelGGL(row_work_kernel, dim3((unsigned)blocks), dim3(256), 0, st, item_lo, item_hi, a_col_ptr, wp, tile_sums, form, work);
-  return hipGetLastError();
-}
-
-
-}
+  hipLaunchKernelGGL(row_work_kernel, dim3((unsigned)blocks), dim3(256), 0, st, item_lo, item_hi, a_col_ptr, wp, wl, tile_sums, form, work);
+  return hipGetLastError();
+}
+
+
+}
diff --git a/universal-recommender_amd/csrc/cco_kernels.h b/universal-recommender_amd/csrc/cco_kernels.h
--- a/universal-recommender_amd/csrc/cco_kernels.h
+++ b/universal-recommender_amd/csrc/cco_kernels.h
@@ -8,6 +8,8 @@
 constexpr int MP_KMAX_HOST = 256;
 
 constexpr int SCAN_TILE = 2048;
+constexpr int SCAN_TILE_LOG2 = 11;
+static_assert((1 << SCAN_TILE_LOG2) == SCAN_TILE, "scan tile");
 constexpr int DS_TILE = 4096;
 constexpr int GLOBAL_BIN_BLOCKS = 128;
 constexpr int BIN_TILE = 1024;
@@ -88,6 +90,8 @@
   int32_t g_blocks;
   const int64_t* pstart64;
   const int64_t* work;
+  const unsigned* wl;
+  const int64_t* tile_base;
 };
 
 hipError_t launch_column_counts(hipStream_t st, int n_cu, const int32_t* col_idx, int64_t nnz, int32_t n_cols, int32_t* counts);
@@ -167,12 +171,12 @@
                                  unsigned* pstart32, int64_t* pstart64, int32_t* plen, int64_t* wp, int64_t* tile_sums, ExpandForm form);
 constexpr int EXPAND_MULTI_MAX = 8;
 hipError_t launch_expand_prepare_multi(hipStream_t st, int n_cu, const int64_t* a_col_ptr, int32_t n_items_a, const int32_t* a_row_idx, int n,
-                                       const int64_t* const* b_row_ptr, int64_t n_rows_b, int64_t cap, unsigned* const* pstart, int32_t* const* plen, void* T,
+                                       const int64_t* const* b_row_ptr, int64_t n_rows_b, int64_t cap, unsigned* const* pstart, unsigned* const* wl , void* T,
                                        int64_t* const* tsum );
-hipError_t launch_expand_scan(hipStream_t st, const int64_t* a_col_ptr, int32_t n_items_a, const int32_t* plen, int64_t cap, int64_t* wp, int64_t* tile_sums,
-                              bool tile_sums_ready, const unsigned* pstart32, int64_t* pstart64, ExpandForm form);
-hipError_t launch_row_work(hipStream_t st, int n_cu, int32_t item_lo, int32_t item_hi, const int64_t* a_col_ptr, const int64_t* wp, const int64_t* tile_sums,
-                           const int32_t* form, int64_t* work);
+hipError_t launch_expand_scan(hipStream_t st, int n_cu, const int64_t* a_col_ptr, int32_t n_items_a, unsigned* wl, int64_t cap, int64_t* wp, int64_t* tile_sums,
+                              const unsigned* pstart32, int64_t* pstart64, ExpandForm form);
+hipError_t launch_row_work(hipStream_t st, int n_cu, int32_t item_lo, int32_t item_hi, const int64_t* a_col_ptr, const int64_t* wp, const unsigned* wl,
+                           const int64_t* tile_sums, const int32_t* form, int64_t* work);
 
 hipError_t launch_binning(hipStream_t st, int32_t item_lo, int32_t n, const int64_t* work, const int32_t* cnt_a, int32_t n_cols_b,
                           int32_t count_bits, int32_t k, int64_t* tile_counts, int32_t* bin_off, int32_t* bin_rows, int64_t* stats);
diff --git a/universal-recommender_amd/csrc/cco_rows.hip b/universal-recommender_amd/csrc/cco_rows.hip
--- a/universal-recommender_amd/csrc/cco_rows.hip
+++ b/universal-recommender_amd/csrc/cco_rows.hip
@@ -466,12 +466,25 @@
 constexpr int URCCO_SEL_M_BLOCK = 128;
 constexpr int URCCO_G_CU = 2;
 template <bool NARROW> struct PStart { typedef int64_t type; };
+struct WpPair { unsigned base, in; };
+template <bool NARROW>
+__device__ __forceinline__ WpPair wp_pair(const unsigned* __restrict__ w , const unsigned* __restrict__ tb , int64_t p) {
+  WpPair r;
+  if constexpr (NARROW) {
+    r.base = tb[2 * ((uint64_t)p >> SCAN_TILE_LOG2)];
+    r.in = w[p];
+  } else {
+    r.base = 0u;
+    r.in = w[2 * p];
+  }
+  return r;
+}
+#define URCCO_SETTLE_WP(narrow, x) do { URCCO_SETTLE((x).in); if constexpr (narrow) URCCO_SETTLE((x).base); } while (0)
 template <> struct PStart<true> { typedef unsigned type; };
 template <int T, int E, int U, bool MP = false, bool DBG = false, bool PK = false>
 __global__ __launch_bounds__((T < 256 ? 256 : T), (T == 64 ? URCCO_OCC_WAVE : (T == 256 && E == 4096 ? URCCO_OCC_BS : (T == 512 ? 4 : 1)))) void cco_rows_kernel(CcoArgs a, int bin) {
   if ((a.b_packed != nullptr && (a.pk_known != 0 || *a.form == 0)) != PK) return;
   using PS = typename PStart<PK>::type;
-  constexpr int WS = PK ? 1 : 2;
   const int dbg = DBG ? a.debug : 0;
   constexpr bool packed = PK;
   URCCO_OWN_GLOBAL_PTR(const int32_t, b_col_idx, PK ? a.b_packed : a.b_col_idx);
@@ -556,7 +569,8 @@
   if (li >= list_n) return;
   const int S = total_teams;
   auto pos_of = [&](int l) { return list_start + (l < list_n ? l : list_n - 1); };
-  const unsigned* wp32 = reinterpret_cast<const unsigned*>(a.wp);
+  const unsigned* wp32 = PK ? a.wl : reinterpret_cast<const unsigned*>(a.wp);
+  const unsigned* tb32 = reinterpret_cast<const unsigned*>(a.tile_base);
   const PS* pstart;
   if constexpr (PK) pstart = a.pstart32;
   else pstart = a.pstart64;
@@ -571,17 +585,17 @@
     ce_c = uni(a.a_col_ptr[id0 + 1]);
     bnd_b = a.a_col_ptr[id1 + (lane & 1)];
   }
-  unsigned pf_w0, pf_w1, pf_wp;
+  WpPair pf_w0, pf_w1, pf_wp;
   PS pf_start;
   {
     const int64_t c1 = cs_c + T < ce_c ? cs_c + T : ce_c;
     const int64_t pl = cs_c + tl < c1 ? cs_c + tl : c1 - 1;
-    pf_w0 = wp32[WS * cs_c];
-    pf_w1 = wp32[WS * c1];
-    pf_wp = wp32[WS * pl];
+    pf_w0 = wp_pair<PK>(wp32, tb32, cs_c);
+    pf_w1 = wp_pair<PK>(wp32, tb32, c1);
+    pf_wp = wp_pair<PK>(wp32, tb32, pl);
     pf_start = pstart[pl];
   }
-  URCCO_SETTLE(idv); URCCO_SETTLE(bnd_b); URCCO_SETTLE(pf_w0); URCCO_SETTLE(pf_w1); URCCO_SETTLE(pf_wp); URCCO_SETTLE(pf_start);
+  URCCO_SETTLE(idv); URCCO_SETTLE(bnd_b); URCCO_SETTLE_WP(PK, pf_w0); URCCO_SETTLE_WP(PK, pf_w1); URCCO_SETTLE_WP(PK, pf_wp); URCCO_SETTLE(pf_start);
   int64_t cs_n = 0, ce_n = 0, bnd_c = 0;
   for (; li < list_n; li += S, cs_c = cs_n, ce_c = ce_n, bnd_b = bnd_c) {
     const int i = (int)wave_read_lane((unsigned)idv, 0);
@@ -589,8 +603,8 @@
     const int64_t cs = cs_c, ce = ce_c;
     cs_n = wave_read_lane64(bnd_b, 0);
     ce_n = wave_read_lane64(bnd_b, 1);
-    const unsigned row_w0 = uni(pf_w0), row_w1 = uni(pf_w1);
-    const unsigned my_wp = pf_wp;
+    const unsigned row_w0 = uni(pf_w0.base + pf_w0.in), row_w1 = uni(pf_w1.base + pf_w1.in);
+    const unsigned my_wp = pf_wp.base + pf_wp.in;
     const PS my_start = pf_start;
     int lz = lane;
     URCCO_OPAQUE(lz);
@@ -599,9 +613,9 @@
     if (!MP) {
       const int64_t c1 = cs_n + T < ce_n ? cs_n + T : ce_n;
       const int64_t pl = cs_n + tl < c1 ? cs_n + tl : c1 - 1;
-      pf_w0 = wp32[WS * cs_n];
-      pf_w1 = wp32[WS * c1];
-      pf_wp = wp32[WS * pl];
+      pf_w0 = wp_pair<PK>(wp32, tb32, cs_n);
+      pf_w1 = wp_pair<PK>(wp32, tb32, c1);
+      pf_wp = wp_pair<PK>(wp32, tb32, pl);
       pf_start = pstart[pl];
     }
     int mp_s = 0;
@@ -639,12 +653,22 @@
     for (int64_t c0 = cs; c0 < ce; c0 += T) {
       const int64_t c1 = c0 + T < ce ? c0 + T : ce;
       const bool pre = !MP && c0 == cs;
-      const unsigned w0 = pre ? row_w0 : uni(wp32[WS * c0]);
-      const unsigned total = (pre ? row_w1 : uni(wp32[WS * c1])) - w0;
+      unsigned w0 = row_w0, w1 = row_w1;
+      if (!pre) {
+        const WpPair x0 = wp_pair<PK>(wp32, tb32, c0), x1 = wp_pair<PK>(wp32, tb32, c1);
+        w0 = uni(x0.base + x0.in);
+        w1 = uni(x1.base + x1.in);
+      }
+      const unsigned total = w1 - w0;
       const int64_t p = c0 + tl;
       if (p < c1) {
         ustart[tl] = pre ? my_start : pstart[p];
-        uoff[tl] = (pre ? my_wp : wp32[WS * p]) - w0;
+        unsigned wpp = my_wp;
+        if (!pre) {
+          const WpPair x = wp_pair<PK>(wp32, tb32, p);
+          wpp = x.base + x.in;
+        }
+        uoff[tl] = wpp - w0;
       } else {
         uoff[tl] = total;
       }
@@ -823,7 +847,7 @@
       }
     }
     URCCO_SETTLE(idv); URCCO_SETTLE(bnd_c);
-    if (!MP) { URCCO_SETTLE(pf_w0); URCCO_SETTLE(pf_w1); URCCO_SETTLE(pf_wp); URCCO_SETTLE(pf_start); }
+    if (!MP) { URCCO_SETTLE_WP(PK, pf_w0); URCCO_SETTLE_WP(PK, pf_w1); URCCO_SETTLE_WP(PK, pf_wp); URCCO_SETTLE(pf_start); }
     if (SKIP_SHARED) {
       wave_and_or_u64(kand, kor);
       if (lane == 0) {
@@ -1197,7 +1221,6 @@
 __global__ __launch_bounds__(256, (L == WAVE ? URCCO_OCC_MICRO : URCCO_OCC_MICRO - 2)) void cco_rows_micro_kernel(CcoArgs a) {
   if ((a.b_packed != nullptr && (a.pk_known != 0 || *a.form == 0)) != PK) return;
   using PS = typename PStart<PK>::type;
-  constexpr int WS = PK ? 1 : 2;
   using G = MicroGeom<L>;
   constexpr int S = G::S;
   const int dbg = DBG ? a.debug : 0;
@@ -1245,13 +1268,14 @@
   if (li >= n_groups) return;
   const int stride = total_teams;
   auto row_at = [&](int g) { const int l = g * S + seg; return bin_rows[list_start + (l < list_n ? l : list_n - 1)]; };
-  const unsigned* wp32 = reinterpret_cast<const unsigned*>(a.wp);
+  const unsigned* wp32 = PK ? a.wl : reinterpret_cast<const unsigned*>(a.wp);
+  const unsigned* tb32 = reinterpret_cast<const unsigned*>(a.tile_base);
   const unsigned* cnt_words = use16 ? reinterpret_cast<const unsigned*>(a.cnt_b16) : reinterpret_cast<const unsigned*>(a.cnt_b);
   int i_cur = row_at(li);
   int i_n1 = row_at(li + stride);
   int i_n2 = row_at(li + 2 * stride);
   int64_t cs1 = a_col_ptr[i_n1], ce1 = a_col_ptr[i_n1 + 1];
-  unsigned pf_w1, pf_wp;
+  WpPair pf_w1, pf_wp;
   PS pf_start;
   int pf_ca;
   double pf_ent;
@@ -1260,33 +1284,34 @@
     const int64_t cs0 = a_col_ptr[i_cur], ce0 = a_col_ptr[i_cur + 1];
     n_cur = (int)(ce0 - cs0);
     const int64_t pl = sl < n_cur ? cs0 + sl : ce0 - 1;
-    pf_w1 = wp32[WS * ce0];
-    pf_wp = wp32[WS * pl];
+    pf_w1 = wp_pair<PK>(wp32, tb32, ce0);
+    pf_wp = wp_pair<PK>(wp32, tb32, pl);
     pf_start = pstart[pl];
     pf_ca = cnt_a[i_cur];
     pf_ent = ent_a[i_cur];
   }
-  URCCO_SETTLE(pf_w1); URCCO_SETTLE(pf_wp); URCCO_SETTLE(pf_start); URCCO_SETTLE(pf_ca); URCCO_SETTLE(pf_ent);
+  URCCO_SETTLE_WP(PK, pf_w1); URCCO_SETTLE_WP(PK, pf_wp); URCCO_SETTLE(pf_start); URCCO_SETTLE(pf_ca); URCCO_SETTLE(pf_ent);
   URCCO_SETTLE(cs1); URCCO_SETTLE(ce1); URCCO_SETTLE(i_n2);
 #pragma unroll
   for (int q = 0; q < 4; ++q) tab_w[lane + q * WAVE] = 0u;
   for (; li < n_groups; li += stride) {
     const int i = i_cur;
     const bool live = S == 1 || li * S + seg < list_n;
-    const unsigned w0 = S == 1 ? wave_read_lane(pf_wp, 0) : wave_gather(pf_wp, (unsigned)(lane & ~(L - 1)));
-    const unsigned total = live ? pf_w1 - w0 : 0u;
+    const unsigned cur_wp = pf_wp.base + pf_wp.in;
+    const unsigned w0 = S == 1 ? wave_read_lane(cur_wp, 0) : wave_gather(cur_wp, (unsigned)(lane & ~(L - 1)));
+    const unsigned total = live ? pf_w1.base + pf_w1.in - w0 : 0u;
     const bool owns_user = live && sl < n_cur;
     const long long ca = (long long)pf_ca;
     const double row_entropy = pf_ent;
     const PS my_start = owns_user ? pf_start : (PS)0;
-    const unsigned my_off = owns_user ? pf_wp - w0 : total;
+    const unsigned my_off = owns_user ? cur_wp - w0 : total;
     int i_n3 = row_at(li + 3 * stride);
     int64_t cs2 = a_col_ptr[i_n2], ce2 = a_col_ptr[i_n2 + 1];
     n_cur = (int)(ce1 - cs1);
     {
       const int64_t pl = sl < n_cur ? cs1 + sl : ce1 - 1;
-      pf_w1 = wp32[WS * ce1];
-      pf_wp = wp32[WS * pl];
+      pf_w1 = wp_pair<PK>(wp32, tb32, ce1);
+      pf_wp = wp_pair<PK>(wp32, tb32, pl);
       pf_start = pstart[pl];
       pf_ca = cnt_a[i_n1];
       pf_ent = ent_a[i_n1];
@@ -1352,7 +1377,7 @@
     const int n_valid = __popcll(valid_mask & seg_mask);
     const bool all_fit_k = (int)seg_max_popc<L>(valid_mask) <= a.k;
     auto settle_prefetch = [&]() {
-      URCCO_SETTLE(pf_w1); URCCO_SETTLE(pf_wp); URCCO_SETTLE(pf_start); URCCO_SETTLE(pf_ca); URCCO_SETTLE(pf_ent);
+      URCCO_SETTLE_WP(PK, pf_w1); URCCO_SETTLE_WP(PK, pf_wp); URCCO_SETTLE(pf_start); URCCO_SETTLE(pf_ca); URCCO_SETTLE(pf_ent);
       URCCO_SETTLE(cs2); URCCO_SETTLE(ce2); URCCO_SETTLE(i_n3);
     };
     if (a.unordered && all_fit_k && !(dbg & DBG_NO_TOPK)) {
@@ -1419,9 +1444,10 @@
 constexpr int GSEL_K = 1024;
 
 __device__ __forceinline__ int64_t g_start(const unsigned* ps32, const int64_t* ps64, bool nar, int64_t p) { return nar ? (int64_t)ps32[p] : ps64[p]; }
-__device__ __forceinline__ int64_t g_len(const int64_t* wp, bool nar, int64_t p) {
-  const unsigned* w = reinterpret_cast<const unsigned*>(wp);
-  return nar ? (int64_t)(unsigned)(w[p + 1] - w[p]) : wp[p + 1] - wp[p];
+__device__ __forceinline__ int64_t g_len(const int64_t* wp, const unsigned* wl, const int64_t* tile_base, bool nar, int64_t p) {
+  if (!nar) return wp[p + 1] - wp[p];
+  const unsigned* tb = reinterpret_cast<const unsigned*>(tile_base);
+  return (int64_t)(unsigned)((tb[2 * ((p + 1) >> SCAN_TILE_LOG2)] + wl[p + 1]) - (tb[2 * (p >> SCAN_TILE_LOG2)] + wl[p]));
 }
 __global__ __launch_bounds__(GB_THREADS) void cco_rows_global_kernel(CcoArgs a) {
   constexpr int NW = GB_THREADS / WAVE;
@@ -1449,14 +1475,14 @@
     const int64_t cs = a.a_col_ptr[i], ce = a.a_col_ptr[i + 1];
     if (threadIdx.x == 0) s_ncand = 0;
     for (int64_t p = cs + grp; p < ce; p += ngrp) {
-      const int64_t s = g_start(a.pstart32, a.pstart64, nar, p), e = s + g_len(a.wp, nar, p);
+      const int64_t s = g_start(a.pstart32, a.pstart64, nar, p), e = s + g_len(a.wp, a.wl, a.tile_base, nar, p);
       for (int64_t q = s + gl; q < e; q += G) atomicAdd(&cnt[(unsigned)a.b_col_idx[q] & a.b_col_mask], 1);
     }
     __syncthreads();
     const long long ca = a.cnt_a[i];
     const double row_entropy = a.ent_a[i];
     for (int64_t p = cs + grp; p < ce; p += ngrp) {
-      const int64_t s = g_start(a.pstart32, a.pstart64, nar, p), e = s + g_len(a.wp, nar, p);
+      const int64_t s = g_start(a.pstart32, a.pstart64, nar, p), e = s + g_len(a.wp, a.wl, a.tile_base, nar, p);
       for (int64_t q = s + gl; q < e; q += G) {
         const int j = (int)((unsigned)a.b_col_idx[q] & a.b_col_mask);
         const long long k11 = atomicExch(&cnt[j], 0);
diff --git a/universal-recommender_amd/csrc/urcco_api.hip b/universal-recommender_amd/csrc/urcco_api.hip
--- a/universal-recommender_amd/csrc/urcco_api.hip
+++ b/universal-recommender_amd/csrc/urcco_api.hip
@@ -334,17 +334,17 @@
     return fail(URCCO_BAD_ARG, "urcco_dev_row_work: bad argument");
   const int64_t cap = nnz_a_bound;
   const int64_t n_tiles = (cap + urcco::SCAN_TILE - 1) / urcco::SCAN_TILE;
-  URC(s->reserve(urcco_session::need((size_t)cap, 4) + urcco_session::need((size_t)cap + 1, 8) + urcco_session::need((size_t)n_tiles + 2, 8)));
+  URC(s->reserve(urcco_session::need((size_t)cap + 1, 4) + urcco_session::need((size_t)cap + 1, 8) + urcco_session::need((size_t)n_tiles + 2, 8)));
   if (!s->form_word) HIPC(hipMalloc((void**)&s->form_word, sizeof(int32_t)));
   s->form_valid = false;
-  int32_t* plen = s->take<int32_t>((size_t)cap);
+  int32_t* plen = s->take<int32_t>((size_t)cap + 1);
   int64_t* wp = s->take<int64_t>((size_t)cap + 1);
   int64_t* tile_sums = s->take<int64_t>((size_t)n_tiles + 2);
   int32_t* form = s->form_word;
   s->begin(URCCO_STAGE_ROW_WORK);
   HIPC(urcco::launch_expand_prepare(s->stream, s->n_cu, a_col_ptr, n_items_a, a_row_idx, b_row_ptr, nullptr, 0, cap, nullptr, nullptr, plen, wp, tile_sums,
                                     urcco::ExpandForm{form, nullptr, 0, 0, s->narrow_limit, s->prefix_seed}));
-  HIPC(urcco::launch_row_work(s->stream, s->n_cu, item_lo, item_hi, a_col_ptr, wp, tile_sums, form, work));
+  HIPC(urcco::launch_row_work(s->stream, s->n_cu, item_lo, item_hi, a_col_ptr, wp, reinterpret_cast<const unsigned*>(plen), tile_sums, form, work));
   s->form_valid = true;
   s->end();
   return URCCO_OK;
@@ -388,7 +388,7 @@
                        const int32_t* counts_a, const int32_t* counts_b, int64_t n_users, int32_t exclude_self, int32_t k,
                        int32_t has_min_llr, double min_llr, int32_t* out_count, int32_t* out_idx, double* out_llr, int64_t* stats_dev) {
   return urcco_detail::cco_rows_impl(s, item_lo, item_hi, n_items_a, a_col_ptr, a_row_idx, nnz_a_bound, b_row_ptr, b_col_idx, n_cols_b, counts_a, counts_b, n_users,
-                                     exclude_self, k, has_min_llr, min_llr, out_count, out_idx, out_llr, stats_dev, nullptr, nullptr);
+                                     exclude_self, k, has_min_llr, min_llr, out_count, out_idx, out_llr, stats_dev, nullptr, nullptr, nullptr);
 }
 
 int urcco_dev_pack_counts(urcco_session* s, int64_t n_rows_b, const int64_t* b_row_ptr, const int32_t* b_col_idx, int64_t nnz_b_bound, const int32_t* counts_b,
@@ -425,9 +425,11 @@
 int cco_rows_impl(urcco_session* s, int32_t item_lo, int32_t item_hi, int32_t n_items_a, const int64_t* a_col_ptr, const int32_t* a_row_idx, int64_t nnz_a_bound,
                   const int64_t* b_row_ptr, const int32_t* b_col_idx, int32_t n_cols_b, const int32_t* counts_a, const int32_t* counts_b, int64_t n_users,
                   int32_t exclude_self, int32_t k, int32_t has_min_llr, double min_llr, int32_t* out_count, int32_t* out_idx, double* out_llr, int64_t* stats_dev,
-                  const unsigned* pre_pstart, const int32_t* pre_plen, int64_t* pre_tile_sums, const int32_t* b_packed, const int32_t* pack_bad, bool pk_known, int64_t b_nnz_bound) {
+                  const unsigned* pre_pstart, unsigned* pre_wl, int64_t* pre_tile_sums, const int32_t* b_packed, const int32_t* pack_bad, bool pk_known, int64_t b_nnz_bound) {
   if (!s || item_lo < 0 || item_hi < item_lo || item_hi > n_items_a || n_cols_b < 0 || n_users < 0 || nnz_a_bound < 0 || !a_col_ptr || !b_row_ptr)
     return fail(URCCO_BAD_ARG, "urcco_dev_cco_rows: bad argument");
+  const bool pre = pre_pstart != nullptr;
+  if (pre != (pre_wl != nullptr) || pre != (pre_tile_sums != nullptr)) return fail(URCCO_BAD_ARG, "urcco_dev_cco_rows: a prepared expand share comes as three tables");
   if (k <= 0) return fail(URCCO_BAD_ARG, "maxInterestingElements must be positive, got %d", k);
   const int32_t n = item_hi - item_lo;
   if (n == 0) {
@@ -460,15 +462,16 @@
   const int64_t p_tiles = (cap + urcco::SCAN_TILE - 1) / urcco::SCAN_TILE;
   if (!s->form_word) HIPC(hipMalloc((void**)&s->form_word, sizeof(int32_t)));
   s->form_valid = false;
-  URC(s->reserve(urcco_session::need((size_t)cap, 8) + urcco_session::need((size_t)cap, 4) + (pre_pstart ? 0 : urcco_session::need((size_t)cap, 4)) + urcco_session::need((size_t)cap + 1, 8) +
+  URC(s->reserve(urcco_session::need((size_t)cap, 8) + (pre ? 0 : urcco_session::need((size_t)cap, 4) + urcco_session::need((size_t)cap + 1, 4)) + urcco_session::need((size_t)cap + 1, 8) +
                  urcco_session::need((size_t)p_tiles + 2, 8) +
                  urcco_session::need((size_t)n, 8) + urcco_session::need((size_t)(n_tiles + 1) * urcco::BIN_COLS_HOST, 8) +
                  urcco_session::need(urcco::BIN_OFF_LEN, 4) + urcco_session::need((size_t)n, 4) + urcco_session::need((size_t)n_items_a, 8) +
                  urcco_session::need((size_t)n_cols_b, 2) + urcco_session::need(1, 4) + urcco_session::need(urcco::CAND_SLOTS, 8) + urcco_session::need(1, 8) + urcco_session::need(URCCO_STATS_LEN, 8) +
                  urcco_session::need((size_t)n_users + 1, 4)));
   int64_t* pstart64 = s->take<int64_t>((size_t)cap);
-  unsigned* own_pstart = pre_pstart ? nullptr : s->take<unsigned>((size_t)cap);
-  int32_t* own_plen = s->take<int32_t>((size_t)cap);
+  unsigned* own_pstart = pre ? nullptr : s->take<unsigned>((size_t)cap);
+  int32_t* own_plen = pre ? nullptr : s->take<int32_t>((size_t)cap + 1);
+  const unsigned* wl = pre ? pre_wl : reinterpret_cast<const unsigned*>(own_plen);
   const unsigned* pstart32 = pre_pstart ? pre_pstart : own_pstart;
   int64_t* wp = s->take<int64_t>((size_t)cap + 1);
   int32_t* form = s->form_word;
@@ -490,13 +493,13 @@
   const bool narrow_known = pk_known && !host_wide && b_nnz_bound >= 0 && b_nnz_bound < ((int64_t)1 << 32) &&
                             (unsigned long long)n_cols_b * (unsigned long long)urcco::SCAN_TILE < s->narrow_limit;
   const urcco::ExpandForm ef{form, pk_known ? nullptr : pack_bad, host_wide ? 1 : 0, narrow_known ? 1 : 0, s->narrow_limit, s->prefix_seed};
-  int64_t* tile_sums = (pre_pstart && pre_plen && pre_tile_sums) ? pre_tile_sums : p_tile_sums;
+  int64_t* tile_sums = pre ? pre_tile_sums : p_tile_sums;
   s->begin(URCCO_STAGE_ROW_WORK);
-  if (pre_pstart && pre_plen)
-    HIPC(urcco::launch_expand_scan(s->stream, a_col_ptr, n_items_a, pre_plen, cap, wp, tile_sums, pre_tile_sums != nullptr, pre_pstart, pstart64, ef));
+  if (pre)
+    HIPC(urcco::launch_expand_scan(s->stream, s->n_cu, a_col_ptr, n_items_a, pre_wl, cap, wp, tile_sums, pre_pstart, pstart64, ef));
   else
     HIPC(urcco::launch_expand_prepare(s->stream, s->n_cu, a_col_ptr, n_items_a, a_row_idx, b_row_ptr, b_rp32, n_users, cap, own_pstart, pstart64, own_plen, wp, tile_sums, ef));
-  HIPC(urcco::launch_row_work(s->stream, s->n_cu, item_lo, item_hi, a_col_ptr, wp, tile_sums, form, work));
+  HIPC(urcco::launch_row_work(s->stream, s->n_cu, item_lo, item_hi, a_col_ptr, wp, wl, tile_sums, form, work));
   s->form_valid = true;
   s->end();
   s->begin(URCCO_STAGE_BINNING);
@@ -510,7 +513,7 @@
 
   urcco::CcoArgs a;
   a.bin_rows = bin_rows; a.bin_off = bin_off;
-  a.a_col_ptr = a_col_ptr; a.pstart32 = pstart32; a.pstart64 = pstart64; a.wp = wp; a.form = form; a.work = work; a.b_col_idx = b_col_idx;
+  a.a_col_ptr = a_col_ptr; a.pstart32 = pstart32; a.pstart64 = pstart64; a.wp = wp; a.wl = wl; a.tile_base = tile_sums; a.form = form; a.work = work; a.b_col_idx = b_col_idx;
   a.b_packed = packed; a.pk_known = narrow_known ? 1 : 0;
   a.b_col_mask = pk_known ? (key_bits >= 32 ? 0xffffffffu : (1u << key_bits) - 1u) : 0xffffffffu;
   a.cnt_a = counts_a; a.cnt_b = counts_b; a.ent_a = ent_a; a.cnt_b16 = cnt_b16; a.cnt16_bad = cnt16_bad; a.xlx_n = xlx_n; a.xlx_tab = s->xlx_tab; a.xlx_hi = s->xlx_hi; a.col_ent = s->xlx_hi + urcco::XLX_TABLE_HOST; a.debug = s->debug;
@@ -552,12 +555,12 @@
 }
 
 int expand_multi(urcco_session* s, int n, const int64_t* a_col_ptr, int32_t n_items_a, const int32_t* a_row_idx, int64_t cap, const int64_t* const* b_row_ptr,
-                 int64_t n_users, unsigned* const* pstart, int32_t* const* plen, int64_t* const* tile_sums) {
-  if (!s || n < 1 || n > urcco::EXPAND_MULTI_MAX || !a_col_ptr || cap < 0) return fail(URCCO_BAD_ARG, "expand_multi: bad argument");
+                 int64_t n_users, unsigned* const* pstart, unsigned* const* wl, int64_t* const* tile_sums) {
+  if (!s || n < 1 || n > urcco::EXPAND_MULTI_MAX || !a_col_ptr || cap < 0 || !pstart || !wl || !tile_sums) return fail(URCCO_BAD_ARG, "expand_multi: bad argument");
   URC(s->reserve(urcco_session::need(((size_t)n_users + 2) * (size_t)n, 4) + 256));
   void* T = s->take<unsigned>(((size_t)n_users + 2) * (size_t)n);
   s->begin(URCCO_STAGE_ROW_WORK);
-  HIPC(urcco::launch_expand_prepare_multi(s->stream, s->n_cu, a_col_ptr, n_items_a, a_row_idx, n, b_row_ptr, n_users, cap, pstart, plen, T, tile_sums));
+  HIPC(urcco::launch_expand_prepare_multi(s->stream, s->n_cu, a_col_ptr, n_items_a, a_row_idx, n, b_row_ptr, n_users, cap, pstart, wl, T, tile_sums));
   s->end();
   return URCCO_OK;
 }
diff --git a/universal-recommender_amd/csrc/urcco_context.hip b/universal-recommender_amd/csrc/urcco_context.hip
--- a/universal-recommender_amd/csrc/urcco_context.hip
+++ b/universal-recommender_amd/csrc/urcco_context.hip
@@ -175,7 +175,7 @@
     return URCCO_OK;
   }
   DBuf<unsigned> pre_pstart;
-  DBuf<int32_t> pre_plen;
+  DBuf<unsigned> pre_wl;
   DBuf<int64_t> pre_tsum;
   DBuf<int32_t> mlen, pack;
   DBuf<unsigned short> mlen16;
@@ -191,7 +191,7 @@
     in_rp.release(); in_ci.release(); raw.release(); post.release(); s_rp.release(); s_ci.release(); deg.release(); f_deg.release();
     deg16.release(); f_deg16.release();
     f_rp.release(); f_ci.release(); sizes.release(); scan_tmp.release(); o_count.release(); o_idx.release(); o_llr.release(); c_rp.release();
-    c_idx.release(); c_llr.release(); stats.release(); verr.release(); b_pk.release(); pk_bad.release(); s_pk.release(); pre_pstart.release(); pre_plen.release(); pre_tsum.release();
+    c_idx.release(); c_llr.release(); stats.release(); verr.release(); b_pk.release(); pk_bad.release(); s_pk.release(); pre_pstart.release(); pre_wl.release(); pre_tsum.release();
     mlen.release(); pack.release(); mlen16.release(); mlen_bad.release(); moff.release(); mtmp.release(); to_nnz.release();
     if (h_verr) (void)hipHostFree(h_verr);
     h_verr = nullptr;
@@ -512,7 +512,7 @@
   }
   URC(cco_rows_impl(E.s, D.item_lo, D.item_hi, (int32_t)pa.n_cols, D.a_cp[D.par].p, D.a_ri[D.par].p, a_nnz_bound, E.b_rp, E.b_ci, (int32_t)p.n_cols,
                     post_of(D, 0).p, post_of(D, d).p, n_users, d == 0 ? 1 : 0, p.k, p.has_min_llr, p.min_llr, E.o_count.p, E.o_idx.p, E.o_llr.p, E.stats.p,
-                    pre_expanded ? E.pre_pstart.p : nullptr, pre_expanded ? E.pre_plen.p : nullptr, pre_expanded ? E.pre_tsum.p : nullptr,
+                    pre_expanded ? E.pre_pstart.p : nullptr, pre_expanded ? E.pre_wl.p : nullptr, pre_expanded ? E.pre_tsum.p : nullptr,
                     E.b_pk_known ? nullptr : E.b_pk.p, E.b_pk_known ? nullptr : E.pk_bad.p, E.b_pk_known, E.b_nnz_bound));
   URC(urcco_dev_compact_indicators(E.s, n, p.k, E.o_count.p, E.o_idx.p, E.o_llr.p, E.c_rp.p, E.c_idx.p, E.c_llr.p));
   HIPC(hipEventRecord(E.ev_done, E.s->stream));
@@ -576,18 +576,18 @@
     if (L.s != A.s) HIPC(hipStreamWaitEvent(L.s->stream, D.a_ready, 0));
     std::vector<const int64_t*> rp((size_t)(n_ds - f0));
     std::vector<unsigned*> ps((size_t)(n_ds - f0));
-    std::vector<int32_t*> pl((size_t)(n_ds - f0));
+    std::vector<unsigned*> pl((size_t)(n_ds - f0));
     std::vector<int64_t*> ts((size_t)(n_ds - f0));
     for (int d = f0; d < n_ds; ++d) {
       EvState& E = D.ev[(size_t)d];
       if (d > 0 && E.s != L.s) HIPC(hipStreamWaitEvent(L.s->stream, E.ev_sampled, 0));
       URC(E.pre_pstart.ensure((size_t)a_cap + 1));
-      URC(E.pre_plen.ensure((size_t)a_cap + 1));
+      URC(E.pre_wl.ensure((size_t)a_cap + 1));
       URC(E.pre_tsum.ensure(expand_tile_words(a_cap)));
       ts[(size_t)(d - f0)] = E.pre_tsum.p;
       rp[(size_t)(d - f0)] = E.s_rp.p;
       ps[(size_t)(d - f0)] = E.pre_pstart.p;
-      pl[(size_t)(d - f0)] = E.pre_plen.p;
+      pl[(size_t)(d - f0)] = E.pre_wl.p;
     }
     URC(expand_multi(L.s, n_ds - f0, D.a_cp[D.par].p, (int32_t)ps_[0].n_cols, D.a_ri[D.par].p, a_cap, rp.data(), n_users, ps.data(), pl.data(), ts.data()));
     HIPC(hipEventRecord(D.b_expanded, L.s->stream));
@@ -1122,19 +1122,19 @@
       if (L.s != D.ev[0].s) HIPC(hipStreamWaitEvent(L.s->stream, D.a_ready, 0));
       std::vector<const int64_t*> rp((size_t)n_ds - 1);
       std::vector<unsigned*> pst((size_t)n_ds - 1);
-      std::vector<int32_t*> pl((size_t)n_ds - 1);
+      std::vector<unsigned*> pl((size_t)n_ds - 1);
       std::vector<int64_t*> ts((size_t)n_ds - 1);
       for (int d = 1; d < n_ds; ++d) {
         EvState& E = D.ev[(size_t)d];
         HIPC(hipEventRecord(E.ev_sampled, E.s->stream));
         if (E.s != L.s) HIPC(hipStreamWaitEvent(L.s->stream, E.ev_sampled, 0));
         URC(E.pre_pstart.ensure((size_t)D.a_ents + 1));
-        URC(E.pre_plen.ensure((size_t)D.a_ents + 1));
+        URC(E.pre_wl.ensure((size_t)D.a_ents + 1));
         URC(E.pre_tsum.ensure(expand_tile_words(D.a_ents)));
         ts[(size_t)d - 1] = E.pre_tsum.p;
         rp[(size_t)d - 1] = E.b_rp;
         pst[(size_t)d - 1] = E.pre_pstart.p;
-        pl[(size_t)d - 1] = E.pre_plen.p;
+        pl[(size_t)d - 1] = E.pre_wl.p;
       }
       URC(expand_multi(L.s, n_ds - 1, D.a_cp[D.par].p, n_items_a, D.a_ri[D.par].p, D.a_ents, rp.data(), n_users, pst.data(), pl.data(), ts.data()));
       HIPC(hipEventRecord(D.b_expanded, L.s->stream));
diff --git a/universal-recommender_amd/csrc/urcco_internal.h b/universal-recommender_amd/csrc/urcco_internal.h
--- a/universal-recommender_amd/csrc/urcco_internal.h
+++ b/universal-recommender_amd/csrc/urcco_internal.h
@@ -79,7 +79,7 @@
 int cco_rows_impl(urcco_session* s, int32_t item_lo, int32_t item_hi, int32_t n_items_a, const int64_t* a_col_ptr, const int32_t* a_row_idx, int64_t nnz_a_bound,
                   const int64_t* b_row_ptr, const int32_t* b_col_idx, int32_t n_cols_b, const int32_t* counts_a, const int32_t* counts_b, int64_t n_users,
                   int32_t exclude_self, int32_t k, int32_t has_min_llr, double min_llr, int32_t* out_count, int32_t* out_idx, double* out_llr, int64_t* stats_dev,
-                  const unsigned* pre_pstart, const int32_t* pre_plen, int64_t* pre_tile_sums = nullptr ,
+                  const unsigned* pre_pstart, unsigned* pre_wl , int64_t* pre_tile_sums ,
                   const int32_t* b_packed = nullptr , const int32_t* pack_bad = nullptr ,
                   bool pk_known = false ,
                   int64_t b_nnz_bound = -1 );
@@ -87,7 +87,7 @@
                 int32_t* out, int32_t* bad);
 int partition_dev(urcco_session* s, int32_t n_items, const int64_t* work, int32_t n_parts, int32_t* bounds_dev, int32_t** bounds_out);
 int expand_multi(urcco_session* s, int n, const int64_t* a_col_ptr, int32_t n_items_a, const int32_t* a_row_idx, int64_t cap, const int64_t* const* b_row_ptr,
-                 int64_t n_users, unsigned* const* pstart, int32_t* const* plen, int64_t* const* tile_sums = nullptr );
+                 int64_t n_users, unsigned* const* pstart, unsigned* const* wl , int64_t* const* tile_sums );
 inline size_t expand_tile_words(int64_t cap) { return (size_t)((cap + urcco::SCAN_TILE - 1) / urcco::SCAN_TILE + 2); }
 }
 
```

Result: no change. 35.07 billion pairs/s (-0.0%).
